# TIGER-AI-Lab/AnyV2V

Measured on AMD Instinct MI355X. Metric: frames/sec for 16fx512x512 DDIM-inversion+PnP-edit; spatial-attn MFMA % of peak, higher is better.
Workload: dtype f16; 1 GPU; BASELINE config 3 per GPU: 1 clip x 16f x 512x512, 50-step DDIM inversion (UNet B=1) + 50-step PnP edit (UNet B=3, cfg 9.0, conv+spatial+temporal injection on every step); a bench step = 1 inversion step + 1 edit step = 1/50 clip; I2VGen-XL 3D-UNet 1.42B params, random init; frames=16, hip_graphs=True, finite=True

## Files before the change

anyv2v_amd/_lib.py:

```python
from __future__ import annotations

import ctypes as C
import os

_HERE = os.path.dirname(os.path.abspath(__file__))
LIB_PATH = os.path.join(_HERE, "libanyv2v_hip.so")
ABI_VERSION = 105


class HipExtensionMissing(RuntimeError):
    pass


class HipKernelError(RuntimeError):
    pass


class GemmDesc(C.Structure):
    _fields_ = [
        ("A0", C.c_void_p), ("A1", C.c_void_p), ("W", C.c_void_p), ("C", C.c_void_p),
        ("bias", C.c_void_p), ("rowvec", C.c_void_p), ("R", C.c_void_p),
        ("M", C.c_int32), ("N", C.c_int32), ("C0", C.c_int32), ("C1", C.c_int32),
        ("lda0", C.c_int32), ("lda1", C.c_int32), ("ldc", C.c_int32), ("ldr", C.c_int32),
        ("ldrv", C.c_int32), ("rowvec_div", C.c_int32), ("mode", C.c_int32),
        ("Hi", C.c_int32), ("Wi", C.c_int32), ("Ho", C.c_int32), ("Wo", C.c_int32),
        ("stride", C.c_int32), ("up", C.c_int32), ("asym", C.c_int32), ("F", C.c_int32), ("HW", C.c_int32),
        ("act", C.c_int32), ("flags", C.c_int32),
        ("workspace", C.c_void_p), ("workspace_bytes", C.c_int64),
        ("ln_c1", C.c_void_p), ("ln_eps", C.c_float), ("reserved0", C.c_int32),
        ("gn_stats", C.c_void_p), ("gn_stats_floats", C.c_int64), ("gn_rows_per_group", C.c_int32), ("gn_groups", C.c_int32),
    ]

ANYV2V_GEMM_NAIVE = 1 << 0
ANYV2V_GEMM_LDS_DMA = 1 << 1
ANYV2V_GEMM_NO_BIG = 1 << 2
ANYV2V_GEMM_FORCE_BIG = 1 << 3
ANYV2V_GEMM_NO_SPLITK = 1 << 4
ANYV2V_GEMM_PROBE_TRACE = 1 << 5
ANYV2V_GEMM_PROBE_KO_SHIFT = 6
ANYV2V_GEMM_NO_WS = 1 << 9
ANYV2V_GEMM_FORCE_WS = 1 << 10
ANYV2V_GEMM_NF4 = 1 << 11
ANYV2V_GEMM_NF5 = 1 << 12
ANYV2V_GEMM_RASTER_SHIFT = 13
ANYV2V_GEMM_RASTER_NFAST = 1 << 16
ANYV2V_GEMM_PP = 1 << 17
ANYV2V_GEMM_NO_PP = 1 << 18
ANYV2V_GEMM_PP_192 = 1 << 19
ANYV2V_GEMM_PP_256 = 1 << 20
ANYV2V_GEMM_SW = 1 << 21
ANYV2V_GEMM_NO_SW = 1 << 22
ANYV2V_GEMM_PROBE_SW_KO_SHIFT = 23
ANYV2V_GEMM_STREAMK = 1 << 26
ANYV2V_GEMM_FORCE_STREAMK = 1 << 27
ANYV2V_GEMM_SWH = 1 << 28
ANYV2V_GEMM_PROBE_KORDER_SHIFT = 29


class FFDesc(C.Structure):
    _fields_ = [
        ("X", C.c_void_p), ("W1", C.c_void_p), ("b1", C.c_void_p), ("W2", C.c_void_p), ("b2", C.c_void_p), ("R", C.c_void_p),
        ("Y", C.c_void_p), ("M", C.c_int32), ("C", C.c_int32), ("H", C.c_int32), ("ldx", C.c_int32), ("ldr", C.c_int32),
        ("ldy", C.c_int32), ("flags", C.c_int32), ("reserved0", C.c_int32),
    ]


class AttnDesc(C.Structure):
    _fields_ = [
        ("Q", C.c_void_p), ("K", C.c_void_p), ("V", C.c_void_p), ("O", C.c_void_p),
        ("ldq", C.c_int32), ("ldk", C.c_int32), ("ldv", C.c_int32), ("ldo", C.c_int32),
        ("batch", C.c_int32), ("heads", C.c_int32), ("Sq", C.c_int32), ("Sk", C.c_int32),
        ("inner", C.c_int32),
        ("q_outer", C.c_int64), ("q_inner", C.c_int64), ("q_seq", C.c_int64),
        ("kv_outer", C.c_int64), ("kv_inner", C.c_int64), ("kv_seq", C.c_int64),
        ("kv_div", C.c_int32), ("qk_mod", C.c_int32), ("scale", C.c_float), ("flags", C.c_int32),
    ]


_VP, _I32, _I64, _F32 = C.c_void_p, C.c_int32, C.c_int64, C.c_float
SYMBOLS = {
    "anyv2v_gemm_f16": (C.c_int, [C.POINTER(GemmDesc), _VP]),
    "anyv2v_gemm_gn_stats_floats": (C.c_int64, [C.POINTER(GemmDesc)]),
    "anyv2v_gemm_gn_launches": (C.c_int64, [_I32]),
    "anyv2v_ff_geglu_f16": (C.c_int, [C.POINTER(FFDesc), _VP]),
    "anyv2v_groupnorm_f16": (C.c_int, [_VP, _VP, _I32, _I32, _VP, _VP, _VP, _VP, _I32, _I32, _I32, _F32, _I32, _VP]),
    "anyv2v_groupnorm_scratch_floats": (C.c_int64, [_I32, _I32, _I32]),
    "anyv2v_groupnorm_stats_floats": (C.c_int64, [_I32, _I32, _I32]),
    "anyv2v_groupnorm_apply_stats_f16": (C.c_int, [_VP, _VP, _VP, _VP, _VP, C.POINTER(C.c_int32), _F32, _I32, _VP]),
    "anyv2v_groupnorm_partial_floats": (C.c_int64, [_I32, _I32, _I32, _I32]),
    "anyv2v_groupnorm_partial_f16": (C.c_int, [_VP, _VP, _I32, _I32, _VP, _I32, _I32, _I32, _VP]),
    "anyv2v_groupnorm_apply_f16": (C.c_int, [_VP, _VP, _I32, _I32, _VP, _VP, _VP, _VP, _I32, _I32, _I32, _F32, _I32, _I32, _VP]),
    "anyv2v_groupnorm_pivot_f16": (C.c_int, [_VP, _VP, _I32, _I32, _VP, _I32, _I32, _I32, _I32, _VP]),
    "anyv2v_groupnorm_partial_pivot_f16": (C.c_int, [_VP, _VP, _I32, _I32, _VP, _VP, _I32, _I32, _I32, _VP]),
    "anyv2v_groupnorm_apply_pivot_f16": (C.c_int, [_VP, _VP, _I32, _I32, _VP, _VP, _VP, _VP, _VP, _I32, _I32, _I32, _F32, _I32, _I32, _VP]),
    "anyv2v_layernorm_f16": (C.c_int, [_VP, _VP, _VP, _VP, _I32, _I32, _F32, _VP]),
    "anyv2v_attention_f16": (C.c_int, [C.POINTER(AttnDesc), _VP]),
    "anyv2v_attention_small_f16": (C.c_int, [C.POINTER(AttnDesc), _I32, _VP]),
    "anyv2v_attention_bias_f16": (C.c_int, [C.POINTER(AttnDesc), _I32, _VP, _VP]),
    "anyv2v_softmax_rows_f32_f16": (C.c_int, [_VP, _I32, _VP, _I32, _I32, _I32, _F32, _VP]),
    "anyv2v_silu_f16": (C.c_int, [_VP, _VP, _I64, _VP]),
    "anyv2v_add_f16": (C.c_int, [_VP, _VP, _VP, _I64, _VP]),
    "anyv2v_timestep_embedding_f16": (C.c_int, [_VP, _VP, _I32, _I32, _VP]),
    "anyv2v_ncfhw_to_tokens_f16": (C.c_int, [_VP, _VP, _I32, _I32, _I32, _I32, _I32, _I32, _VP]),
    "anyv2v_tokens_to_ncfhw_f16": (C.c_int, [_VP, _VP, _I32, _I32, _I32, _I32, _I32, _I32, _VP]),
    "anyv2v_adaptive_avgpool_f16": (C.c_int, [_VP, _VP, _I32, _I32, _I32, _I32, _I32, _I32, _VP]),
    "anyv2v_copy_cols_f16": (C.c_int, [_VP, _I32, _I32, _VP, _I32, _I32, _I64, _I32, _VP]),
    "anyv2v_gather_rows_f16": (C.c_int, [_VP, _I32, _I32, _VP, _VP, _I32, _I32, _I64, _I32, _VP]),
    "anyv2v_freeu_f16": (C.c_int, [_VP, _I32, _VP, _I32, _I32, _F32, _VP, _I32, _VP, _I32, _I32, _F32, _I32, _I32, _I32, _VP]),
    "anyv2v_rotary_f16":(C.c_int, [_VP, _I32, _I64, _I32, _I32, _I32, _I32, _I32, _I32, C.c_float, _VP]),
    "anyv2v_cfg_ddim_step_f16": (C.c_int, [_VP, _I32, _I32, _I32, _F32, _VP, _VP, _VP, _I32, _I32, _I32, _VP]),
    "anyv2v_ddim_step_f16": (C.c_int, [_VP, _VP, _VP, _F32, _F32, _F32, _F32, _I64, _VP]),
    "anyv2v_guided_step_f16": (C.c_int, [_VP, _I64, _I32, _I32, _I32, _F32, _F32, _I32, _F32, _F32, _F32, _F32, _VP, _VP, _VP]),
    "anyv2v_guided_step_noise_f16": (C.c_int, [_VP, _I64, _I32, _I32, _I32, _F32, _F32, _I32, _F32, _F32, _F32, _F32, _VP, _VP, _VP, _F32, _VP]),
    "anyv2v_set_batch_hint": (C.c_int, [_I32, _I32]),
    "anyv2v_last_error": (C.c_char_p, []),
    "anyv2v_version": (C.c_int, []),
    "anyv2v_selftest": (C.c_int, [_VP, _I64, _VP]),
}

_lib = None


def load():
    global _lib
    if _lib is not None:
        return _lib
    if not os.path.isfile(LIB_PATH):
        raise HipExtensionMissing(
            f"{LIB_PATH} not found: the HIP kernels are the product path and there is no fallback. "
            f"Build with `make -C {os.path.join(_HERE, 'csrc')}` (or `python -c 'import __graft_entry__ as g; g.build()'`).")
    lib = C.CDLL(LIB_PATH)
    for name, (res, args) in SYMBOLS.items():
        fn = getattr(lib, name)
        fn.restype = res
        fn.argtypes = args
    if lib.anyv2v_version() < ABI_VERSION:
        raise HipExtensionMissing(f"{LIB_PATH} is ABI {lib.anyv2v_version()}, this binding needs >= {ABI_VERSION}: rebuild it "
                                  f"(`make -C {os.path.join(_HERE, 'csrc')}`)")
    _lib = lib
    return lib


def check(rc: int, what: str = ""):
    if rc != 0:
        msg = load().anyv2v_last_error()
        raise HipKernelError(f"{what} failed (rc={rc}): {msg.decode() if msg else ''}")
```

anyv2v_amd/csrc/gemm.hip:

```cpp
#include <stdlib.h>

#include "gemm_common.h"

__device__ __attribute__((aligned(256))) half_t g_zero_line[128];

static const half_t* zero_line() {
    static const half_t* z = nullptr;
    if (z == nullptr) {
        void* ptr = nullptr;
        if (hipGetSymbolAddress(&ptr, HIP_SYMBOL(g_zero_line)) == hipSuccess) z = (const half_t*)ptr;
    }
    return z;
}

static int64_t g_gn_launches = 0;

extern "C" int anyv2v_gemm_f16(const AnyV2VGemmDesc* d, void* stream) {
    AV_CHECK(d != nullptr, "gemm: null descriptor");
    AV_CHECK(d->A0 && d->W && d->C, "gemm: null A0/W/C");
    const int hinted = av_hint_rows(d->M);
    const GemmPlan plan = av_gemm_plan(*d, hinted);
    AV_CHECK(d->gn_stats == nullptr || plan.gn_decline == nullptr,
             "gemm: gn_stats set, but this launch runs on %s, which writes no GroupNorm statistics (ask anyv2v_gemm_gn_stats_floats first)",
             plan.gn_decline);
    if (plan.status != ANYV2V_OK) return plan.status;
    GemmK k = {};
    k.A0 = (const half_t*)d->A0;
    k.A1 = d->C1 > 0 ? (const half_t*)d->A1 : (const half_t*)d->A0;
    k.W = (const half_t*)d->W;
    k.C = (half_t*)d->C;
    k.bias = (const half_t*)d->bias;
    k.rowvec = (const half_t*)d->rowvec;
    k.R = (const half_t*)d->R;
    k.zeros = zero_line();
    AV_CHECK(k.zeros != nullptr, "gemm: zero line symbol unavailable");
    k.M = d->M; k.N = d->N; k.C0 = d->C0; k.C1 = d->C1;
    k.lda0 = d->lda0; k.lda1 = d->C1 > 0 ? d->lda1 : d->lda0; k.ldc = d->ldc; k.ldr = d->ldr; k.ldrv = d->ldrv;
    k.rowvec_div = d->rowvec_div > 0 ? d->rowvec_div : 1;
    k.mode = d->mode; k.Hi = d->Hi; k.Wi = d->Wi; k.Ho = d->Ho; k.Wo = d->Wo; k.stride = d->stride; k.up = d->up;
    k.F = d->F; k.HW = d->HW; k.act = d->act;
    k.pad_lo = d->asym ? 0 : 1;
    k.taps = plan.taps; k.Ktot = k.taps * (d->C0 + d->C1); k.nt0 = d->C0 / 64; k.nt1 = d->C1 / 64;
    k.tilesN = plan.tilesN; k.vec_epi = plan.vec_epi; k.splits = plan.splits;
    if (plan.splits > 1 || plan.family == GEMM_SW_STREAMK) k.partial = (float*)d->workspace;
    if (plan.family == GEMM_WS_LN) k.ln_c1 = d->ln_c1, k.ln_eps = d->ln_eps;
    k.rast_gm = plan.rast_gm; k.rast_gn = plan.rast_gn; k.rast_sm = plan.rast_sm; k.rast_sn = plan.rast_sn; k.rast_nfast = plan.rast_nfast;
    if (d->gn_stats != nullptr) {
        AV_CHECK(d->gn_stats_floats >= (int64_t)3 * (d->M / 16) * d->gn_groups, "gemm: gn_stats holds %lld floats, the launch writes %lld",
                 (long long)d->gn_stats_floats, (long long)3 * (d->M / 16) * d->gn_groups);
        AV_CHECK((((uintptr_t)d->gn_stats) & 3) == 0, "gemm: gn_stats must be 4-byte aligned");
        k.gn_stats = d->gn_stats;
        k.gn_groups = d->gn_groups;
        k.gn_cg = d->N / d->gn_groups;
        ++g_gn_launches;
    }
    static const bool log_on = getenv("ANYV2V_GEMM_LOG") != nullptr;
    if (log_on)
        fprintf(stderr, "gemm-plan mode %d M %d (hinted %d) N %d K %d act %d res %d big %d splits %d kernel %s nf %d grid %d\n", d->mode, d->M,
                hinted, d->N, k.Ktot, d->act, d->R != nullptr, plan.family == GEMM_BIG, plan.splits, av_gemm_family_name(plan.family),
                plan.nf, plan.grid);
    hipStream_t s = (hipStream_t)stream;
    switch (plan.family) {
    case GEMM_WS:
    case GEMM_WS_LN: return av_gemm_ws_launch(k, d, plan, s);
    case GEMM_SW: return av_gemm_sw_launch(k, d, plan, s);
    case GEMM_SW_STREAMK: return av_gemm_sw_sk_launch(k, d, plan, s);
    case GEMM_SWH: return av_gemm_swh_launch(k, d, plan, s);
    case GEMM_NAIVE: return av_gemm_naive_launch(k, d, plan, s);
    case GEMM_PP: return av_gemm_pp_launch(k, d, plan, s);
    case GEMM_BIG: return av_gemm_big_launch(k, d, plan, s);
    default: return av_gemm_mfma_launch(k, d, plan, s);
    }
}

extern "C" int64_t anyv2v_gemm_gn_stats_floats(const AnyV2VGemmDesc* d) {
    if (d == nullptr) return 0;
    const GemmPlan plan = av_gemm_plan(*d, av_hint_rows(d->M));
    return plan.status == ANYV2V_OK && plan.gn_records ? (int64_t)3 * (d->M / 16) * d->gn_groups : 0;
}

extern "C" int64_t anyv2v_gemm_gn_launches(int32_t reset) {
    const int64_t n = g_gn_launches;
    if (reset) g_gn_launches = 0;
    return n;
}
```

anyv2v_amd/csrc/gemm_big.hip:

```cpp
#include "gemm_common.h"

#ifdef ANYV2V_EXPERIMENTS
#include "../../tools/experiments/gemm_probe_config.h"
#else
constexpr int AV_TRACE_TILE = 0;
#endif

template <int MF, typename PieceFn>
__device__ __forceinline__ void mma_tile_big(f4 (&acc)[MF][10], const char* as, const char* bs, int wr, int wc, int lane,
                                             PieceFn&& piece) {
    const int l15 = lane & 15, lq = lane >> 4;
    const char* a0 = as + (wr * MF * 16 + l15) * 128;
    const char* b0 = bs + (wc * 160 + l15) * 128;
    const int c0 = ((0 * 4 + lq) ^ (l15 & 7)) * 16, c1 = ((1 * 4 + lq) ^ (l15 & 7)) * 16;
    h8 af[2][MF], bf[2][10];
    int seq = 0, a_seq[2] = {0, 0}, b_seq[2][10] = {};
    const unsigned abase[2] = {(unsigned)(size_t)(a0 + c0), (unsigned)(size_t)(a0 + c1)};
    const unsigned bbase[2] = {(unsigned)(size_t)(b0 + c0), (unsigned)(size_t)(b0 + c1)};
#define AV_RA(ks, mf) (af[ks][mf] = lds_frag(abase[ks], (mf) * 2048), a_seq[ks] = ++seq)
#define AV_RB(ks, nf) (bf[ks][nf] = lds_frag(bbase[ks], (nf) * 2048), b_seq[ks][nf] = ++seq)
#pragma unroll
    for (int mf = 0; mf < MF; ++mf) AV_RA(0, mf);
    AV_RB(0, 0);
    AV_RB(0, 1);
    __builtin_amdgcn_sched_barrier(0);
    int npiece = 0;
#pragma unroll
    for (int ks = 0; ks < 2; ++ks) {
#pragma unroll
        for (int nf = 0; nf < 10; ++nf) {
            {
                const int need = b_seq[ks][nf] > a_seq[ks] ? b_seq[ks][nf] : a_seq[ks];
                lgkm_wait(seq - need);
                __builtin_amdgcn_sched_barrier(0);
            }
#pragma unroll
            for (int mf = 0; mf < MF; ++mf)
                acc[mf][nf] = __builtin_amdgcn_mfma_f32_16x16x32_f16(bf[ks][nf], af[ks][mf], acc[mf][nf], 0, 0, 0);
            __builtin_amdgcn_sched_barrier(0);
            if (ks == 0 && nf >= 10 - MF) AV_RA(1, nf - (10 - MF));
            if (nf + 2 < 10) {
                AV_RB(ks, nf + 2);
            } else if (ks == 0) {
                AV_RB(1, nf + 2 - 10);
            }
            if (npiece < MF + 5) piece(npiece++);
            __builtin_amdgcn_sched_barrier(0);
        }
    }
#undef AV_RA
#undef AV_RB
}

template <int MF, bool GEGLU, int MODE, bool TRACE = false, bool SPLIT = false, bool RES = false, bool GN = false>
__global__ __launch_bounds__(512) void gemm_big_kernel(const GemmK p) {
    static_assert(!(RES && (GEGLU || SPLIT)), "no residual on GEGLU / split-K launches");
    static_assert(!(GN && (GEGLU || SPLIT)), "no GroupNorm records on GEGLU / split-K launches");
    constexpr int BM = 64 * MF, BN = 320;
    constexpr int A_BYTES = BM * 128, B_BYTES = BN * 128, STAGE_BYTES = A_BYTES + B_BYTES;
    constexpr int SLAB_LD = (GEGLU ? 80 : 160) + 8;
    constexpr int SLAB_BYTES = 16 * SLAB_LD * 2;
    static_assert(8 * SLAB_BYTES <= STAGE_BYTES, "epilogue slabs must fit in one pipeline stage");
    __shared__ __attribute__((aligned(16))) char smem[2 * STAGE_BYTES];

    const int tid = threadIdx.x, lane = tid & 63, w = tid >> 6, wr = w >> 1, wc = w & 1;
    const int G = gridDim.x;
    const bool rast = !SPLIT && p.rast_gm > 0;
    const int b0 = rast ? (int)blockIdx.x : (((G & 7) == 0) ? (blockIdx.x & 7) * (G >> 3) + (blockIdx.x >> 3) : blockIdx.x);
    const int tilesM = (p.M + BM - 1) / BM;
    const int ntiles_out = tilesM * p.tilesN;
    const int ntiles = SPLIT ? ntiles_out * p.splits : (rast ? G * ((p.rast_sm * p.rast_sn + 7) >> 3) : ntiles_out);
    auto decode = [&](int t, int& mt, int& nt) -> bool {
        if (!rast) {
            const int to = SPLIT ? t % ntiles_out : t;
            mt = to / p.tilesN;
            nt = to - mt * p.tilesN;
            return true;
        }
        const int q = (t & 7) + 8 * (t / G), j = (t % G) >> 3;
        int sm, sn;
        if (p.rast_nfast) {
            sm = q / p.rast_sn;
            sn = q - sm * p.rast_sn;
        } else {
            sn = q / p.rast_sm;
            sm = q - sn * p.rast_sm;
        }
        const int jm = j / p.rast_gn, jn = j - jm * p.rast_gn;
        mt = sm * p.rast_gm + jm;
        nt = sn * p.rast_gn + jn;
        return q < p.rast_sm * p.rast_sn && mt < tilesM;
    };
    auto next_valid = [&](int t) {
        int mt_, nt_;
        while (t < ntiles && !decode(t, mt_, nt_)) t += G;
        return t;
    };

    const int srow0 = tid >> 3, pc = tid & 7, kc = pc ^ (srow0 & 7);
    const int ntap = p.nt0 + p.nt1;
    const int nk_all = p.taps * ntap;
    auto k_begin = [&](int item) { return SPLIT ? (nk_all * (item / ntiles_out)) / p.splits : 0; };
    auto k_end = [&](int item) { return SPLIT ? (nk_all * (item / ntiles_out + 1)) / p.splits : nk_all; };

    RowInfo ri[4];
    const half_t* bptr;
    const size_t brow = (size_t)64 * p.Ktot;
    AGen<MODE, 4> gen;
    auto producer_start = [&](int item) {
        int mt, nt;
        decode(item, mt, nt);
        const int kb = k_begin(item);
#pragma unroll
        for (int i = 0; i < 4; ++i) ri[i] = make_row<MODE>(p, i < MF ? mt * BM + srow0 + 64 * i : p.M);
        bptr = p.W + (size_t)(nt * BN + srow0) * p.Ktot + kc * 8 + (size_t)kb * 64;
        if constexpr (SPLIT)
            gen.start(p, ri, kc, kb, ntap);
        else
            gen.start(p, ri, kc);
    };
    auto advance = [&]() {
        bptr += 64;
        gen.next(p, ri, kc, ntap);
    };
    auto issue = [&](int stage) {
        char* st = smem + stage * STAGE_BYTES;
#pragma unroll
        for (int i = 0; i < MF; ++i) glds16(gen.ap[i], st + (i * 512 + w * 64) * 16);
#pragma unroll
        for (int i = 0; i < 5; ++i) glds16(bptr + i * brow, st + A_BYTES + (i * 512 + w * 64) * 16);
        advance();
    };

    f4 acc[MF][10];
    int tile = next_valid(b0);
    if (tile >= ntiles) return;
    producer_start(tile);
    issue(0);
    int stage = 0;
    bool landed = false;
    bool rederive = false;
    while (true) {
        int mt, nt;
        decode(tile, mt, nt);
        const int nk = k_end(tile) - k_begin(tile);
        const int m_wave = mt * BM + wr * MF * 16;
        const int n_wave = nt * BN + wc * 160;
        const int next_tile = next_valid(tile + G);
        const bool has_next = next_tile < ntiles;
#pragma unroll
        for (int i = 0; i < MF; ++i)
#pragma unroll
            for (int j = 0; j < 10; ++j) acc[i][j] = (f4){0.f, 0.f, 0.f, 0.f};
        if (rederive) {
            producer_start(tile);
            advance();
        }

        for (int kt = 0; kt < nk; ++kt) {
            if constexpr (TRACE) if (tid == 0 && tile == b0 + AV_TRACE_TILE * G && kt < 8) p.trace[(size_t)blockIdx.x * 32 + 2 + 3 * kt] = (long long)__builtin_amdgcn_s_memtime();
            if (kt > 0 || !landed) asm volatile("s_waitcnt vmcnt(0)" ::: "memory");
            if constexpr (TRACE) if (tid == 0 && tile == b0 + AV_TRACE_TILE * G && kt == 3) p.trace[(size_t)blockIdx.x * 32 + 29] = (long long)__builtin_amdgcn_s_memtime();
            __builtin_amdgcn_s_barrier();
            if constexpr (TRACE) if (tid == 0 && tile == b0 + AV_TRACE_TILE * G && kt < 8) p.trace[(size_t)blockIdx.x * 32 + 3 + 3 * kt] = (long long)__builtin_amdgcn_s_memtime();
            const bool last = kt + 1 == nk;
            if (last) producer_start(has_next ? next_tile : tile);
            const bool fetch = !last || has_next;
            const char* as = smem + stage * STAGE_BYTES;
            char* st = smem + (stage ^ 1) * STAGE_BYTES;
            mma_tile_big<MF>(acc, as, as + A_BYTES, wr, wc, lane, [&](int i) {
                if (i < MF)
                    glds16(gen.ap[i], st + (i * 512 + w * 64) * 16);
                else
                    glds16(bptr + (i - MF) * brow, st + A_BYTES + ((i - MF) * 512 + w * 64) * 16);
            });
            if constexpr (TRACE) if (tid == 0 && tile == b0 + AV_TRACE_TILE * G && kt < 8) p.trace[(size_t)blockIdx.x * 32 + 4 + 3 * kt] = (long long)__builtin_amdgcn_s_memtime();
            if (fetch) advance();
            stage ^= 1;
        }
        if constexpr (TRACE) if (tid == 0 && tile == b0 + AV_TRACE_TILE * G) p.trace[(size_t)blockIdx.x * 32 + 26] = (long long)__builtin_amdgcn_s_memtime();
        constexpr int OUT_W = GEGLU ? 80 : 160;
        constexpr int CPRW = OUT_W / 8;
        constexpr int NIT = (16 * CPRW + 63) / 64;
        const int n_out_wave = GEGLU ? n_wave / 2 : n_wave;
        h8 rr[RES ? MF : 1][NIT];
        if constexpr (RES) {
            int lane_r = lane;
            asm volatile("" : "+v"(lane_r));
#pragma unroll
            for (int mf = 0; mf < MF; ++mf)
#pragma unroll
                for (int it = 0; it < NIT; ++it) {
                    const int c = it * 64 + lane_r;
                    const int row = c / CPRW, cc = c - row * CPRW;
                    int m = m_wave + mf * 16 + row;
                    m = m < p.M ? m : p.M - 1;
                    rr[mf][it] = *(const h8*)(p.R + (size_t)m * p.ldr + n_out_wave + cc * 8);
                }
        }
        asm volatile("s_waitcnt vmcnt(0)" ::: "memory");
        if constexpr (TRACE) if (tid == 0 && tile == b0 + AV_TRACE_TILE * G) p.trace[(size_t)blockIdx.x * 32 + 30] = (long long)__builtin_amdgcn_s_memtime();
        __builtin_amdgcn_s_barrier();
        if constexpr (TRACE) if (tid == 0 && tile == b0 + AV_TRACE_TILE * G) p.trace[(size_t)blockIdx.x * 32 + 31] = (long long)__builtin_amdgcn_s_memtime();
        landed = true;
        rederive = true;

        int lane_e = lane;
        asm volatile("" : "+v"(lane_e));
        const int l15 = lane_e & 15, lq = lane_e >> 4;
        if constexpr (SPLIT) {
            float* dst = p.partial + (size_t)(tile / ntiles_out) * p.M * p.N;
#pragma unroll
            for (int mf = 0; mf < MF; ++mf) {
                const int m = m_wave + mf * 16 + l15;
#pragma unroll
                for (int nf = 0; nf < 10; ++nf)
                    if (m < p.M) *(f4*)(dst + (size_t)m * p.N + n_wave + nf * 16 + 4 * lq) = acc[mf][nf];
            }
            if (!has_next) break;
            tile = next_tile;
            continue;
        }
        if constexpr (SPLIT) __builtin_unreachable();
        half_t* const slab = (half_t*)(smem + (stage ^ 1) * STAGE_BYTES + w * SLAB_BYTES);
        h4 bvec[10];
#pragma unroll
        for (int nf = 0; nf < 10; ++nf)
            bvec[nf] = *(const h4*)(p.bias != nullptr ? p.bias + n_wave + nf * 16 + 4 * lq : p.zeros);
        if constexpr (RES) {
#pragma unroll
            for (int mf = 0; mf < MF; ++mf)
#pragma unroll
                for (int it = 0; it < NIT; ++it) asm volatile("" : "+v"(rr[mf][it]));
        }
#pragma unroll
        for (int mf = 0; mf < MF; ++mf) {
            if constexpr (GEGLU) {
#pragma unroll
                for (int np = 0; np < 5; ++np) {
                    h4 o;
#pragma unroll
                    for (int r = 0; r < 4; ++r) {
                        const float hv = acc[mf][2 * np][r] + (float)bvec[2 * np][r];
                        const float gv = acc[mf][2 * np + 1][r] + (float)bvec[2 * np + 1][r];
                        o[r] = (half_t)(hv * av_gelu(gv));
                    }
                    *(h4*)(slab + l15 * SLAB_LD + np * 16 + 4 * lq) = o;
                }
            } else {
                const bool has_rv = p.rowvec != nullptr;
                const int mrow = m_wave + mf * 16 + l15;
                const half_t* rv = has_rv ? p.rowvec + (size_t)((mrow < p.M ? mrow : 0) / p.rowvec_div) * p.ldrv + n_wave + 4 * lq
                                          : p.zeros;
#pragma unroll
                for (int nf = 0; nf < 10; ++nf) {
                    h4 tv = (h4){0, 0, 0, 0};
                    if (has_rv) tv = *(const h4*)(rv + nf * 16);
                    h4 o;
#pragma unroll
                    for (int r = 0; r < 4; ++r) o[r] = (half_t)(acc[mf][nf][r] + (float)bvec[nf][r] + (float)tv[r]);
                    *(h4*)(slab + l15 * SLAB_LD + nf * 16 + 4 * lq) = o;
                }
            }
#pragma unroll
            for (int it = 0; it < NIT; ++it) {
                const int c = it * 64 + lane_e;
                const int row = c / CPRW, cc = c - row * CPRW;
                const bool ok = (16 * CPRW % 64 == 0 || c < 16 * CPRW) && m_wave + mf * 16 + row < p.M;
                h8 v = *(const h8*)(slab + (ok ? row * SLAB_LD + cc * 8 : 0));
                if constexpr (RES) v = v + rr[mf][it];
                if constexpr (RES && GN) {
                    if (ok) *(h8*)(slab + row * SLAB_LD + cc * 8) = v;
                }
                if (ok) *(h8*)(p.C + (size_t)(m_wave + mf * 16 + row) * p.ldc + n_out_wave + cc * 8) = v;
            }
            if constexpr (GN) {
                const int m0 = m_wave + mf * 16;
                if (m0 < p.M)
                    gn_slab_records(slab, SLAB_LD, p.gn_cg, lane_e, p.gn_stats + ((size_t)(m0 >> 4) * p.gn_groups + n_wave / p.gn_cg) * 3);
            }
        }

        if constexpr (TRACE) {
            if (tid == 0 && tile == b0 + AV_TRACE_TILE * G) {
                p.trace[(size_t)blockIdx.x * 32 + 27] = (long long)__builtin_amdgcn_s_memtime();
                p.trace[(size_t)blockIdx.x * 32 + 28] = nk;
            }
        }
        if (!has_next) break;
        tile = next_tile;
    }
}

#define AV_GO(kernel, threads) hipLaunchKernelGGL((kernel), grid, dim3(threads), 0, s, k)
template <int MODE>
static int big_launch_mode(GemmK k, const AnyV2VGemmDesc* d, const GemmPlan& plan, hipStream_t s) {
    const bool geglu = d->act == ACT_GEGLU, res = d->R != nullptr, gn = k.gn_stats != nullptr;
    const dim3 grid((unsigned)plan.grid);
    if (plan.splits > 1) {
        AV_GO((gemm_big_kernel<3, false, MODE, false, true>), 512);
        av_gemm_splitk_reduce_launch(k, s);
        return av_launch_status("gemm_big<split-K>");
    }
#ifdef ANYV2V_EXPERIMENTS
#include "../../tools/experiments/gemm_dispatch_big_probe.inc"
#endif
    if (gn) {
        if (res) AV_GO((gemm_big_kernel<3, false, MODE, false, false, true, true>), 512);
        else AV_GO((gemm_big_kernel<3, false, MODE, false, false, false, true>), 512);
        return av_launch_status("gemm_big<gn>");
    }
    if constexpr (MODE == MODE_LINEAR) {
        if (geglu) {
            AV_GO((gemm_big_kernel<3, true, MODE_LINEAR>), 512);
            return av_launch_status("gemm_big");
        }
    }
    if (res) AV_GO((gemm_big_kernel<3, false, MODE, false, false, true>), 512);
    else AV_GO((gemm_big_kernel<3, false, MODE>), 512);
    return av_launch_status("gemm_big");
}
#undef AV_GO

int av_gemm_big_launch(const GemmK& k, const AnyV2VGemmDesc* d, const GemmPlan& plan, hipStream_t s) {
    if (d->mode == MODE_CONV2D) return big_launch_mode<MODE_CONV2D>(k, d, plan, s);
    if (d->mode == MODE_TEMPORAL) return big_launch_mode<MODE_TEMPORAL>(k, d, plan, s);
    return big_launch_mode<MODE_LINEAR>(k, d, plan, s);
}
```

anyv2v_amd/csrc/gemm_common.h:

```cpp
#pragma once
#include "common.h"
#include "gemm_plan.h"

struct GemmK {
    const half_t* A0;
    const half_t* A1;
    const half_t* W;
    half_t* C;
    const half_t* bias;
    const half_t* rowvec;
    const half_t* R;
    const half_t* zeros;
    int M, N, C0, C1, lda0, lda1, ldc, ldr, ldrv, rowvec_div;
    int mode, Hi, Wi, Ho, Wo, stride, up, F, HW, act;
    int pad_lo;
    int taps, Ktot, nt0, nt1, tilesN;
    int vec_epi;
    int splits;
    float* partial;
    long long* trace;
    const float* ln_c1;
    float ln_eps;
    int rast_gm, rast_gn, rast_sm, rast_sn, rast_nfast;
    float* gn_stats;
    int gn_groups, gn_cg;
};

struct RowInfo {
    int base;
    int y, x;
};

template <int MODE>
__device__ __forceinline__ RowInfo make_row(const GemmK& p, int m) {
    RowInfo r;
    const bool ok = m < p.M;
    if constexpr (MODE == MODE_CONV2D) {
        const int hw = p.Ho * p.Wo;
        const int img = m / hw, rem = m - img * hw;
        const int yo = rem / p.Wo, xo = rem - yo * p.Wo;
        r.base = img * p.Hi * p.Wi;
        r.y = ok ? yo * p.stride - p.pad_lo : -(1 << 28);
        r.x = xo * p.stride - p.pad_lo;
    } else if constexpr (MODE == MODE_TEMPORAL) {
        r.base = m;
        r.y = ok ? (m / p.HW) % p.F : -(1 << 28);
        r.x = 0;
    } else {
        r.base = ok ? m : -1;
        r.y = r.x = 0;
    }
    return r;
}

template <int MODE>
__device__ __forceinline__ int src_row(const GemmK& p, const RowInfo& r, int tap) {
    if constexpr (MODE == MODE_CONV2D) {
        const int dy = tap / 3, dx = tap - dy * 3;
        int yi = r.y + dy, xi = r.x + dx;
        const int ly = p.Hi << p.up, lx = p.Wi << p.up;
        const bool ok = (yi >= 0) & (yi < ly) & (xi >= 0) & (xi < lx);
        yi >>= p.up;
        xi >>= p.up;
        return ok ? r.base + yi * p.Wi + xi : -1;
    } else if constexpr (MODE == MODE_TEMPORAL) {
        const int f = r.y + tap - 1;
        const bool ok = (f >= 0) & (f < p.F);
        return ok ? r.base + (tap - 1) * p.HW : -1;
    } else {
        return r.base;
    }
}

struct ASrc {
    const half_t* base;
    int ld;
};
__device__ __forceinline__ ASrc a_source(const GemmK& p, int kt_c, int kc) {
    ASrc s;
    const bool first = kt_c < p.nt0;
    s.base = (first ? p.A0 + kt_c * 64 : p.A1 + (kt_c - p.nt0) * 64) + kc * 8;
    s.ld = first ? p.lda0 : p.lda1;
    return s;
}
__device__ __forceinline__ const half_t* a_addr(const GemmK& p, const ASrc& s, int sr) {
    const half_t* g = s.base + (long long)sr * s.ld;
    return sr < 0 ? p.zeros : g;
}

template <int MODE, int ROWS, int ORD = 0>
struct AGen {
    const half_t* ap[ROWS];
    int astep[ROWS];
    int ktc, tap;
    __device__ __forceinline__ void recompute(const GemmK& p, const RowInfo (&ri)[ROWS], int kc) {
        const ASrc s = a_source(p, ktc, kc);
#pragma unroll
        for (int i = 0; i < ROWS; ++i) {
            const int sr = src_row<MODE>(p, ri[i], tap);
            ap[i] = a_addr(p, s, sr);
            astep[i] = sr < 0 ? 0 : 64;
        }
    }
    __device__ __forceinline__ void start(const GemmK& p, const RowInfo (&ri)[ROWS], int kc, int kt0 = 0, int ntap = 1) {
        tap = kt0 / ntap;
        ktc = kt0 - tap * ntap;
        recompute(p, ri, kc);
    }
    __device__ __forceinline__ void next(const GemmK& p, const RowInfo (&ri)[ROWS], int kc, int ntap) {
        if constexpr (ORD == 1) {
            if (++tap == p.taps) {
                tap = 0;
                ++ktc;
            }
            recompute(p, ri, kc);
            return;
        }
        if (++ktc == ntap) {
            ktc = 0;
            ++tap;
        }
        if (ktc == 0 || ktc == p.nt0) {
            recompute(p, ri, kc);
        } else {
#pragma unroll
            for (int i = 0; i < ROWS; ++i) ap[i] += astep[i];
        }
    }
    __device__ __forceinline__ void bump() {
#pragma unroll
        for (int i = 0; i < ROWS; ++i) ap[i] += astep[i];
    }
    __device__ __forceinline__ void count(const GemmK& p, const RowInfo (&ri)[ROWS], int kc, int ntap) {
        if (++ktc == ntap) {
            ktc = 0;
            ++tap;
        }
        if (ktc == 0 || ktc == p.nt0) recompute(p, ri, kc);
    }
};

__device__ __forceinline__ void glds16(const half_t* g, char* lds_wave_base) {
    __builtin_amdgcn_global_load_lds((const __attribute__((address_space(1))) void*)g,
                                     (__attribute__((address_space(3))) void*)lds_wave_base, 16, 0, 0);
}

#if defined(HIP_VERSION_MAJOR) && (HIP_VERSION_MAJOR != 7 || HIP_VERSION_MINOR != 2)
#warning "GEMM kernels: inline-asm LDS fragment reads were validated with ROCm 7.2 only; rerun tests/test_isa_guards.py and the -m gpu suite"
#endif
__device__ __forceinline__ h8 lds_frag(unsigned base, int off) {
    h8 v;
    asm volatile("ds_read_b128 %0, %1 offset:%2" : "=v"(v) : "v"(base), "n"(off) : "memory");
    return v;
}
__device__ __forceinline__ h8 lds_frag(unsigned addr) {
    h8 v;
    asm volatile("ds_read_b128 %0, %1" : "=v"(v) : "v"(addr) : "memory");
    return v;
}
__device__ __forceinline__ void lgkm_wait(int n) {
    switch (n) {
#define AV_LGW(k) case k: asm volatile("s_waitcnt lgkmcnt(" #k ")" ::: "memory"); break;
        AV_LGW(0) AV_LGW(1) AV_LGW(2) AV_LGW(3) AV_LGW(4) AV_LGW(5) AV_LGW(6) AV_LGW(7) AV_LGW(8) AV_LGW(9) AV_LGW(10)
        AV_LGW(11) AV_LGW(12) AV_LGW(13) AV_LGW(14) AV_LGW(15)
#undef AV_LGW
        default: asm volatile("s_waitcnt lgkmcnt(15)" ::: "memory"); break;
    }
}

__device__ __forceinline__ float acc_read(const float& a) {
    float v;
    asm volatile("v_accvgpr_read_b32 %0, %1" : "=v"(v) : "a"(a));
    return v;
}

__device__ __forceinline__ void gn_slab_records(const half_t* slab, int ld, int cg, int lane, float* dst) {
    const int r = lane & 15, q = lane >> 4;
    const int ngq = 40 / cg;
    for (int gi = 0; gi < ngq; ++gi) {
        const int gl = q * ngq + gi;
        const half_t* g0 = slab + gl * cg;
        const float K = (float)g0[0];
        const half_t* x = g0 + r * ld;
        float s = 0.f, qq = 0.f;
        for (int c = 0; c < cg; ++c) {
            const float f = (float)x[c] - K;
            s += f;
            qq = fmaf(f, f, qq);
        }
#pragma unroll
        for (int o = 1; o < 16; o <<= 1) {
            s += __shfl_xor(s, o, 64);
            qq += __shfl_xor(qq, o, 64);
        }
        if (r == 0) {
            float* o = dst + gl * 3;
            o[0] = K;
            o[1] = s;
            o[2] = qq;
        }
    }
}

int av_gemm_mfma_launch(const GemmK& k, const AnyV2VGemmDesc* d, const GemmPlan& plan, hipStream_t s);
int av_gemm_big_launch(const GemmK& k, const AnyV2VGemmDesc* d, const GemmPlan& plan, hipStream_t s);
int av_gemm_pp_launch(const GemmK& k, const AnyV2VGemmDesc* d, const GemmPlan& plan, hipStream_t s);
int av_gemm_naive_launch(const GemmK& k, const AnyV2VGemmDesc* d, const GemmPlan& plan, hipStream_t s);
void av_gemm_splitk_reduce_launch(const GemmK& k, hipStream_t s);
struct WsPlan {
    int S;
    int px;
    int nstrips;
    int spr;
    int trace_waves;
};
int av_gemm_ws_launch(const GemmK& k, const AnyV2VGemmDesc* d, const GemmPlan& plan, hipStream_t s);
int av_gemm_sw_launch(const GemmK& k, const AnyV2VGemmDesc* d, const GemmPlan& plan, hipStream_t s);
int av_gemm_sw_sk_launch(const GemmK& k, const AnyV2VGemmDesc* d, const GemmPlan& plan, hipStream_t s);
int av_gemm_swh_launch(const GemmK& k, const AnyV2VGemmDesc* d, const GemmPlan& plan, hipStream_t s);
```

anyv2v_amd/csrc/gemm_mfma.hip:

```cpp
#include <type_traits>

#include "gemm_common.h"

template <int NF, bool GEGLU, int BM, int NTHREADS, bool GN = false>
__device__ __forceinline__ void epilogue(const GemmK& p, f4 (&acc)[4][NF], char* smem, int m_blk, int n_blk, int wr,
                                         int wc, int lane, int tid, int split = 0, long long* tr = nullptr) {
    constexpr int BN = NF * 32;
    constexpr int BNO = GEGLU ? BN / 2 : BN;
    constexpr int CS_LD = BNO + 8;
    half_t* const Cs = (half_t*)smem;
    const int l15 = lane & 15, lq = lane >> 4;
    if (p.splits > 1) {
        float* dst = p.partial + (size_t)split * p.M * p.N;
#pragma unroll
        for (int mf = 0; mf < 4; ++mf) {
            const int m = m_blk + wr * 64 + mf * 16 + l15;
#pragma unroll
            for (int nf = 0; nf < NF; ++nf) {
                const int n = n_blk + wc * NF * 16 + nf * 16 + 4 * lq;
                if (m < p.M && n + 4 <= p.N) *(f4*)(dst + (size_t)m * p.N + n) = acc[mf][nf];
            }
        }
        return;
    }
    if (p.act == ACT_F32OUT) {
        float* dst = (float*)p.C;
#pragma unroll
        for (int mf = 0; mf < 4; ++mf) {
            const int m = m_blk + wr * 64 + mf * 16 + l15;
#pragma unroll
            for (int nf = 0; nf < NF; ++nf) {
                const int n = n_blk + wc * NF * 16 + nf * 16 + 4 * lq;
                if (m < p.M && n + 4 <= p.N) {
                    f4 v = acc[mf][nf];
                    if (p.bias != nullptr) {
                        const h4 b = *(const h4*)(p.bias + n);
#pragma unroll
                        for (int r = 0; r < 4; ++r) v[r] += (float)b[r];
                    }
                    *(f4*)(dst + (size_t)m * p.ldc + n) = v;
                }
            }
        }
        return;
    }
    const int Nout = GEGLU ? p.N / 2 : p.N;
    const int n_out_blk = GEGLU ? n_blk / 2 : n_blk;
    constexpr int CPR = BNO / 8;
    constexpr int NIT = BM * CPR / NTHREADS;
    static_assert(BM * CPR % NTHREADS == 0, "store phase assumes an exact chunk split");
    const bool full_chunks = (Nout & 7) == 0;
    h8 rr[NIT];
    if (p.R != nullptr && full_chunks) {
#pragma unroll
        for (int it = 0; it < NIT; ++it) {
            const int id = tid + it * NTHREADS;
            const int r = id / CPR, cc = id - r * CPR;
            const int m = m_blk + r, n0 = n_out_blk + cc * 8;
            rr[it] = *(const h8*)((m < p.M && n0 < Nout) ? p.R + (size_t)m * p.ldr + n0 : p.zeros);
        }
    }
    h4 bvec[NF];
#pragma unroll
    for (int nf = 0; nf < NF; ++nf) {
        const int n = n_blk + wc * NF * 16 + nf * 16 + 4 * lq;
        const half_t* src = (p.bias != nullptr && n + 4 <= p.N) ? p.bias + n : p.zeros;
        bvec[nf] = *(const h4*)src;
    }
    h4 tvec[GEGLU ? 1 : 4][GEGLU ? 1 : NF];
    const bool has_rowvec = !GEGLU && p.rowvec != nullptr;
    if constexpr (!GEGLU) {
        if (has_rowvec) {
#pragma unroll
            for (int mf = 0; mf < 4; ++mf) {
                const int m = m_blk + wr * 64 + mf * 16 + l15;
                const bool ok = m < p.M;
                const half_t* rv = p.rowvec + (size_t)((ok ? m : 0) / p.rowvec_div) * p.ldrv;
#pragma unroll
                for (int nf = 0; nf < NF; ++nf) {
                    const int n = n_blk + wc * NF * 16 + nf * 16 + 4 * lq;
                    tvec[mf][nf] = *(const h4*)((ok && n + 4 <= p.N) ? rv + n : p.zeros);
                }
            }
        }
    }
    if constexpr (GEGLU) {
#pragma unroll
        for (int mf = 0; mf < 4; ++mf) {
            const int ml = wr * 64 + mf * 16 + l15;
#pragma unroll
            for (int np = 0; np < NF / 2; ++np) {
                h4 o;
#pragma unroll
                for (int r = 0; r < 4; ++r) {
                    const float hv = acc[mf][2 * np][r] + (float)bvec[2 * np][r];
                    const float gv = acc[mf][2 * np + 1][r] + (float)bvec[2 * np + 1][r];
                    o[r] = (half_t)(hv * av_gelu(gv));
                }
                *(h4*)(Cs + ml * CS_LD + wc * NF * 8 + np * 16 + 4 * lq) = o;
            }
        }
    } else {
        auto stage = [&](auto act_tag) {
            constexpr int ACT = decltype(act_tag)::value;
#pragma unroll
            for (int mf = 0; mf < 4; ++mf) {
                const int ml = wr * 64 + mf * 16 + l15;
#pragma unroll
                for (int nf = 0; nf < NF; ++nf) {
                    const int nl = wc * NF * 16 + nf * 16 + 4 * lq;
                    h4 o;
#pragma unroll
                    for (int r = 0; r < 4; ++r) {
                        float v = acc[mf][nf][r] + (float)bvec[nf][r];
                        if (has_rowvec) v += (float)tvec[mf][nf][r];
                        if constexpr (ACT == ACT_SILU) v = av_silu(v);
                        if constexpr (ACT == ACT_GELU) v = av_gelu(v);
                        o[r] = (half_t)v;
                    }
                    *(h4*)(Cs + ml * CS_LD + nl) = o;
                }
            }
        };
        if (p.act == ACT_SILU)
            stage(std::integral_constant<int, ACT_SILU>{});
        else if (p.act == ACT_GELU)
            stage(std::integral_constant<int, ACT_GELU>{});
        else
            stage(std::integral_constant<int, ACT_NONE>{});
    }
    if (tr != nullptr && tid == 0) tr[24] = (long long)__builtin_amdgcn_s_memtime();
    __syncthreads();
    if (tr != nullptr && tid == 0) tr[25] = (long long)__builtin_amdgcn_s_memtime();
    if (full_chunks) {
#pragma unroll
        for (int it = 0; it < NIT; ++it) {
            const int id = tid + it * NTHREADS;
            const int r = id / CPR, cc = id - r * CPR;
            const int m = m_blk + r, n0 = n_out_blk + cc * 8;
            h8 v = *(const h8*)(Cs + r * CS_LD + cc * 8);
            if (p.R != nullptr) {
                v = v + rr[it];
                if constexpr (GN) *(h8*)(Cs + r * CS_LD + cc * 8) = v;
            }
            if (m < p.M && n0 < Nout) *(h8*)(p.C + (size_t)m * p.ldc + n0) = v;
        }
        if constexpr (GN) {
            static_assert(!GEGLU && BN == 160 && BM % 16 == 0, "GroupNorm records: 160-column tiles of 16-row fragments");
            if (p.R != nullptr) __syncthreads();
            const int wv = tid >> 6;
            for (int f = wv; f < BM / 16; f += NTHREADS / 64) {
                const int m0 = m_blk + f * 16;
                if (m0 < p.M)
                    gn_slab_records(Cs + f * 16 * CS_LD, CS_LD, p.gn_cg, lane,
                                    p.gn_stats + ((size_t)(m0 >> 4) * p.gn_groups + n_blk / p.gn_cg) * 3);
            }
        }
        return;
    }
    for (int id = tid; id < BM * CPR; id += NTHREADS) {
        const int r = id / CPR, cc = id - r * CPR;
        const int m = m_blk + r;
        const int n0 = n_out_blk + cc * 8;
        if (m >= p.M || n0 >= Nout) continue;
        const h8 v = *(const h8*)(Cs + r * CS_LD + cc * 8);
        for (int e = 0; e < 8 && n0 + e < Nout; ++e) {
            float x = (float)v[e];
            if (p.R != nullptr) x += (float)p.R[(size_t)m * p.ldr + n0 + e];
            p.C[(size_t)m * p.ldc + n0 + e] = (half_t)x;
        }
    }
}

template <int NF, int KO = 0>
__device__ __forceinline__ void mma_tile(f4 (&acc)[4][NF], const char* as, const char* bs, int wr, int wc, int lane) {
    const int l15 = lane & 15, lq = lane >> 4;
    h8 af[2][4], bf[2][NF];
#pragma unroll
    for (int ks = 0; ks < 2; ++ks) {
        const int c = (ks * 4 + lq) ^ (l15 & 7);
        if constexpr (KO == 4) {
            h8 x;
#pragma unroll
            for (int e = 0; e < 8; ++e) x[e] = (half_t)(float)(lane + e);
            asm volatile("" : "+v"(x));
#pragma unroll
            for (int nf = 0; nf < NF; ++nf) bf[ks][nf] = x;
#pragma unroll
            for (int mf = 0; mf < 4; ++mf) af[ks][mf] = x;
        } else {
#pragma unroll
            for (int nf = 0; nf < NF; ++nf) bf[ks][nf] = *(const h8*)(bs + ((wc * NF * 16 + nf * 16 + l15) * 8 + c) * 16);
#pragma unroll
            for (int mf = 0; mf < 4; ++mf) af[ks][mf] = *(const h8*)(as + ((wr * 64 + mf * 16 + l15) * 8 + c) * 16);
        }
    }
    if constexpr (KO == 5) {
#pragma unroll
        for (int ks = 0; ks < 2; ++ks) {
#pragma unroll
            for (int nf = 0; nf < NF; ++nf) asm volatile("" ::"v"(bf[ks][nf]));
#pragma unroll
            for (int mf = 0; mf < 4; ++mf) asm volatile("" ::"v"(af[ks][mf]));
        }
        return;
    }
#pragma unroll
    for (int ks = 0; ks < 2; ++ks)
#pragma unroll
        for (int mf = 0; mf < 4; ++mf)
#pragma unroll
            for (int nf = 0; nf < NF; ++nf)
                acc[mf][nf] = __builtin_amdgcn_mfma_f32_16x16x32_f16(bf[ks][nf], af[ks][mf], acc[mf][nf], 0, 0, 0);
    if constexpr (KO == 4) {
        __builtin_amdgcn_sched_barrier(0);
        return;
    }
    __builtin_amdgcn_sched_group_barrier(0x100, 4 + NF, 0);
#pragma unroll
    for (int i = 0; i < 4 + NF; ++i) {
        __builtin_amdgcn_sched_group_barrier(0x008, 2, 0);
        __builtin_amdgcn_sched_group_barrier(0x100, 1, 0);
    }
    __builtin_amdgcn_sched_group_barrier(0x008, 8 * NF - 2 * (4 + NF), 0);
    __builtin_amdgcn_sched_barrier(0);
}

template <int NF>
__device__ __forceinline__ void mma_tile_asm(f4 (&acc)[4][NF], const char* as, const char* bs, int wr, int wc, int lane) {
    const int l15 = lane & 15, lq = lane >> 4;
    const int c0 = ((0 * 4 + lq) ^ (l15 & 7)) * 16, c1 = ((1 * 4 + lq) ^ (l15 & 7)) * 16;
    const char* a0 = as + (wr * 64 + l15) * 128;
    const char* b0 = bs + (wc * NF * 16 + l15) * 128;
    const unsigned abase[2] = {(unsigned)(size_t)(a0 + c0), (unsigned)(size_t)(a0 + c1)};
    const unsigned bbase[2] = {(unsigned)(size_t)(b0 + c0), (unsigned)(size_t)(b0 + c1)};
    h8 af[2][4], bf[2][NF];
    int seq = 0, done = 0, a_seq[2][4] = {}, b_seq[2][NF] = {};
#define AV_RA(ks, mf) (af[ks][mf] = lds_frag(abase[ks], (mf) * 2048), a_seq[ks][mf] = ++seq)
#define AV_RB(ks, nf) (bf[ks][nf] = lds_frag(bbase[ks], (nf) * 2048), b_seq[ks][nf] = ++seq)
    AV_RA(0, 0);
#pragma unroll
    for (int nf = 0; nf < NF; ++nf) AV_RB(0, nf);
#pragma unroll
    for (int mf = 1; mf < 4; ++mf) AV_RA(0, mf);
    __builtin_amdgcn_sched_barrier(0);
    int slot = 0;
#pragma unroll
    for (int ks = 0; ks < 2; ++ks)
#pragma unroll
        for (int mf = 0; mf < 4; ++mf)
#pragma unroll
            for (int nf = 0; nf < NF; ++nf) {
                const int need = a_seq[ks][mf] > b_seq[ks][nf] ? a_seq[ks][mf] : b_seq[ks][nf];
                if (need > done) {
                    lgkm_wait(seq - need);
                    done = need;
                    __builtin_amdgcn_sched_barrier(0);
                }
                acc[mf][nf] = __builtin_amdgcn_mfma_f32_16x16x32_f16(bf[ks][nf], af[ks][mf], acc[mf][nf], 0, 0, 0);
                if (ks == 0 && ((mf * NF + nf) & 1) && slot < 4 + NF) {
                    __builtin_amdgcn_sched_barrier(0);
                    if (slot == 0)
                        AV_RA(1, 0);
                    else if (slot <= NF)
                        AV_RB(1, slot - 1);
                    else
                        AV_RA(1, slot - NF);
                    ++slot;
                    __builtin_amdgcn_sched_barrier(0);
                }
            }
#undef AV_RA
#undef AV_RB
    __builtin_amdgcn_sched_barrier(0);
}

template <int NF, bool GLDS, bool GEGLU, int MODE, bool TRACE = false, int KO = 0, bool GN = false>
__global__ __launch_bounds__(256, 2) void gemm_mfma_kernel(const GemmK p) {
    constexpr int BM = 128, BN = NF * 32;
    constexpr int A_BYTES = BM * 64 * 2;
    constexpr int B_BYTES = BN * 64 * 2;
    constexpr int NB = BN / 32;
    __shared__ __attribute__((aligned(16))) char smem[2 * (A_BYTES + B_BYTES)];
    char* const As0 = smem;
    char* const Bs0 = smem + 2 * A_BYTES;

    const int tid = threadIdx.x, lane = tid & 63, w = tid >> 6, wr = w >> 1, wc = w & 1;
    int bid = blockIdx.x;
    const int nwg = gridDim.x;
    long long* tr = nullptr;
    if constexpr (TRACE) {
        tr = p.trace + (size_t)blockIdx.x * 32;
        if (tid == 0) {
            tr[0] = ((long long)__builtin_amdgcn_s_getreg((3 << 11) | 20) << 32) | (unsigned)__builtin_amdgcn_s_getreg((31 << 11) | 4);
            tr[1] = (long long)__builtin_amdgcn_s_memrealtime();
            tr[2] = (long long)__builtin_amdgcn_s_memtime();
        }
    }
    if ((nwg & 7) == 0) bid = (bid & 7) * (nwg >> 3) + (bid >> 3);
    const int ntiles = nwg / p.splits;
    const int split = bid / ntiles;
    bid -= split * ntiles;
    const int mt = bid / p.tilesN, nt = bid - mt * p.tilesN;
    const int m_blk = mt * BM, n_blk = nt * BN;

    const int srow0 = tid >> 3;
    const int pc = tid & 7;
    const int kc = pc ^ (srow0 & 7);
    RowInfo ri[4];
#pragma unroll
    for (int i = 0; i < 4; ++i) ri[i] = make_row<MODE>(p, m_blk + srow0 + 32 * i);
    const half_t* bptr[NB];
#pragma unroll
    for (int i = 0; i < NB; ++i) {
        int n = n_blk + srow0 + 32 * i;
        n = n < p.N ? n : p.N - 1;
        bptr[i] = p.W + (size_t)n * p.Ktot + kc * 8;
    }

    h8 ra[4], rb[NB];
    const int ntap = p.nt0 + p.nt1;
    const int nk_all = p.taps * ntap;
    const int kt_begin = (int)(((long long)nk_all * split) / p.splits);
    const int kt_end = (int)(((long long)nk_all * (split + 1)) / p.splits);
#pragma unroll
    for (int i = 0; i < NB; ++i) bptr[i] += (size_t)kt_begin * 64;
    AGen<MODE, 4> gen;
    gen.start(p, ri, kc, kt_begin, ntap);
    auto issue = [&](int buf, bool with_a = true) {
#pragma unroll
        for (int i = 0; i < 4; ++i) {
            if constexpr (GLDS) {
                if (with_a) glds16(gen.ap[i], As0 + buf * A_BYTES + (i * 256 + w * 64) * 16);
            } else {
                ra[i] = *(const h8*)gen.ap[i];
            }
        }
#pragma unroll
        for (int i = 0; i < NB; ++i) {
            if constexpr (GLDS)
                glds16(bptr[i], Bs0 + buf * B_BYTES + (i * 256 + w * 64) * 16);
            else
                rb[i] = *(const h8*)bptr[i];
            bptr[i] += 64;
        }
        gen.next(p, ri, kc, ntap);
    };
    auto commit = [&](int buf) {
#pragma unroll
        for (int i = 0; i < 4; ++i) *(h8*)(As0 + buf * A_BYTES + ((srow0 + 32 * i) * 8 + pc) * 16) = ra[i];
#pragma unroll
        for (int i = 0; i < NB; ++i) *(h8*)(Bs0 + buf * B_BYTES + ((srow0 + 32 * i) * 8 + pc) * 16) = rb[i];
    };

    f4 acc[4][NF];
#pragma unroll
    for (int i = 0; i < 4; ++i)
#pragma unroll
        for (int j = 0; j < NF; ++j) acc[i][j] = (f4){0.f, 0.f, 0.f, 0.f};

    const int nk = kt_end - kt_begin;
    issue(0);
    if constexpr (!GLDS) commit(0);
    if constexpr (GLDS) asm volatile("s_waitcnt vmcnt(0)" ::: "memory");
    __syncthreads();
    if constexpr (TRACE) if (tid == 0) tr[3] = (long long)__builtin_amdgcn_s_memtime();
    for (int kt = 0; kt < nk; ++kt) {
        const int cur = kt & 1;
        const bool has_next = kt + 1 < nk;
        if (has_next && KO != 3) issue(cur ^ 1, KO != 2);
        if constexpr (GLDS && KO == 0)
            mma_tile_asm<NF>(acc, As0 + cur * A_BYTES, Bs0 + cur * B_BYTES, wr, wc, lane);
        else
            mma_tile<NF, KO>(acc, As0 + cur * A_BYTES, Bs0 + cur * B_BYTES, wr, wc, lane);
        if constexpr (TRACE) if (tid == 0 && kt < 8) tr[4 + kt] = (long long)__builtin_amdgcn_s_memtime();
        if constexpr (!GLDS) {
            if (has_next) commit(cur ^ 1);
        } else {
            asm volatile("s_waitcnt vmcnt(0)" ::: "memory");
        }
        __syncthreads();
        if constexpr (TRACE) if (tid == 0 && kt < 8) tr[12 + kt] = (long long)__builtin_amdgcn_s_memtime();
    }
    if constexpr (TRACE) if (tid == 0) tr[20] = (long long)__builtin_amdgcn_s_memtime();
    epilogue<NF, GEGLU, BM, 256, GN>(p, acc, smem, m_blk, n_blk, wr, wc, lane, tid, split, tr);
    if constexpr (TRACE) {
        if (tid == 0) tr[26] = (long long)__builtin_amdgcn_s_memtime();
        asm volatile("s_waitcnt vmcnt(0)" ::: "memory");
        if (tid == 0) {
            tr[21] = (long long)__builtin_amdgcn_s_memtime();
            tr[22] = (long long)__builtin_amdgcn_s_memrealtime();
            tr[23] = nk;
        }
    }
}

#define AV_GO(kernel, threads) hipLaunchKernelGGL((kernel), grid, dim3(threads), 0, s, k)
template <int MODE>
static int mfma_launch_mode(GemmK k, const AnyV2VGemmDesc* d, const GemmPlan& plan, hipStream_t s) {
    const bool geglu = d->act == ACT_GEGLU, gn = k.gn_stats != nullptr;
    const bool glds = (d->flags & ANYV2V_GEMM_LDS_DMA) != 0;
    const dim3 grid((unsigned)plan.grid);
#ifdef ANYV2V_EXPERIMENTS
#include "../../tools/experiments/gemm_dispatch_mfma_probe.inc"
#endif
    if (gn) AV_GO((gemm_mfma_kernel<5, true, false, MODE, false, 0, true>), 256);
    else if (geglu && glds) AV_GO((gemm_mfma_kernel<4, true, true, MODE>), 256);
    else if (geglu) AV_GO((gemm_mfma_kernel<4, false, true, MODE>), 256);
    else if (plan.nf == 5 && glds) AV_GO((gemm_mfma_kernel<5, true, false, MODE>), 256);
    else if (plan.nf == 5) AV_GO((gemm_mfma_kernel<5, false, false, MODE>), 256);
    else if (glds) AV_GO((gemm_mfma_kernel<4, true, false, MODE>), 256);
    else AV_GO((gemm_mfma_kernel<4, false, false, MODE>), 256);
    if (plan.splits > 1) av_gemm_splitk_reduce_launch(k, s);
    return av_launch_status("gemm_mfma");
}
#undef AV_GO

int av_gemm_mfma_launch(const GemmK& k, const AnyV2VGemmDesc* d, const GemmPlan& plan, hipStream_t s) {
    if (d->mode == MODE_CONV2D) return mfma_launch_mode<MODE_CONV2D>(k, d, plan, s);
    if (d->mode == MODE_TEMPORAL) return mfma_launch_mode<MODE_TEMPORAL>(k, d, plan, s);
    return mfma_launch_mode<MODE_LINEAR>(k, d, plan, s);
}
```

anyv2v_amd/csrc/gemm_plan.cpp:

```cpp
#include "gemm_plan.h"

const char* av_gemm_family_name(GemmFamily f) {
    static const char* const names[] = {"naive", "ws", "ws_ln", "mfma128", "big", "pp", "sw", "sw_streamk", "swh"};
    static_assert(sizeof(names) / sizeof(names[0]) == GEMM_FAMILY_COUNT, "one name per family");
    return names[f];
}

namespace {
bool aligned16(const void* p) { return (((uintptr_t)p) & 15) == 0; }
int ceil_div(int a, int b) { return (a + b - 1) / b; }

#define PLAN_FAIL(code, ...) do { anyv2v_set_error(__VA_ARGS__); p.status = code; return p; } while (0)
#define PLAN_CHECK(cond, ...) if (!(cond)) PLAN_FAIL(ANYV2V_EINVAL, __VA_ARGS__)

int ws_slab_cols(const AnyV2VGemmDesc& d) {
    if (d.C0 == 320) return 160;
    if (d.C0 == 512) return d.act == ACT_GEGLU ? 128 : (d.N == 512 ? 64 : 0);
    return 0;
}
bool ws_eligible(const AnyV2VGemmDesc& d) {
    const int ns = ws_slab_cols(d);
    if (d.ln_c1 != nullptr && (d.R != nullptr || (d.C0 == 512 && d.act != ACT_GEGLU))) return false;
    return d.mode == MODE_LINEAR && ns > 0 && d.C1 == 0 && d.N % ns == 0 && d.N / ns <= 32 &&
           (d.act == ACT_NONE || (d.act == ACT_GEGLU && d.R == nullptr)) && d.rowvec == nullptr && d.M > 0;
}

bool sw_eligible(const AnyV2VGemmDesc& d, int nk) {
    const bool geglu = d.act == ACT_GEGLU;
    return d.N % 320 == 0 && (geglu ? d.mode == MODE_LINEAR && d.R == nullptr && d.rowvec == nullptr : d.act == ACT_NONE) &&
           !(d.R != nullptr && d.rowvec != nullptr) && nk >= 2 && d.ldc % 8 == 0 && (d.R == nullptr || d.ldr % 8 == 0) &&
           (d.rowvec == nullptr || d.ldrv % 8 == 0);
}
size_t sw_sk_workspace(int blocks) { return (size_t)2 * blocks * AV_GEMM_BM * AV_GEMM_BN * sizeof(float); }
int sw_sk_blocks(int tiles, int nk, bool force) {
    const long long U = (long long)tiles * nk;
    if (U < 256 * 4 || U > (1ll << 22)) return force && U >= 8 ? (int)(U / 4 < 256 ? U / 4 : 256) : 0;
    if (force) return 256;
    const int rounds = (tiles + 255) / 256;
    const double eff = (double)tiles / (rounds * 256.0);
    return eff < 0.9 ? 256 : 0;
}

bool swh_eligible(const AnyV2VGemmDesc& d) {
    return d.mode == MODE_CONV2D && d.stride == 1 && d.up == 0 && d.asym == 0 && d.Hi == d.Ho && d.Wi == d.Wo &&
           (d.Wi == 16 || d.Wi == 32 || d.Wi == 64) && d.N % 320 == 0 && d.act == ACT_NONE && d.C0 % 64 == 0 && d.C1 % 64 == 0 &&
           !(d.R != nullptr && d.rowvec != nullptr) && d.ldc % 8 == 0 && (d.R == nullptr || d.ldr % 8 == 0) &&
           (d.rowvec == nullptr || d.ldrv % 8 == 0);
}

bool gn_shape_ok(const AnyV2VGemmDesc& d) {
    if (d.gn_groups <= 0 || d.gn_rows_per_group <= 0 || d.N % 160 != 0 || d.N % d.gn_groups != 0) return false;
    const int cg = d.N / d.gn_groups;
    return 40 % cg == 0 && d.M % 16 == 0 && d.gn_rows_per_group % 16 == 0 && d.M % d.gn_rows_per_group == 0 &&
           (d.act == ACT_NONE || d.act == ACT_SILU || d.act == ACT_GELU);
}

void persistent_grid(GemmPlan& p, const AnyV2VGemmDesc& d) {
    p.tilesN = d.N / AV_GEMM_BN;
    p.tiles = ceil_div(d.M, AV_GEMM_BM) * p.tilesN;
    p.grid = p.tiles < 256 ? p.tiles : 256;
}
void raster(GemmPlan& p, const AnyV2VGemmDesc& d) {
    const int code = (d.flags >> ANYV2V_GEMM_RASTER_SHIFT) & 7;
    static const int gm_of[8] = {0, 0, 4, 8, 16, 32, 2, 0};
    int gm = gm_of[code];
    if (code == 0 && p.tilesN >= 8 && p.tiles >= 512) gm = 8;
    if (gm > 0 && p.grid == 256 && p.tilesN % (32 / gm) == 0) {
        p.rast_gm = gm;
        p.rast_gn = 32 / gm;
        p.rast_sm = ceil_div(ceil_div(d.M, AV_GEMM_BM), gm);
        p.rast_sn = p.tilesN / p.rast_gn;
        p.rast_nfast = (d.flags & ANYV2V_GEMM_RASTER_NFAST) != 0;
    }
}

}

GemmPlan av_gemm_plan(const AnyV2VGemmDesc& d, int hinted_rows) {
    GemmPlan p = {};
    p.nf = 4;
    p.splits = p.tilesN = 1;
    auto take = [&p](GemmFamily family, const char* what) { p.family = family; p.gn_decline = what; return p; };
    PLAN_CHECK(d.A0 && d.W, "gemm: null A0/W/C");
    PLAN_CHECK(d.M > 0 && d.N > 0 && d.C0 > 0 && d.C1 >= 0, "gemm: bad M/N/C0/C1 (%d %d %d %d)", d.M, d.N, d.C0, d.C1);
    PLAN_CHECK(d.mode >= 0 && d.mode <= 2, "gemm: bad mode %d", d.mode);
    PLAN_CHECK(d.act >= 0 && d.act <= 4, "gemm: bad act %d", d.act);
    PLAN_CHECK(d.act != ACT_F32OUT || (d.rowvec == nullptr && d.R == nullptr && d.N % 4 == 0 && d.ldc % 4 == 0),
               "gemm: fp32 output supports bias only and needs N, ldc multiples of 4");
    PLAN_CHECK(d.asym == 0 || d.asym == 1, "gemm: asym must be 0 or 1");
    PLAN_CHECK(d.C1 == 0 || d.A1 != nullptr, "gemm: C1 > 0 but A1 is null");
    PLAN_CHECK(d.rowvec == nullptr || d.rowvec_div > 0, "gemm: rowvec needs rowvec_div > 0");
    if (d.mode == MODE_CONV2D) {
        PLAN_CHECK(d.Hi > 0 && d.Wi > 0 && d.Ho > 0 && d.Wo > 0 && (d.stride == 1 || d.stride == 2), "gemm: bad conv geometry");
        PLAN_CHECK(d.M % (d.Ho * d.Wo) == 0, "gemm: M not a multiple of Ho*Wo");
        PLAN_CHECK(d.up == 0 || d.up == 1, "gemm: up must be 0 or 1");
    }
    if (d.mode == MODE_TEMPORAL) { PLAN_CHECK(d.F > 0 && d.HW > 0 && d.M % (d.F * d.HW) == 0, "gemm: bad temporal geometry"); }
    const bool geglu = d.act == ACT_GEGLU;
    if (geglu) {
        PLAN_CHECK(d.N % 32 == 0, "gemm: GEGLU needs N %% 32 == 0");
        PLAN_CHECK(d.rowvec == nullptr, "gemm: GEGLU with rowvec unsupported");
    }
    p.taps = d.mode == MODE_LINEAR ? 1 : (d.mode == MODE_CONV2D ? 9 : 3);
    p.nk = p.taps * (d.C0 / 64 + d.C1 / 64);
    p.vec_epi = (((uintptr_t)d.bias & 7) == 0) && (((uintptr_t)d.rowvec & 7) == 0) && (d.ldrv % 4 == 0) && (d.N % 4 == 0);
    const int flags = d.flags, nk = p.nk;
    const bool glds = (flags & ANYV2V_GEMM_LDS_DMA) != 0;
    const bool fast = !(flags & ANYV2V_GEMM_NAIVE) && d.C0 % 64 == 0 && d.C1 % 64 == 0 && d.lda0 % 8 == 0 &&
                      (d.C1 == 0 || d.lda1 % 8 == 0) && d.ldc % 8 == 0 && aligned16(d.A0) && (d.C1 == 0 || aligned16(d.A1)) &&
                      aligned16(d.W) && aligned16(d.C) && (d.R == nullptr || (d.ldr % 8 == 0 && aligned16(d.R))) &&
                      (!geglu || d.N % 128 == 0) && p.vec_epi;

    const bool ws_ok = fast && glds && ws_eligible(d);
    const bool ws_take = ws_ok && !(flags & (ANYV2V_GEMM_NO_WS | ANYV2V_GEMM_NO_BIG)) && (hinted_rows >= 32768 || (flags & ANYV2V_GEMM_FORCE_WS));
    if (d.ln_c1 != nullptr || ws_take) {
        p.grid = 256;
        if (ws_ok) p.tilesN = d.N / ws_slab_cols(d);
        if (d.ln_c1 == nullptr) return take(GEMM_WS, "the weight-stationary kernel");
        take(GEMM_WS_LN, "the LayerNorm-fold kernel");
        if (!(ws_ok && aligned16(d.ln_c1)))
            PLAN_FAIL(ANYV2V_EUNSUPPORTED, "gemm: ln_c1 (LayerNorm fold) needs mode 0, C0 = 320 (N %% 160 = 0) or C0 = 512 with GEGLU "
                      "(N %% 128 = 0), no residual / rowvec, 16-byte aligned operands -- got C0 %d N %d act %d", d.C0, d.N, d.act);
        return p;
    }
    if (!fast) {
        p.grid = (int)(unsigned)(((long long)d.M * (geglu ? d.N / 2 : d.N) + 255) / 256);
        return take(GEMM_NAIVE, "the naive kernel");
    }
    const bool sw_on = glds && !(flags & ANYV2V_GEMM_NO_SW);
    if (sw_on && (flags & (ANYV2V_GEMM_STREAMK | ANYV2V_GEMM_FORCE_STREAMK)) && sw_eligible(d, nk) && hinted_rows == d.M &&
        d.workspace != nullptr) {
        persistent_grid(p, d);
        const int blocks = sw_sk_blocks(p.tiles, nk, (flags & ANYV2V_GEMM_FORCE_STREAMK) != 0);
        if (blocks > 0 && sw_sk_workspace(blocks) <= (size_t)d.workspace_bytes) {
            p.grid = p.sk_blocks = blocks;
            return take(GEMM_SW_STREAMK, "the stream-K kernel");
        }
    }
    if (sw_on && (flags & ANYV2V_GEMM_SWH) && swh_eligible(d)) {
        persistent_grid(p, d);
        return take(GEMM_SWH, "the LDS-patch convolution kernel");
    }
    if (sw_on && (flags & ANYV2V_GEMM_SW) && sw_eligible(d, nk)) {
        persistent_grid(p, d);
        raster(p, d);
        return take(GEMM_SW, "the one-wave-per-SIMD kernel");
    }
    auto choose_nf = [&](int rows) -> int {
        int nf_ = geglu ? 4 : (d.N % 160 == 0 ? 5 : 4);
        if (!geglu && nf_ == 5 && d.N % 128 == 0) {
            const int mt = (rows + 127) / 128;
            const int t5 = mt * (d.N / 160), t4 = mt * (d.N / 128);
            const bool would_split = t4 < 384 && ((t4 <= 128 && nk >= 32) || nk >= 72);
            const bool prefer4 = !would_split && ((t4 <= 256) || (t5 > 256 && (t5 + 511) / 512 == (t4 + 511) / 512));
            if (((flags & ANYV2V_GEMM_NF4) || prefer4) && !(flags & ANYV2V_GEMM_NF5)) nf_ = 4;
        }
        return nf_;
    };
    const bool big_ok = glds && !(flags & ANYV2V_GEMM_NO_BIG) && d.N % 320 == 0 && (!geglu || d.mode == MODE_LINEAR) &&
                        (geglu || d.act == ACT_NONE);
    const size_t split_ws_bytes = (size_t)d.workspace_bytes < ((size_t)64 << 20) ? (size_t)d.workspace_bytes : ((size_t)64 << 20);
    struct Choice { bool big; int splits; };
    auto choose = [&](int rows) -> Choice {
        const bool ws_buf = d.workspace != nullptr && d.N % 8 == 0;
        if (big_ok) {
            const int tb = ceil_div(rows, AV_GEMM_BM) * (d.N / 320);
            const int rounds = (tb + 255) / 256;
            const bool fills = tb >= 224 && tb * 4 >= rounds * 256 * 3;
            if (!fills && !geglu && !(flags & (ANYV2V_GEMM_NO_SPLITK | ANYV2V_GEMM_FORCE_BIG)) && ws_buf && tb <= 128 && nk >= 72) {
                int sp = 256 / tb;
                if (sp > 8) sp = 8;
                if (sp > nk / 12) sp = nk / 12;
                if (sp >= 2 && tb * sp >= 224 && (size_t)sp * rows * d.N * sizeof(float) <= split_ws_bytes) return {true, sp};
            }
            if (fills || (flags & ANYV2V_GEMM_FORCE_BIG)) return {true, 1};
        }
        const int tm = ((rows + 127) / 128) * ceil_div(d.N, choose_nf(rows) * 32);
        const bool split_pays = (tm <= 128 && nk >= 32) || nk >= 72;
        if (glds && !geglu && d.act != ACT_F32OUT && !(flags & ANYV2V_GEMM_NO_SPLITK) && ws_buf && tm < 384 && split_pays) {
            int sp = (512 + tm - 1) / tm;
            if (sp > 8) sp = 8;
            if (sp > nk / 8) sp = nk / 8;
            if (sp >= 2 && (size_t)sp * rows * d.N * sizeof(float) <= split_ws_bytes) return {false, sp};
        }
        return {false, 1};
    };
    Choice use = choose(d.M);
    if (hinted_rows != d.M) {
        const Choice ref = choose(hinted_rows);
        if (ref.splits > 1)
            use = ref;
        else if (use.splits > 1)
            use = Choice{false, 1};
    }
    p.splits = use.splits;
    if (big_ok && !geglu && use.splits == 1 && !(flags & ANYV2V_GEMM_NO_PP) && (flags & ANYV2V_GEMM_PP)) {
        auto tiles_of = [&](int mf) { return ceil_div(d.M, 64 * mf) * (d.N / 320); };
        auto eff = [&](int mf) { return (double)tiles_of(mf) / (((tiles_of(mf) + 255) / 256) * 256.0); };
        p.pp_mf = (flags & ANYV2V_GEMM_PP_192) ? 3 : ((flags & ANYV2V_GEMM_PP_256) ? 4 : (eff(4) + 0.02 >= eff(3) ? 4 : 3));
        p.tilesN = d.N / 320;
        p.tiles = tiles_of(p.pp_mf);
        p.grid = p.tiles < 256 ? p.tiles : 256;
        return take(GEMM_PP, "the ping-pong kernel");
    }
    if (use.splits > 1)
        p.gn_decline = "a split-K plan";
    else if (geglu || d.act == ACT_F32OUT || !glds || !gn_shape_ok(d))
        p.gn_decline = "a GEGLU / fp32-output / register-staged launch or a shape the record layout does not cover (N % 160 = 0, "
                       "N / gn_groups dividing 40, M and gn_rows_per_group multiples of 16)";
    else
        p.gn_records = true;
    if (use.big) {
        p.family = GEMM_BIG;
        persistent_grid(p, d);
        if (use.splits > 1)
            p.grid = p.tiles * use.splits < 256 ? p.tiles * use.splits : 256;
        else
            raster(p, d);
        return p;
    }
    p.family = GEMM_MFMA128;
    p.nf = d.gn_stats != nullptr && p.gn_records ? 5 : choose_nf(d.M);
    p.tilesN = ceil_div(d.N, p.nf * 32);
    p.tiles = ((d.M + 127) / 128) * p.tilesN;
    p.grid = p.tiles * p.splits;
    return p;
}
```

anyv2v_amd/csrc/gemm_plan.h:

```cpp
#pragma once
#include <stddef.h>

#include "../../include/anyv2v_hip.h"

enum { MODE_LINEAR = 0, MODE_CONV2D = 1, MODE_TEMPORAL = 2 };
enum { ACT_NONE = 0, ACT_SILU = 1, ACT_GELU = 2, ACT_GEGLU = 3, ACT_F32OUT = 4 };

enum GemmFamily { GEMM_NAIVE, GEMM_WS, GEMM_WS_LN, GEMM_MFMA128, GEMM_BIG, GEMM_PP, GEMM_SW, GEMM_SW_STREAMK, GEMM_SWH, GEMM_FAMILY_COUNT };
const char* av_gemm_family_name(GemmFamily f);
void anyv2v_set_error(const char* fmt, ...);

constexpr int AV_GEMM_BM = 192, AV_GEMM_BN = 320;

struct GemmPlan {
    int status;
    GemmFamily family;
    int taps, nk;
    bool vec_epi;
    int nf;
    int splits;
    int tilesN, tiles, grid;
    int rast_gm, rast_gn, rast_sm, rast_sn, rast_nfast;
    int pp_mf;
    int sk_blocks;
    bool gn_records;
    const char* gn_decline;
};

GemmPlan av_gemm_plan(const AnyV2VGemmDesc& d, int hinted_rows);
```

anyv2v_amd/ops.py:

```python
from __future__ import annotations

import ctypes as C
import os
from typing import Optional

import torch

from . import _lib
from ._lib import AttnDesc, GemmDesc

MODE_LINEAR, MODE_CONV2D, MODE_TEMPORAL = 0, 1, 2
ACT_NONE, ACT_SILU, ACT_GELU, ACT_GEGLU, ACT_F32OUT = 0, 1, 2, 3, 4

FORCE_NAIVE = False
ATTN_FLAGS = int(os.environ.get("ANYV2V_ATTN_FLAGS", "0"))
GEMM_FLAGS = int(os.environ.get("ANYV2V_GEMM_FLAGS", "0"))
USE_GLDS = os.environ.get("ANYV2V_GLDS", "1") == "1"


def _parse_switch(value: Optional[str]) -> bool:
    return (value or "0").strip() == "1"


GN_EPILOGUE = _parse_switch(os.environ.get("ANYV2V_GN_EPILOGUE"))


def _stream() -> int:
    return torch.cuda.current_stream().cuda_stream


def _p(t: Optional[torch.Tensor]) -> Optional[int]:
    return None if t is None else t.data_ptr()


def _rowmajor(t: torch.Tensor, name: str):
    assert t.dim() == 2 and t.stride(1) == 1, f"{name}: need a 2-D row-major (stride(1)==1) fp16 view, got {tuple(t.shape)} {t.stride()}"
    assert t.dtype == torch.float16, f"{name}: fp16 expected, got {t.dtype}"
    assert t.is_cuda, f"{name}: device tensor expected"


_WS = {}
WS_SLOT = 0


class workspace_slot:

    def __init__(self, slot: int):
        self.slot, self.prev = int(slot), 0

    def __enter__(self):
        global WS_SLOT
        self.prev, WS_SLOT = WS_SLOT, self.slot
        return self

    def __exit__(self, *exc):
        global WS_SLOT
        WS_SLOT = self.prev
        return False


def _workspace(device) -> torch.Tensor:
    key = f"{device}:{WS_SLOT}"
    if key not in _WS:
        _WS[key] = torch.empty(32 * 1024 * 1024, dtype=torch.float32, device=device)
    return _WS[key]


def gemm(a0: torch.Tensor, w: torch.Tensor, *, a1: Optional[torch.Tensor] = None, bias=None, rowvec=None,
         rowvec_div: int = 0, residual=None, act: int = ACT_NONE, out: Optional[torch.Tensor] = None,
         mode: int = MODE_LINEAR, conv=None, temporal=None, M: Optional[int] = None, naive: bool = False, ln=None, gn=None,
         _query: bool = False):
    lib = _lib.load()
    _rowmajor(a0, "A0")
    _rowmajor(w, "W")
    C0 = a0.shape[1]
    C1 = 0
    if a1 is not None:
        _rowmajor(a1, "A1")
        C1 = a1.shape[1]
    taps = 1 if mode == MODE_LINEAR else (9 if mode == MODE_CONV2D else 3)
    N = w.shape[0]
    assert w.shape[1] == taps * (C0 + C1), f"W is {tuple(w.shape)}, expected [{N}, {taps}*({C0}+{C1})]"
    assert w.stride(0) == w.shape[1], "W must be contiguous"
    if M is None:
        M = a0.shape[0]
    n_out = N // 2 if act == ACT_GEGLU else N
    if _query and out is None:
        pass
    elif act == ACT_F32OUT:
        if out is None:
            out = torch.empty((M, n_out), dtype=torch.float32, device=a0.device)
        assert out.dim() == 2 and out.stride(1) == 1 and out.dtype == torch.float32 and out.is_cuda
        assert rowvec is None and residual is None
    else:
        if out is None:
            out = torch.empty((M, n_out), dtype=torch.float16, device=a0.device)
        _rowmajor(out, "C")
    assert out is None or (out.shape[0] >= M and out.shape[1] >= n_out)
    d = GemmDesc()
    d.A0, d.A1, d.W, d.C = _p(a0), _p(a1), _p(w), _p(out)
    d.bias, d.rowvec, d.R = _p(bias), _p(rowvec), _p(residual)
    d.M, d.N, d.C0, d.C1 = M, N, C0, C1
    d.lda0 = a0.stride(0)
    d.lda1 = a1.stride(0) if a1 is not None else 0
    d.ldc = out.stride(0) if out is not None else n_out
    d.ldr = residual.stride(0) if residual is not None else 0
    d.ldrv = rowvec.stride(0) if rowvec is not None else 0
    d.rowvec_div = rowvec_div
    d.mode = mode
    if mode == MODE_CONV2D:
        d.Hi, d.Wi, d.Ho, d.Wo, d.stride, d.up = conv[:6]
        d.asym = conv[6] if len(conv) > 6 else 0
    elif mode == MODE_TEMPORAL:
        d.F, d.HW = temporal
    d.act = act
    d.flags = ((_lib.ANYV2V_GEMM_NAIVE if (naive or FORCE_NAIVE) else 0) | (_lib.ANYV2V_GEMM_LDS_DMA if USE_GLDS else 0)
               | GEMM_FLAGS)
    if ln is not None:
        c1, eps = ln
        assert c1.dtype == torch.float32 and c1.is_cuda and c1.numel() >= N and c1.is_contiguous()
        d.ln_c1, d.ln_eps = _p(c1), float(eps)
    ws = _workspace(a0.device)
    d.workspace, d.workspace_bytes = ws.data_ptr(), ws.numel() * 4
    if gn is not None:
        stats, rows_per_group, groups = gn
        d.gn_rows_per_group, d.gn_groups = int(rows_per_group), int(groups)
        if stats is not None:
            assert stats.dtype == torch.float32 and stats.is_cuda and stats.is_contiguous()
            d.gn_stats, d.gn_stats_floats = stats.data_ptr(), stats.numel()
    if _query:
        return int(lib.anyv2v_gemm_gn_stats_floats(C.byref(d)))
    _lib.check(lib.anyv2v_gemm_f16(C.byref(d), _stream()), "anyv2v_gemm_f16")
    return out


def gemm_gn_stats_floats(a0: torch.Tensor, w: torch.Tensor, *, rows_per_group: int, groups: int = 32, **kw) -> int:
    return gemm(a0, w, gn=(None, rows_per_group, groups), _query=True, **kw)


def gn_launches(reset: bool = True) -> int:
    return int(_lib.load().anyv2v_gemm_gn_launches(int(reset)))


def gn_stats_floats(M: int, rows_per_group: int, groups: int = 32) -> int:
    return int(_lib.load().anyv2v_groupnorm_stats_floats(int(M), int(rows_per_group), int(groups)))


def groupnorm_from_stats(x: torch.Tensor, gamma, beta, stats: torch.Tensor, rows_per_group: int, *, groups: int = 32,
                         eps: float = 1e-5, silu: bool = False, out=None):
    lib = _lib.load()
    _rowmajor(x, "X")
    assert x.is_contiguous()
    M, Cc = x.shape
    if out is None:
        out = torch.empty((M, Cc), dtype=torch.float16, device=x.device)
    assert out.is_contiguous()
    assert stats.dtype == torch.float32 and stats.is_contiguous() and stats.numel() >= gn_stats_floats(M, rows_per_group, groups) > 0
    sizes = (C.c_int32 * 5)(M, Cc, rows_per_group, groups, min(stats.numel(), 2 ** 31 - 1))
    _lib.check(lib.anyv2v_groupnorm_apply_stats_f16(_p(x), _p(out), _p(gamma), _p(beta), _p(stats), sizes, eps, int(silu),
                                                    _stream()), "anyv2v_groupnorm_apply_stats_f16")
    return out


FF_FUSED = os.environ.get("ANYV2V_FF_FUSED", "1") == "1"


def ff_fused_supported(M: int, C: int, H: int) -> bool:
    return FF_FUSED and not FORCE_NAIVE and USE_GLDS and C == 320 and H == 1280 and M * _HINT[0] // _HINT[1] >= 32768


def ff_pack_w2(w2: torch.Tensor) -> torch.Tensor:
    C, H = w2.shape
    assert H % 32 == 0
    q, e = torch.arange(4).view(4, 1), torch.arange(8).view(1, 8)
    perm = torch.where(e < 4, 4 * q + e, 16 + 4 * q + (e - 4)).reshape(32).to(w2.device)
    return w2.view(C, H // 32, 32)[:, :, perm].permute(1, 0, 2).contiguous()


def ff_geglu(x: torch.Tensor, w1p: torch.Tensor, b1p: torch.Tensor, w2s: torch.Tensor, b2: torch.Tensor, residual=None, out=None):
    lib = _lib.load()
    M, Cc = x.shape
    H = w2s.shape[0] * 32
    assert x.dtype == torch.float16 and x.stride(1) == 1 and w1p.is_contiguous() and w2s.is_contiguous()
    assert tuple(w1p.shape) == (2 * H, Cc) and tuple(w2s.shape) == (H // 32, Cc, 32) and b1p.numel() == 2 * H and b2.numel() == Cc
    if out is None:
        out = torch.empty((M, Cc), dtype=torch.float16, device=x.device)
    for name, t in (("residual", residual), ("out", out)):
        assert t is None or (tuple(t.shape) == (M, Cc) and t.dtype == torch.float16 and t.stride(1) == 1 and t.device == x.device), \
            f"ff_geglu: {name} must be an fp16 [{M}, {Cc}] matrix with unit column stride on {x.device}"
    d = _lib.FFDesc()
    d.X, d.W1, d.b1, d.W2, d.b2, d.Y = _p(x), _p(w1p), _p(b1p), _p(w2s), _p(b2), _p(out)
    d.R = _p(residual) if residual is not None else None
    d.M, d.C, d.H = M, Cc, H
    d.ldx, d.ldy, d.ldr = x.stride(0), out.stride(0), (residual.stride(0) if residual is not None else 0)
    d.flags = d.reserved0 = 0
    _lib.check(lib.anyv2v_ff_geglu_f16(C.byref(d), _stream()), "anyv2v_ff_geglu_f16")
    return out


def ln_gemm_supported(M: int, K: int, N: int, act: int = ACT_NONE, hinted: bool = True) -> bool:
    if FORCE_NAIVE or not USE_GLDS or (GEMM_FLAGS & (_lib.ANYV2V_GEMM_NO_WS | _lib.ANYV2V_GEMM_NO_BIG)) or (M * _HINT[0] // _HINT[1] if hinted else M) < 32768:
        return False
    if K == 320:
        return N % 160 == 0 and N // 160 <= 32
    return K == 512 and act == ACT_GEGLU and N % 128 == 0 and N // 128 <= 32


def ln_fold(w: torch.Tensor, bias: Optional[torch.Tensor], gamma: torch.Tensor, beta: torch.Tensor):
    wf = w.float() * gamma.float()[None, :]
    w16 = wf.to(torch.float16).contiguous()
    c1 = w16.float().sum(1).contiguous()
    b = w.float() @ beta.float()
    if bias is not None:
        b = b + bias.float()
    return w16, b.to(torch.float16).contiguous(), c1


def gn_scratch_floats(M: int, rows_per_group: int, groups: int = 32) -> int:
    return (M // rows_per_group) * groups * 2 * 257


def groupnorm(x0: torch.Tensor, gamma, beta, stats: torch.Tensor, rows_per_group: int, *, x1=None, groups: int = 32,
              eps: float = 1e-5, silu: bool = False, out=None, shard=None):
    if shard is not None:
        return _groupnorm_sharded(x0, gamma, beta, stats, rows_per_group, x1, groups, eps, silu, out, shard)
    lib = _lib.load()
    _rowmajor(x0, "X0")
    assert x0.is_contiguous()
    M, C0 = x0.shape
    C1 = 0
    if x1 is not None:
        _rowmajor(x1, "X1")
        assert x1.is_contiguous() and x1.shape[0] == M
        C1 = x1.shape[1]
    if out is None:
        out = torch.empty((M, C0 + C1), dtype=torch.float16, device=x0.device)
    assert out.is_contiguous()
    need = gn_scratch_floats(M, rows_per_group, groups)
    assert stats.dtype == torch.float32 and stats.numel() >= need, "GroupNorm scratch too small"
    _lib.check(lib.anyv2v_groupnorm_f16(_p(x0), _p(x1), C0, C1, _p(out), _p(gamma), _p(beta), _p(stats), M,
                                        rows_per_group, groups, eps, int(silu), _stream()), "anyv2v_groupnorm_f16")
    return out


def _groupnorm_sharded(x0, gamma, beta, stats, rows_per_group, x1, groups, eps, silu, out, shard):
    lib = _lib.load()
    shards, all_reduce_sum = shard
    _rowmajor(x0, "X0")
    assert x0.is_contiguous()
    M, C0 = x0.shape
    C1 = 0
    if x1 is not None:
        _rowmajor(x1, "X1")
        assert x1.is_contiguous() and x1.shape[0] == M
        C1 = x1.shape[1]
    if out is None:
        out = torch.empty((M, C0 + C1), dtype=torch.float16, device=x0.device)
    assert out.is_contiguous()
    n = int(lib.anyv2v_groupnorm_partial_floats(M, rows_per_group, groups, C0 + C1))
    npiv = (M // rows_per_group) * groups
    assert n > 0 and stats.dtype == torch.float32 and stats.numel() >= n + npiv, "GroupNorm scratch too small"
    piv = stats[n:n + npiv]
    _lib.check(lib.anyv2v_groupnorm_pivot_f16(_p(x0), _p(x1), C0, C1, _p(piv), M, rows_per_group, groups, int(shards), _stream()),
               "anyv2v_groupnorm_pivot_f16")
    all_reduce_sum(piv)
    _lib.check(lib.anyv2v_groupnorm_partial_pivot_f16(_p(x0), _p(x1), C0, C1, _p(piv), _p(stats), M, rows_per_group, groups,
                                                      _stream()), "anyv2v_groupnorm_partial_pivot_f16")
    all_reduce_sum(stats[:n])
    _lib.check(lib.anyv2v_groupnorm_apply_pivot_f16(_p(x0), _p(x1), C0, C1, _p(out), _p(gamma), _p(beta), _p(piv), _p(stats), M,
                                                    rows_per_group, groups, eps, int(silu), int(shards), _stream()),
               "anyv2v_groupnorm_apply_pivot_f16")
    return out


def layernorm(x: torch.Tensor, gamma, beta, eps: float = 1e-5, out=None):
    lib = _lib.load()
    _rowmajor(x, "X")
    assert x.is_contiguous()
    M, Cc = x.shape
    if out is None:
        out = torch.empty_like(x)
    _lib.check(lib.anyv2v_layernorm_f16(_p(x), _p(out), _p(gamma), _p(beta), M, Cc, eps, _stream()), "anyv2v_layernorm_f16")
    return out


def softmax_rows(s: torch.Tensor, scale: float, out: Optional[torch.Tensor] = None):
    lib = _lib.load()
    assert s.dim() == 2 and s.stride(1) == 1 and s.dtype == torch.float32 and s.is_cuda
    rows, cols = s.shape
    if out is None:
        out = torch.empty((rows, cols), dtype=torch.float16, device=s.device)
    _rowmajor(out, "P")
    _lib.check(lib.anyv2v_softmax_rows_f32_f16(_p(s), s.stride(0), _p(out), out.stride(0), rows, cols, float(scale), _stream()),
               "anyv2v_softmax_rows_f32_f16")
    return out


def attention(q, k, v, out, *, batch, heads, Sq, Sk, inner=1, q_strides, kv_strides, kv_div=1, qk_mod=0,
              scale=0.125, head_dim=64, naive=False, causal=False, bias=None):
    lib = _lib.load()
    for t, n in ((q, "Q"), (k, "K"), (v, "V"), (out, "O")):
        _rowmajor(t, n)
    d = AttnDesc()
    d.Q, d.K, d.V, d.O = _p(q), _p(k), _p(v), _p(out)
    d.ldq, d.ldk, d.ldv, d.ldo = q.stride(0), k.stride(0), v.stride(0), out.stride(0)
    d.batch, d.heads, d.Sq, d.Sk, d.inner = batch, heads, Sq, Sk, inner
    d.q_outer, d.q_inner, d.q_seq = q_strides
    d.kv_outer, d.kv_inner, d.kv_seq = kv_strides
    d.kv_div, d.qk_mod, d.scale = kv_div, qk_mod, scale
    d.flags = (1 if (naive or FORCE_NAIVE) else 0) | ATTN_FLAGS | (16 if causal else 0)
    if bias is not None:
        assert bias.dtype == torch.float32 and bias.is_contiguous() and tuple(bias.shape) == (heads, Sq, Sk) and bias.device == q.device
        _lib.check(lib.anyv2v_attention_bias_f16(C.byref(d), head_dim, _p(bias), _stream()), "anyv2v_attention_bias_f16")
    elif head_dim == 64 and not causal:
        _lib.check(lib.anyv2v_attention_f16(C.byref(d), _stream()), "anyv2v_attention_f16")
    else:
        _lib.check(lib.anyv2v_attention_small_f16(C.byref(d), head_dim, _stream()), "anyv2v_attention_small_f16")
    return out


def silu(x: torch.Tensor, out=None):
    lib = _lib.load()
    assert x.is_contiguous() and x.dtype == torch.float16
    if out is None:
        out = torch.empty_like(x)
    _lib.check(lib.anyv2v_silu_f16(_p(x), _p(out), x.numel(), _stream()), "anyv2v_silu_f16")
    return out


def add(a: torch.Tensor, b: torch.Tensor, out=None):
    lib = _lib.load()
    assert a.is_contiguous() and b.is_contiguous() and a.numel() == b.numel()
    if out is None:
        out = torch.empty_like(a)
    _lib.check(lib.anyv2v_add_f16(_p(a), _p(b), _p(out), a.numel(), _stream()), "anyv2v_add_f16")
    return out


def timestep_embedding(t_f32: torch.Tensor, dim: int, out=None):
    lib = _lib.load()
    assert t_f32.dtype == torch.float32 and t_f32.is_contiguous()
    B = t_f32.numel()
    if out is None:
        out = torch.empty((B, dim), dtype=torch.float16, device=t_f32.device)
    _lib.check(lib.anyv2v_timestep_embedding_f16(_p(t_f32), _p(out), B, dim, _stream()), "anyv2v_timestep_embedding_f16")
    return out


def ncfhw_to_tokens(x: torch.Tensor, out: torch.Tensor, col0: int = 0):
    lib = _lib.load()
    B, Cc, F, H, W = x.shape
    assert x.is_contiguous() and x.dtype == torch.float16
    _rowmajor(out, "Y")
    _lib.check(lib.anyv2v_ncfhw_to_tokens_f16(_p(x), _p(out), B, Cc, F, H * W, out.stride(0), col0, _stream()),
               "anyv2v_ncfhw_to_tokens_f16")
    return out


def tokens_to_ncfhw(x: torch.Tensor, B: int, Cc: int, F: int, H: int, W: int, col0: int = 0, out=None):
    lib = _lib.load()
    _rowmajor(x, "X")
    if out is None:
        out = torch.empty((B, Cc, F, H, W), dtype=torch.float16, device=x.device)
    _lib.check(lib.anyv2v_tokens_to_ncfhw_f16(_p(x), _p(out), B, Cc, F, H * W, x.stride(0), col0, _stream()),
               "anyv2v_tokens_to_ncfhw_f16")
    return out


def adaptive_avgpool(x: torch.Tensor, N: int, Hi: int, Wi: int, Ho: int, Wo: int, out=None):
    lib = _lib.load()
    _rowmajor(x, "X")
    assert x.is_contiguous()
    Cc = x.shape[1]
    if out is None:
        out = torch.empty((N * Ho * Wo, Cc), dtype=torch.float16, device=x.device)
    assert out.is_contiguous() and out.dtype == torch.float16 and tuple(out.shape) == (N * Ho * Wo, Cc)
    _lib.check(lib.anyv2v_adaptive_avgpool_f16(_p(x), _p(out), N, Hi, Wi, Ho, Wo, Cc, _stream()), "anyv2v_adaptive_avgpool_f16")
    return out


def copy_cols(x: torch.Tensor, xcol0: int, y: torch.Tensor, ycol0: int, ncols: int):
    lib = _lib.load()
    _rowmajor(x, "X")
    _rowmajor(y, "Y")
    assert x.shape[0] == y.shape[0]
    _lib.check(lib.anyv2v_copy_cols_f16(_p(x), x.stride(0), xcol0, _p(y), y.stride(0), ycol0, x.shape[0], ncols, _stream()),
               "anyv2v_copy_cols_f16")
    return y


def gather_rows(x: torch.Tensor, xcol0: int, idx: torch.Tensor, y: torch.Tensor, ycol0: int, ncols: int):
    lib = _lib.load()
    _rowmajor(x, "X")
    _rowmajor(y, "Y")
    assert idx.dtype == torch.int32 and idx.is_contiguous() and idx.numel() == y.shape[0] and idx.device == x.device
    _lib.check(lib.anyv2v_gather_rows_f16(_p(x), x.stride(0), xcol0, _p(idx), _p(y), y.stride(0), ycol0, y.shape[0], ncols,
                                          _stream()), "anyv2v_gather_rows_f16")
    return y


def freeu(hidden: torch.Tensor, skip: torch.Tensor, n_img: int, H: int, W: int, b: float, s: float, out=None):
    lib = _lib.load()
    _rowmajor(hidden, "hidden")
    _rowmajor(skip, "skip")
    rows = n_img * H * W
    assert hidden.shape[0] == rows and skip.shape[0] == rows, f"freeu: {tuple(hidden.shape)} / {tuple(skip.shape)} rows, expected {rows}"
    if out is None:
        out = (torch.empty((rows, hidden.shape[1]), dtype=torch.float16, device=hidden.device),
               torch.empty((rows, skip.shape[1]), dtype=torch.float16, device=skip.device))
    ho, so = out
    _rowmajor(ho, "hidden'")
    _rowmajor(so, "skip'")
    assert tuple(ho.shape) == tuple(hidden.shape) and tuple(so.shape) == tuple(skip.shape)
    _lib.check(lib.anyv2v_freeu_f16(_p(hidden), hidden.stride(0), _p(ho), ho.stride(0), hidden.shape[1], float(b),
                                    _p(skip), skip.stride(0), _p(so), so.stride(0), skip.shape[1], float(s), n_img, H, W, _stream()),
               "anyv2v_freeu_f16")
    return ho, so


def rotary(x: torch.Tensor, col0: int, rot_dim: int, rows_per_pos: int, n_pos: int, theta: float = 10000.0, windows: int = 1,
           window_stride: int = 0):
    lib = _lib.load()
    _rowmajor(x, "X")
    _lib.check(lib.anyv2v_rotary_f16(_p(x), x.stride(0), x.shape[0], col0, rot_dim, windows, window_stride, rows_per_pos, n_pos,
                                     float(theta), _stream()), "anyv2v_rotary_f16")
    return x


def cfg_ddim_step(vtok: torch.Tensor, b_unc: int, b_cond: int, guidance: float, coef: torch.Tensor,
                  lat: torch.Tensor, out: torch.Tensor):
    lib = _lib.load()
    _rowmajor(vtok, "V")
    assert lat.is_contiguous() and out.is_contiguous() and lat.dtype == torch.float16 and lat.shape[0] == 1
    assert coef.dtype == torch.float32 and coef.numel() >= 4
    _, Cc, F, H, W = lat.shape
    _lib.check(lib.anyv2v_cfg_ddim_step_f16(_p(vtok), vtok.stride(0), b_unc, b_cond, float(guidance), _p(coef), _p(lat),
                                            _p(out), Cc, F, H * W, _stream()), "anyv2v_cfg_ddim_step_f16")
    return out


def ddim_step(v: torch.Tensor, x: torch.Tensor, sa_t: float, sb_t: float, sa_p: float, sb_p: float, out=None):
    lib = _lib.load()
    v = v.to(torch.float16).contiguous()
    x = x.to(torch.float16).contiguous()
    if out is None:
        out = torch.empty_like(x)
    _lib.check(lib.anyv2v_ddim_step_f16(_p(v), _p(x), _p(out), sa_t, sb_t, sa_p, sb_p, x.numel(), _stream()),
               "anyv2v_ddim_step_f16")
    return out


PRED_V, PRED_EPSILON, PRED_SAMPLE = 0, 1, 2


def guided_step(e: torch.Tensor, x: torch.Tensor, coef, *, b_txt: int, b_unc: int = -1, b_img: int = -1, g_txt: float = 1.0,
                g_img: float = 1.0, prediction: int = PRED_V, out=None, noise=None, sigma: float = 0.0):
    lib = _lib.load()
    assert e.is_contiguous() and x.is_contiguous() and e.dtype == x.dtype == torch.float16
    n = x.numel()
    assert e.numel() % n == 0 and max(b_txt, b_unc, b_img) < e.numel() // n
    if out is None:
        out = torch.empty_like(x)
    sa_t, sb_t, sa_p, sb_p = (float(c) for c in coef)
    if noise is not None or sigma != 0.0:
        assert noise is None or (noise.is_contiguous() and noise.dtype == torch.float16 and noise.numel() == n)
        _lib.check(lib.anyv2v_guided_step_noise_f16(_p(e), n, b_unc, b_img, b_txt, float(g_img), float(g_txt), int(prediction), sa_t, sb_t,
                                                    sa_p, sb_p, _p(x), _p(out), _p(noise), float(sigma), _stream()),
                   "anyv2v_guided_step_noise_f16")
        return out
    _lib.check(lib.anyv2v_guided_step_f16(_p(e), n, b_unc, b_img, b_txt, float(g_img), float(g_txt), int(prediction), sa_t, sb_t, sa_p,
                                          sb_p, _p(x), _p(out), _stream()), "anyv2v_guided_step_f16")
    return out


_HINT = [1, 1]


def set_batch_hint(num: int, den: int):
    _lib.check(_lib.load().anyv2v_set_batch_hint(int(num), int(den)), "anyv2v_set_batch_hint")
    _HINT[:] = [int(num), int(den)]


class batch_hint:

    def __init__(self, num: int, den: int):
        self.num, self.den = int(num), int(den)

    def __enter__(self):
        _lib.check(_lib.load().anyv2v_set_batch_hint(self.num, self.den), "anyv2v_set_batch_hint")
        _HINT[:] = [self.num, self.den]
        return self

    def __exit__(self, *exc):
        _lib.check(_lib.load().anyv2v_set_batch_hint(1, 1), "anyv2v_set_batch_hint")
        _HINT[:] = [1, 1]
        return False


def selftest(scratch: torch.Tensor):
    lib = _lib.load()
    assert scratch.dtype == torch.uint8 and scratch.is_contiguous()
    _lib.check(lib.anyv2v_selftest(_p(scratch), scratch.numel(), _stream()), "anyv2v_selftest")
```

anyv2v_amd/unet.py:

```python
from __future__ import annotations

import copy
import math
import os

from dataclasses import dataclass
from typing import List, Optional, Tuple

import torch
import torch.nn as nn

from . import ops
from .ops import ACT_GEGLU, ACT_GELU, ACT_NONE, ACT_SILU, MODE_CONV2D, MODE_TEMPORAL


@dataclass
class I2VGenXLUNetConfig:
    in_channels: int = 4
    out_channels: int = 4
    block_out_channels: Tuple[int, ...] = (320, 640, 1280, 1280)
    layers_per_block: int = 2
    norm_num_groups: int = 32
    cross_attention_dim: int = 1024
    attention_head_dim: int = 64
    transformer_in_heads: int = 8
    sample_size: int = 32
    down_block_types: Tuple[str, ...] = ("CrossAttnDownBlock3D",) * 3 + ("DownBlock3D",)
    up_block_types: Tuple[str, ...] = ("UpBlock3D",) + ("CrossAttnUpBlock3D",) * 3

    @property
    def time_embed_dim(self) -> int:
        return self.block_out_channels[0] * 4

    @staticmethod
    def from_json(path: str) -> "I2VGenXLUNetConfig":
        import json
        with open(path) as f:
            d = json.load(f)
        kw = {}
        for k in ("in_channels", "out_channels", "layers_per_block", "norm_num_groups", "cross_attention_dim", "sample_size"):
            if d.get(k) is not None:
                kw[k] = int(d[k])
        for k in ("block_out_channels", "down_block_types", "up_block_types"):
            if d.get(k) is not None:
                kw[k] = tuple(d[k])
        if d.get("attention_head_dim") is not None:
            ahd = d["attention_head_dim"]
            kw["attention_head_dim"] = int(ahd[0] if isinstance(ahd, (list, tuple)) else ahd)
        if d.get("transformer_in_heads") is not None:
            kw["transformer_in_heads"] = int(d["transformer_in_heads"])
        return I2VGenXLUNetConfig(**kw)

    @staticmethod
    def mini() -> "I2VGenXLUNetConfig":
        return I2VGenXLUNetConfig(block_out_channels=(64, 128, 256, 256), cross_attention_dim=128,
                                  transformer_in_heads=2, sample_size=8)


def _param(*shape):
    return nn.Parameter(torch.empty(*shape, dtype=torch.float16), requires_grad=False)


def pnp_on(t, schedule) -> bool:
    if schedule is None or t is None:
        return False
    t = int(t)
    if t == 1000:
        return True
    if isinstance(schedule, (set, frozenset)):
        return t in schedule
    return t in {int(s) for s in schedule}


class Linear(nn.Module):
    def __init__(self, cin, cout, bias=True):
        super().__init__()
        self.in_features, self.out_features = cin, cout
        self.weight = _param(cout, cin)
        self.bias = _param(cout) if bias else None

    def forward(self, x, *unused):
        shp = x.shape
        y = ops.gemm(x.reshape(-1, shp[-1]).contiguous(), self.weight, bias=self.bias)
        return y.reshape(*shp[:-1], self.out_features)


class Conv2d(nn.Module):
    def __init__(self, cin, cout, k, stride=1, padding=0, pad_cin_to: Optional[int] = None):
        super().__init__()
        self.cin, self.cout, self.k, self.stride = cin, cout, k, stride
        self.weight = _param(cout, cin, k, k)
        self.bias = _param(cout)
        self.pad_cin_to = pad_cin_to
        self._w = None

    def pack(self):
        w = self.weight.data
        if self.pad_cin_to and self.pad_cin_to > self.cin:
            wp = torch.zeros(self.cout, self.pad_cin_to, self.k, self.k, dtype=w.dtype, device=w.device)
            wp[:, : self.cin] = w
            w = wp
        self._w = w.permute(0, 2, 3, 1).reshape(self.cout, -1).contiguous()

    def forward(self, x, *unused):
        if self._w is None:
            self.pack()
        n, c, H, W = x.shape
        tok = x.to(torch.float16).permute(0, 2, 3, 1).reshape(n * H * W, c).contiguous()
        if self.pad_cin_to and self.pad_cin_to > c:
            tok = torch.nn.functional.pad(tok, (0, self.pad_cin_to - c))
        y = self.tokens(tok, H, W)
        Ho, Wo = (H, W) if self.k == 1 else ((H + 2 - 3) // self.stride + 1, (W + 2 - 3) // self.stride + 1)
        return y.view(n, Ho, Wo, self.cout).permute(0, 3, 1, 2)

    def tokens(self, x, H, W, *, x1=None, up=False, act=ACT_NONE, rowvec=None, rowvec_div=0, residual=None, out=None,
               asym=False, gn=None, _launch=None):
        if _launch is not None:
            launch, kw = _launch, {}
        else:
            launch, kw = ops.gemm, ({"out": out} if gn is None else {"out": out, "gn": gn})
        if self.k == 1:
            return launch(x, self._w, a1=x1, bias=self.bias, act=act, residual=residual, **kw)
        if up:
            Ho, Wo = 2 * H, 2 * W
        elif asym:
            Ho, Wo = (H + 1 - 3) // self.stride + 1, (W + 1 - 3) // self.stride + 1
        else:
            Ho, Wo = (H + 2 - 3) // self.stride + 1, (W + 2 - 3) // self.stride + 1
        n_img = x.shape[0] // (H * W)
        return launch(x, self._w, a1=x1, bias=self.bias, act=act, rowvec=rowvec, rowvec_div=rowvec_div,
                      residual=residual, mode=MODE_CONV2D, conv=(H, W, Ho, Wo, self.stride, int(up), int(asym)),
                      M=n_img * Ho * Wo, **kw)

    def tokens_gn_floats(self, x, H, W, rows_per_group, groups, **kw):
        return self.tokens(x, H, W, _launch=lambda *a, **k: ops.gemm_gn_stats_floats(*a, rows_per_group=rows_per_group, groups=groups, **k),
                           **kw)


def _gn_records(ctx, M, rows_per_group, groups):
    if not ops.GN_EPILOGUE or getattr(ctx, "fp", None) is not None:
        return None
    need = ops.gn_stats_floats(M, rows_per_group, groups)
    if need == 0:
        return None
    rec = getattr(ctx, "gn_rec", None)
    if rec is None or rec.numel() < need:
        assert not torch.cuda.is_current_stream_capturing(), "GroupNorm record buffer must exist before a graph capture"
        rec = ctx.gn_rec = torch.empty(need, dtype=torch.float32, device="cuda")
    return rec


class Conv3dTemporal(nn.Module):

    def __init__(self, cin, cout):
        super().__init__()
        self.weight = _param(cout, cin, 3, 1, 1)
        self.bias = _param(cout)
        self._w = None

    def pack(self):
        w = self.weight.data[:, :, :, 0, 0]
        self._w = w.permute(0, 2, 1).reshape(w.shape[0], -1).contiguous()


class GroupNorm(nn.Module):
    def __init__(self, groups, channels, eps=1e-5):
        super().__init__()
        self.num_groups, self.eps = groups, eps
        self.weight = _param(channels)
        self.bias = _param(channels)

    def forward(self, x):
        n, c = x.shape[:2]
        hw = x[0, 0].numel()
        tok = x.to(torch.float16).reshape(n, c, hw).permute(0, 2, 1).reshape(n * hw, c).contiguous()
        stats = torch.empty(ops.gn_scratch_floats(n, 1, self.num_groups), dtype=torch.float32, device=x.device)
        y = ops.groupnorm(tok, self.weight, self.bias, stats, hw, groups=self.num_groups, eps=self.eps)
        return y.view(n, hw, c).permute(0, 2, 1).reshape(x.shape)


class LayerNorm(nn.Module):
    def __init__(self, channels, eps=1e-5):
        super().__init__()
        self.eps = eps
        self.weight = _param(channels)
        self.bias = _param(channels)


class SiLU(nn.Module):
    def forward(self, x):
        return ops.silu(x.contiguous())


class Identity(nn.Module):
    def forward(self, x, *a, **k):
        return x


def expand_shared(x, full_ctx):
    Bs = full_ctx.B - 1
    n = x.shape[0] // Bs
    out = torch.empty(((Bs + 1) * n, x.shape[1]), dtype=x.dtype, device=x.device)
    out[:Bs * n].copy_(x)
    out[Bs * n:].copy_(x[(Bs - 1) * n:])
    return out


class Geom:

    def __init__(self, kind: str, B: int, F: int, HW: int):
        self.kind, self.B, self.F, self.HW = kind, B, F, HW
        if kind == "spatial":
            self.batch, self.S, self.inner = B * F, HW, 1
            self.strides = (HW, 0, 1)
        else:
            self.batch, self.S, self.inner = B * HW, F, HW
            self.strides = (F * HW, 1, HW)


class HipAttnProcessor:

    def __init__(self, injection_schedule=None):
        self.injection_schedule = injection_schedule
        self.t = None
        self.src_io = None

    def run(self, attn: "Attention", ctx, h, geom: Geom, residual, kv=None, ln_in=None):
        Cq = attn.inner_dim
        if ln_in is not None:
            h, (w_in, b_in, c1_in), ln_eps = ln_in

            def proj(rows, lo=0, out=None):
                return ops.gemm(rows, w_in[lo:], bias=b_in[lo:], ln=(c1_in[lo:], ln_eps), out=out)
        else:
            def proj(rows, lo=0, out=None):
                return ops.gemm(rows, (attn._w_qkv if kv is None else attn.to_q.weight)[lo:], out=out)
        T = h.shape[0]
        o = torch.empty((T, Cq), dtype=torch.float16, device=h.device)
        if kv is None:
            inject = pnp_on(self.t, self.injection_schedule)
            io = self.src_io if inject else None
            if io is not None and io[0] == "replay":
                src_qk = io[1]
                assert src_qk.shape[0] * 2 == T and src_qk.shape[1] == 2 * Cq
                qkv = torch.empty((T, 3 * Cq), dtype=torch.float16, device=h.device)
                proj(h, 2 * Cq, qkv[:, 2 * Cq:])
                ops.attention(src_qk[:, :Cq], src_qk[:, Cq:], qkv[:, 2 * Cq:], o, batch=geom.batch, heads=attn.heads, Sq=geom.S,
                              Sk=geom.S, inner=geom.inner, q_strides=geom.strides, kv_strides=geom.strides,
                              qk_mod=geom.batch // 2, scale=attn.scale)
                return ops.gemm(o, attn.to_out[0].weight, bias=attn.to_out[0].bias, residual=residual)
            if inject and T % 3 == 0 and _V_ONLY:
                Ts = T // 3
                qkv = torch.empty((T, 3 * Cq), dtype=torch.float16, device=h.device)
                proj(h[:Ts], 0, qkv[:Ts])
                proj(h[Ts:], 2 * Cq, qkv[Ts:, 2 * Cq:])
            else:
                qkv = proj(h)
            if io is not None and io[0] == "record":
                io[1].copy_(qkv[:T // 3, :2 * Cq])
            qk_mod = geom.batch // 3 if inject else 0
            ops.attention(qkv[:, :Cq], qkv[:, Cq:2 * Cq], qkv[:, 2 * Cq:], o, batch=geom.batch, heads=attn.heads,
                          Sq=geom.S, Sk=geom.S, inner=geom.inner, q_strides=geom.strides, kv_strides=geom.strides,
                          qk_mod=qk_mod, scale=attn.scale)
        else:
            q = proj(h)
            k_, v_, Sk = kv
            ops.attention(q, k_, v_, o, batch=geom.batch, heads=attn.heads, Sq=geom.S, Sk=Sk, inner=1,
                          q_strides=geom.strides, kv_strides=(Sk, 0, 1), kv_div=geom.F, scale=attn.scale)
        return ops.gemm(o, attn.to_out[0].weight, bias=attn.to_out[0].bias, residual=residual)


class Attention(nn.Module):
    def __init__(self, query_dim, cross_attention_dim=None, heads=8, dim_head=64):
        super().__init__()
        self.inner_dim = heads * dim_head
        self.heads, self.dim_head = heads, dim_head
        self.scale = dim_head ** -0.5
        self.is_cross = cross_attention_dim is not None
        ctx_dim = cross_attention_dim if cross_attention_dim is not None else query_dim
        self.to_q = Linear(query_dim, self.inner_dim, bias=False)
        self.to_k = Linear(ctx_dim, self.inner_dim, bias=False)
        self.to_v = Linear(ctx_dim, self.inner_dim, bias=False)
        self.to_out = nn.ModuleList([Linear(self.inner_dim, query_dim, bias=True), Identity()])
        self.spatial_norm = None
        self.group_norm = None
        self.norm_cross = None
        self.residual_connection = False
        self.rescale_output_factor = 1.0
        self.processor = HipAttnProcessor()
        self._w_qkv = None
        self._w_kv = None

    def pack(self):
        if self.is_cross:
            self._w_kv = torch.cat([self.to_k.weight.data, self.to_v.weight.data], 0).contiguous()
        else:
            self._w_qkv = torch.cat([self.to_q.weight.data, self.to_k.weight.data, self.to_v.weight.data], 0).contiguous()

    def prepare_attention_mask(self, attention_mask, target_length, batch_size, out_dim=3):
        return attention_mask

    def run(self, ctx, h, geom: Geom, residual, kv=None, ln_in=None):
        proc = self.processor
        if isinstance(proc, HipAttnProcessor):
            return proc.run(self, ctx, h, geom, residual, kv, ln_in)
        assert ln_in is None, "a foreign processor takes the normalised hidden states"
        return self._run_foreign(proc, ctx, h, geom, residual, kv)

    def _run_foreign(self, proc, ctx, h, geom: Geom, residual, kv):
        C = h.shape[1]
        if geom.kind == "spatial":
            hs = h.view(geom.batch, geom.S, C)
        else:
            hs = h.view(geom.B, geom.F, geom.HW, C).permute(0, 2, 1, 3).reshape(geom.batch, geom.S, C)
        ehs = None
        if kv is not None:
            ehs = ctx.context.view(ctx.B, ctx.Sk, -1).repeat_interleave(geom.F, dim=0)
        out = proc(self, hs, encoder_hidden_states=ehs)
        if geom.kind != "spatial":
            out = out.view(geom.B, geom.HW, geom.F, C).permute(0, 2, 1, 3)
        out = out.reshape(-1, C).contiguous()
        return ops.add(out, residual)


class GEGLU(nn.Module):
    def __init__(self, dim_in, dim_out):
        super().__init__()
        self.proj = Linear(dim_in, dim_out * 2)
        self.dim_out = dim_out
        self._w = self._b = None

    def pack(self):
        w, b = self.proj.weight.data, self.proj.bias.data
        n = self.dim_out
        assert n % 16 == 0
        wh, wg = w[:n].view(n // 16, 16, -1), w[n:].view(n // 16, 16, -1)
        self._w = torch.stack([wh, wg], 1).reshape(2 * n, -1).contiguous()
        bh, bg = b[:n].view(n // 16, 16), b[n:].view(n // 16, 16)
        self._b = torch.stack([bh, bg], 1).reshape(2 * n).contiguous()


class GELUProj(nn.Module):
    def __init__(self, dim_in, dim_out):
        super().__init__()
        self.proj = Linear(dim_in, dim_out)


class FeedForward(nn.Module):
    def __init__(self, dim, inner_dim=None, activation_fn="geglu"):
        super().__init__()
        inner_dim = inner_dim or dim * 4
        self.geglu = activation_fn == "geglu"
        act = GEGLU(dim, inner_dim) if self.geglu else GELUProj(dim, inner_dim)
        self.net = nn.ModuleList([act, Identity(), Linear(inner_dim, dim)])

    def pack(self):
        lin = self.net[2]
        self._w2s = ops.ff_pack_w2(lin.weight.data) if (self.geglu and tuple(lin.weight.shape) == (320, 1280)) else None

    def run(self, h, residual, ln_in=None):
        w2s = getattr(self, "_w2s", None)
        if ln_in is None and w2s is not None and ops.ff_fused_supported(h.shape[0], h.shape[1], w2s.shape[0] * 32):
            return ops.ff_geglu(h, self.net[0]._w, self.net[0]._b, w2s, self.net[2].bias, residual=residual)
        if ln_in is not None:
            x, (w_in, b_in, c1_in), ln_eps = ln_in
            g = ops.gemm(x, w_in, bias=b_in, act=ACT_GEGLU, ln=(c1_in, ln_eps))
        elif self.geglu:
            g = ops.gemm(h, self.net[0]._w, bias=self.net[0]._b, act=ACT_GEGLU)
        else:
            g = ops.gemm(h, self.net[0].proj.weight, bias=self.net[0].proj.bias, act=ACT_GELU)
        return ops.gemm(g, self.net[2].weight, bias=self.net[2].bias, residual=residual)


class BasicTransformerBlock(nn.Module):
    def __init__(self, dim, heads, dim_head, cross_attention_dim=None, double_self_attention=False):
        super().__init__()
        self.norm1 = LayerNorm(dim)
        self.attn1 = Attention(dim, None, heads, dim_head)
        self.norm2 = LayerNorm(dim)
        self.attn2 = Attention(dim, None if double_self_attention else cross_attention_dim, heads, dim_head)
        self.norm3 = LayerNorm(dim)
        self.ff = FeedForward(dim)

    def pack(self):
        self._ln = {}
        dim = self.norm1.weight.shape[0]
        if dim not in (320, 512) or _NO_LN_FOLD:
            return
        cat = lambda a: torch.cat([a.to_q.weight.data, a.to_k.weight.data, a.to_v.weight.data], 0)
        if dim == 320:
            self._ln["attn1"] = ops.ln_fold(cat(self.attn1), None, self.norm1.weight.data, self.norm1.bias.data)
            w2 = self.attn2.to_q.weight.data if self.attn2.is_cross else cat(self.attn2)
            self._ln["attn2"] = ops.ln_fold(w2, None, self.norm2.weight.data, self.norm2.bias.data)
        if self.ff.geglu and _LN_FOLD_FF:
            g = self.ff.net[0]
            w, b, c1 = ops.ln_fold(g.proj.weight.data, g.proj.bias.data, self.norm3.weight.data, self.norm3.bias.data)
            n = g.dim_out
            il = lambda t: torch.stack([t[:n].reshape(n // 16, 16, *t.shape[1:]), t[n:].reshape(n // 16, 16, *t.shape[1:])], 1) \
                .reshape(2 * n, *t.shape[1:]).contiguous()
            self._ln["ff"] = (il(w), il(b), il(c1))

    def _fold(self, name, proc_ok, M, N, act=ACT_NONE, per_branch=False):
        f = getattr(self, "_ln", {}).get(name)
        return f if (f is not None and proc_ok and ops.ln_gemm_supported(M, self.norm1.weight.shape[0], N, act, hinted=not per_branch)) else None

    def run(self, ctx, x, geom: Geom, expand=None, shrink=None):
        dim = x.shape[1]
        rows_b = lambda t, g: t.shape[0] // g.B
        f = self._fold("attn1", isinstance(self.attn1.processor, HipAttnProcessor), rows_b(x, geom), 3 * dim, per_branch=True)
        if f is not None:
            x = self.attn1.run(ctx, None, geom, residual=x, ln_in=(x, f, self.norm1.eps))
        else:
            h = ops.layernorm(x, self.norm1.weight, self.norm1.bias, self.norm1.eps)
            x = self.attn1.run(ctx, h, geom, residual=x)
        if expand is not None:
            after = getattr(ctx, "batch_hint_after", None)
            ctx, geom = expand
            x = expand_shared(x, ctx)
            if after is not None:
                ops.set_batch_hint(*after)
        if shrink is not None:
            x = x[x.shape[0] // 3:]
            geom = shrink
            ops.set_batch_hint(3, 2)
        kv = ctx.kv_for(self.attn2) if self.attn2.is_cross else None
        f = self._fold("attn2", isinstance(self.attn2.processor, HipAttnProcessor), rows_b(x, geom), dim if self.attn2.is_cross else 3 * dim,
                       per_branch=True)
        if f is not None:
            x = self.attn2.run(ctx, None, geom, residual=x, kv=kv, ln_in=(x, f, self.norm2.eps))
        else:
            h = ops.layernorm(x, self.norm2.weight, self.norm2.bias, self.norm2.eps)
            x = self.attn2.run(ctx, h, geom, residual=x, kv=kv)
        f = self._fold("ff", True, x.shape[0], 8 * dim, ACT_GEGLU)
        if f is not None:
            return self.ff.run(None, residual=x, ln_in=(x, f, self.norm3.eps))
        h = ops.layernorm(x, self.norm3.weight, self.norm3.bias, self.norm3.eps)
        return self.ff.run(h, residual=x)


class Transformer2DModel(nn.Module):
    def __init__(self, heads, dim_head, in_channels, cross_attention_dim, groups):
        super().__init__()
        inner = heads * dim_head
        self.norm = GroupNorm(groups, in_channels, eps=1e-6)
        self.proj_in = Linear(in_channels, inner)
        self.transformer_blocks = nn.ModuleList([BasicTransformerBlock(inner, heads, dim_head, cross_attention_dim)])
        self.proj_out = Linear(inner, in_channels)

    def run(self, ctx, x, H, W, full_ctx=None):
        HW = H * W
        h = ops.groupnorm(x, self.norm.weight, self.norm.bias, ctx.stats, HW, groups=self.norm.num_groups,
                          eps=self.norm.eps)
        h = ops.gemm(h, self.proj_in.weight, bias=self.proj_in.bias)
        geom = Geom("spatial", ctx.B, ctx.F, HW)
        for i, blk in enumerate(self.transformer_blocks):
            if full_ctx is not None and i == 0:
                h = blk.run(ctx, h, geom, expand=(full_ctx, Geom("spatial", full_ctx.B, full_ctx.F, HW)))
                ctx, geom = full_ctx, Geom("spatial", full_ctx.B, full_ctx.F, HW)
                x = expand_shared(x, full_ctx)
            else:
                h = blk.run(ctx, h, geom)
        return ops.gemm(h, self.proj_out.weight, bias=self.proj_out.bias, residual=x)


class TransformerTemporalModel(nn.Module):
    def __init__(self, heads, dim_head, in_channels, groups):
        super().__init__()
        inner = heads * dim_head
        self.norm = GroupNorm(groups, in_channels, eps=1e-6)
        self.proj_in = Linear(in_channels, inner)
        self.transformer_blocks = nn.ModuleList(
            [BasicTransformerBlock(inner, heads, dim_head, None, double_self_attention=True)])
        self.proj_out = Linear(inner, in_channels)

    def run(self, ctx, x, H, W):
        fp = getattr(ctx, "fp", None)
        return self._run(ctx, x, H * W, None) if fp is None else fp.temporal(ctx, x, H * W, self._run)

    def _run(self, ctx, x, HW, shard):
        h = ops.groupnorm(x, self.norm.weight, self.norm.bias, ctx.stats, ctx.F * HW, groups=self.norm.num_groups,
                          eps=self.norm.eps, shard=shard)
        h = ops.gemm(h, self.proj_in.weight, bias=self.proj_in.bias)
        geom = Geom("temporal", ctx.B, ctx.F, HW)
        drop = shard is None and getattr(ctx, "drop_tail_at", None) is self and not self.transformer_blocks[0].attn2.is_cross
        for i, blk in enumerate(self.transformer_blocks):
            if drop and i == 0:
                h = blk.run(ctx, h, geom, shrink=Geom("temporal", ctx.B - 1, ctx.F, HW))
                geom = Geom("temporal", ctx.B - 1, ctx.F, HW)
                x = x[x.shape[0] // 3:]
            else:
                h = blk.run(ctx, h, geom)
        return ops.gemm(h, self.proj_out.weight, bias=self.proj_out.bias, residual=x)


class Upsample2D(nn.Module):
    def __init__(self, channels):
        super().__init__()
        self.conv = Conv2d(channels, channels, 3, padding=1)


class Downsample2D(nn.Module):
    def __init__(self, channels):
        super().__init__()
        self.conv = Conv2d(channels, channels, 3, stride=2, padding=1)


class ResnetBlock2D(nn.Module):

    def __init__(self, in_channels, out_channels, temb_channels, groups, eps=1e-5):
        super().__init__()
        self.in_channels, self.out_channels = in_channels, out_channels
        self.norm1 = GroupNorm(groups, in_channels, eps)
        self.conv1 = Conv2d(in_channels, out_channels, 3, padding=1)
        self.time_emb_proj = Linear(temb_channels, out_channels)
        self.norm2 = GroupNorm(groups, out_channels, eps)
        self.dropout = Identity()
        self.conv2 = Conv2d(out_channels, out_channels, 3, padding=1)
        self.nonlinearity = SiLU()
        self.upsample = self.downsample = None
        self.conv_shortcut = Conv2d(in_channels, out_channels, 1) if in_channels != out_channels else None
        self.skip_time_act = False
        self.time_embedding_norm = "default"
        self.output_scale_factor = 1.0
        self.t = None
        self.injection_schedule = None
        self.src_io = None
        self._temb_col = 0
        self.norm_over_frames = False

    def forward(self, input_tensor, temb, scale: float = 1.0):
        n, c, H, W = input_tensor.shape
        h = self.nonlinearity(self.norm1(input_tensor))
        h = self.conv1(h) + self.time_emb_proj(self.nonlinearity(temb.to(torch.float16)))[:, :, None, None]
        h = self.conv2(self.nonlinearity(self.norm2(h)))
        if self.conv_shortcut is not None:
            input_tensor = self.conv_shortcut(input_tensor)
        return (input_tensor.to(torch.float16) + h) / self.output_scale_factor

    def _run_foreign(self, ctx, x0, x1, H, W):
        N = x0.shape[0] // (H * W)
        x = x0 if x1 is None else torch.cat([x0, x1], 1)
        x = x.view(N, H, W, -1).permute(0, 3, 1, 2)
        per = N // ctx.emb.shape[0]
        temb = ctx.emb.repeat_interleave(per, dim=0)
        out = self.__dict__["forward"](x, temb)
        return out.to(torch.float16).permute(0, 2, 3, 1).reshape(N * H * W, -1).contiguous()

    def run(self, ctx, x0, x1, H, W):
        if "forward" in self.__dict__:
            return self._run_foreign(ctx, x0, x1, H, W)
        HW = H * W
        T = x0.shape[0]
        inject = pnp_on(self.t, self.injection_schedule)
        io = self.src_io if inject else None
        if io is not None and io[0] == "replay":
            res = self.conv_shortcut.tokens(x0, H, W, x1=x1) if self.conv_shortcut is not None else x0
            hs, Th = io[1], T // 2
            assert hs.shape[0] == Th
            out = torch.empty((T, self.out_channels), dtype=torch.float16, device=x0.device)
            for b in range(2):
                ops.add(res[b * Th:(b + 1) * Th], hs, out=out[b * Th:(b + 1) * Th])
            return out
        Ts = T // 3 if inject else T
        a0 = x0[:Ts]
        a1 = x1[:Ts] if x1 is not None else None
        g = self.norm1.num_groups
        rpg = ctx.F * HW if self.norm_over_frames else HW
        h = ops.groupnorm(a0, self.norm1.weight, self.norm1.bias, ctx.stats, rpg, x1=a1, groups=g, eps=self.norm1.eps,
                          silu=True)
        tv = ctx.temb_all[:, self._temb_col:self._temb_col + self.out_channels]
        rec = _gn_records(ctx, Ts, rpg, g)
        if rec is not None and self.conv1.tokens_gn_floats(h, H, W, rpg, g, rowvec=tv, rowvec_div=ctx.F * HW) > 0:
            h = self.conv1.tokens(h, H, W, rowvec=tv, rowvec_div=ctx.F * HW, gn=(rec, rpg, g))
            h = ops.groupnorm_from_stats(h, self.norm2.weight, self.norm2.bias, rec, rpg, groups=g, eps=self.norm2.eps, silu=True)
        else:
            h = self.conv1.tokens(h, H, W, rowvec=tv, rowvec_div=ctx.F * HW)
            h = ops.groupnorm(h, self.norm2.weight, self.norm2.bias, ctx.stats, rpg, groups=g, eps=self.norm2.eps, silu=True)
        if self.conv_shortcut is not None:
            res = self.conv_shortcut.tokens(x0, H, W, x1=x1)
        else:
            res = x0
        if not inject:
            return self.conv2.tokens(h, H, W, residual=res)
        hs = self.conv2.tokens(h, H, W)
        if io is not None and io[0] == "record":
            io[1].copy_(hs)
        out = torch.empty((T, self.out_channels), dtype=torch.float16, device=x0.device)
        for b in range(3):
            ops.add(res[b * Ts:(b + 1) * Ts], hs, out=out[b * Ts:(b + 1) * Ts])
        return out


class TemporalConvLayer(nn.Module):
    def __init__(self, dim, groups):
        super().__init__()
        self.conv1 = nn.Sequential(GroupNorm(groups, dim), SiLU(), Conv3dTemporal(dim, dim))
        self.conv2 = nn.Sequential(GroupNorm(groups, dim), SiLU(), Identity(), Conv3dTemporal(dim, dim))
        self.conv3 = nn.Sequential(GroupNorm(groups, dim), SiLU(), Identity(), Conv3dTemporal(dim, dim))
        self.conv4 = nn.Sequential(GroupNorm(groups, dim), SiLU(), Identity(), Conv3dTemporal(dim, dim))

    def run(self, ctx, x, H, W):
        fp = getattr(ctx, "fp", None)
        return self._run(ctx, x, H * W, None) if fp is None else fp.temporal(ctx, x, H * W, self._run)

    def _run(self, ctx, x, HW, shard):
        h = x
        seqs = (self.conv1, self.conv2, self.conv3, self.conv4)
        rpg = ctx.F * HW
        rec = None
        for i, seq in enumerate(seqs):
            gn, conv = seq[0], seq[-1]
            if rec is not None:
                h = ops.groupnorm_from_stats(h, gn.weight, gn.bias, rec, rpg, groups=gn.num_groups, eps=gn.eps, silu=True)
            else:
                h = ops.groupnorm(h, gn.weight, gn.bias, ctx.stats, rpg, groups=gn.num_groups, eps=gn.eps, silu=True,
                                  shard=shard)
            rec = None
            if i < 3 and shard is None:
                g_next = seqs[i + 1][0].num_groups
                rec = _gn_records(ctx, h.shape[0], rpg, g_next)
                if rec is not None and ops.gemm_gn_stats_floats(h, conv._w, bias=conv.bias, mode=MODE_TEMPORAL, temporal=(ctx.F, HW),
                                                                rows_per_group=rpg, groups=g_next) == 0:
                    rec = None
            if rec is not None:
                h = ops.gemm(h, conv._w, bias=conv.bias, mode=MODE_TEMPORAL, temporal=(ctx.F, HW), gn=(rec, rpg, g_next))
            else:
                h = ops.gemm(h, conv._w, bias=conv.bias, mode=MODE_TEMPORAL, temporal=(ctx.F, HW),
                             residual=x if i == 3 else None)
        return h


class DownBlock3D(nn.Module):
    def __init__(self, cfg, cin, cout, cross_attn, add_downsample):
        super().__init__()
        g, temb = cfg.norm_num_groups, cfg.time_embed_dim
        self.has_cross_attention = cross_attn
        self.resnets, self.temp_convs = nn.ModuleList(), nn.ModuleList()
        if cross_attn:
            self.attentions, self.temp_attentions = nn.ModuleList(), nn.ModuleList()
        for i in range(cfg.layers_per_block):
            self.resnets.append(ResnetBlock2D(cin if i == 0 else cout, cout, temb, g))
            self.temp_convs.append(TemporalConvLayer(cout, g))
            if cross_attn:
                heads = cout // cfg.attention_head_dim
                self.attentions.append(Transformer2DModel(heads, cfg.attention_head_dim, cout, cfg.cross_attention_dim, g))
                self.temp_attentions.append(TransformerTemporalModel(heads, cfg.attention_head_dim, cout, g))
        self.downsamplers = nn.ModuleList([Downsample2D(cout)]) if add_downsample else None

    def run(self, ctx, x, H, W, stem_ctx=None):
        outs = []
        for i in range(len(self.resnets)):
            c = stem_ctx if (stem_ctx is not None and i == 0) else ctx
            x = self.resnets[i].run(c, x, None, H, W)
            x = self.temp_convs[i].run(c, x, H, W)
            if self.has_cross_attention:
                x = self.attentions[i].run(c, x, H, W, full_ctx=ctx if c is not ctx else None)
                x = self.temp_attentions[i].run(ctx, x, H, W)
            outs.append(x)
        if self.downsamplers is not None:
            x = self.downsamplers[0].conv.tokens(x, H, W)
            H, W = (H - 1) // 2 + 1, (W - 1) // 2 + 1
            outs.append(x)
        return x, outs, H, W


class MidBlock3D(nn.Module):
    def __init__(self, cfg, c):
        super().__init__()
        g, temb = cfg.norm_num_groups, cfg.time_embed_dim
        heads = c // cfg.attention_head_dim
        self.resnets = nn.ModuleList([ResnetBlock2D(c, c, temb, g), ResnetBlock2D(c, c, temb, g)])
        self.temp_convs = nn.ModuleList([TemporalConvLayer(c, g), TemporalConvLayer(c, g)])
        self.attentions = nn.ModuleList([Transformer2DModel(heads, cfg.attention_head_dim, c, cfg.cross_attention_dim, g)])
        self.temp_attentions = nn.ModuleList([TransformerTemporalModel(heads, cfg.attention_head_dim, c, g)])

    def run(self, ctx, x, H, W):
        x = self.resnets[0].run(ctx, x, None, H, W)
        x = self.temp_convs[0].run(ctx, x, H, W)
        x = self.attentions[0].run(ctx, x, H, W)
        x = self.temp_attentions[0].run(ctx, x, H, W)
        x = self.resnets[1].run(ctx, x, None, H, W)
        x = self.temp_convs[1].run(ctx, x, H, W)
        return x


class UpBlock3D(nn.Module):
    def __init__(self, cfg, cin, cout, prev_out, cross_attn, add_upsample):
        super().__init__()
        g, temb = cfg.norm_num_groups, cfg.time_embed_dim
        n = cfg.layers_per_block + 1
        self.has_cross_attention = cross_attn
        self.resnets, self.temp_convs = nn.ModuleList(), nn.ModuleList()
        if cross_attn:
            self.attentions, self.temp_attentions = nn.ModuleList(), nn.ModuleList()
        for i in range(n):
            res_skip = cin if i == n - 1 else cout
            res_in = prev_out if i == 0 else cout
            self.resnets.append(ResnetBlock2D(res_in + res_skip, cout, temb, g))
            self.temp_convs.append(TemporalConvLayer(cout, g))
            if cross_attn:
                heads = cout // cfg.attention_head_dim
                self.attentions.append(Transformer2DModel(heads, cfg.attention_head_dim, cout, cfg.cross_attention_dim, g))
                self.temp_attentions.append(TransformerTemporalModel(heads, cfg.attention_head_dim, cout, g))
        self.upsamplers = nn.ModuleList([Upsample2D(cout)]) if add_upsample else None
        self.freeu = None

    def run(self, ctx, x, skips: List[torch.Tensor], H, W, out_hw=None):
        for i in range(len(self.resnets)):
            skip = skips.pop()
            if self.freeu is not None:
                x, skip = ops.freeu(x, skip, x.shape[0] // (H * W), H, W, *self.freeu)
            x = self.resnets[i].run(ctx, x, skip, H, W)
            x = self.temp_convs[i].run(ctx, x, H, W)
            if self.has_cross_attention:
                x = self.attentions[i].run(ctx, x, H, W)
                x = self.temp_attentions[i].run(ctx, x, H, W)
        if self.upsamplers is not None:
            x, H, W = upsample_tokens(self.upsamplers[0].conv, x, H, W, out_hw)
        return x, H, W


def upsample_tokens(conv, x, H, W, out_hw=None):
    if out_hw is None or tuple(out_hw) == (2 * H, 2 * W):
        return conv.tokens(x, H, W, up=True), 2 * H, 2 * W
    Ho, Wo = out_hw
    if Ho not in (2 * H - 1, 2 * H) or Wo not in (2 * W - 1, 2 * W):
        raise ValueError(f"upsample {H} x {W} -> {Ho} x {Wo}: not the size of a skip connection of this UNet")
    n_img = x.shape[0] // (H * W)
    up = torch.empty((n_img * Ho * Wo, x.shape[1]), dtype=x.dtype, device=x.device)
    ops.gather_rows(x, 0, _nearest_rows(n_img, H, W, Ho, Wo, x.device), up, 0, x.shape[1])
    return conv.tokens(up, Ho, Wo), Ho, Wo


_NEAREST_ROWS = {}


def _nearest_rows(n_img, H, W, Ho, Wo, device):
    key = (n_img, H, W, Ho, Wo, str(device))
    idx = _NEAREST_ROWS.get(key)
    if idx is None:
        yi = (torch.arange(Ho) * H) // Ho
        xi = (torch.arange(Wo) * W) // Wo
        one = (yi[:, None] * W + xi[None, :]).reshape(-1)
        idx = (torch.arange(n_img)[:, None] * (H * W) + one[None, :]).reshape(-1).to(device=device, dtype=torch.int32).contiguous()
        if idx.is_cuda:
            torch.cuda.current_stream(idx.device).synchronize()
        _NEAREST_ROWS[key] = idx
    return idx


class I2VGenXLTransformerTemporalEncoder(nn.Module):
    def __init__(self, dim, heads, dim_head, ff_inner):
        super().__init__()
        self.norm1 = LayerNorm(dim)
        self.attn1 = Attention(dim, None, heads, dim_head)
        self.ff = FeedForward(dim, ff_inner, activation_fn="gelu")


class _Ctx:

    def __init__(self):
        self.key = None
        self.kv_slices = {}

    def kv_for(self, attn):
        c0, C = self.kv_slices[id(attn)]
        return self.kv_all[:, c0:c0 + C], self.kv_all[:, c0 + C:c0 + 2 * C], self.Sk


class _ConfigView:
    def __init__(self, cfg):
        self.in_channels = cfg.in_channels
        self.sample_size = cfg.sample_size
        self.cross_attention_dim = cfg.cross_attention_dim


_V_ONLY = os.environ.get("ANYV2V_VONLY", "1") == "1"
_NO_LN_FOLD = os.environ.get("ANYV2V_LN_FOLD", "1") != "1"
_LN_FOLD_FF = os.environ.get("ANYV2V_LN_FOLD_FF", "0") == "1"
PAD_CIN = 64


class I2VGenXLUNet(nn.Module):
    def __init__(self, cfg: Optional[I2VGenXLUNetConfig] = None):
        super().__init__()
        cfg = cfg or I2VGenXLUNetConfig()
        self.cfg = cfg
        self.config = _ConfigView(cfg)
        boc, g, ic, ted = cfg.block_out_channels, cfg.norm_num_groups, cfg.in_channels, cfg.time_embed_dim
        hd = cfg.attention_head_dim
        self.conv_in = Conv2d(2 * ic, boc[0], 3, padding=1, pad_cin_to=PAD_CIN)
        self.transformer_in = TransformerTemporalModel(cfg.transformer_in_heads, hd, boc[0], g)
        self.image_latents_proj_in = nn.Sequential(Conv2d(4, ic * 4, 3, padding=1), SiLU(),
                                                   Conv2d(ic * 4, ic * 4, 3, padding=1), SiLU(),
                                                   Conv2d(ic * 4, ic, 3, padding=1))
        self.image_latents_temporal_encoder = I2VGenXLTransformerTemporalEncoder(ic, 2, ic, ic * 4)
        self.image_latents_context_embedding = nn.Sequential(
            Conv2d(4, ic * 8, 3, padding=1), SiLU(), Identity(),
            Conv2d(ic * 8, ic * 16, 3, stride=2, padding=1), SiLU(),
            Conv2d(ic * 16, cfg.cross_attention_dim, 3, stride=2, padding=1))
        self.time_embedding = nn.ModuleDict(dict(linear_1=Linear(boc[0], ted), linear_2=Linear(ted, ted)))
        self.context_embedding = nn.Sequential(Linear(cfg.cross_attention_dim, ted), SiLU(),
                                               Linear(ted, cfg.cross_attention_dim * ic))
        self.fps_embedding = nn.Sequential(Linear(boc[0], ted), SiLU(), Linear(ted, ted))
        self.down_blocks = nn.ModuleList()
        out = boc[0]
        for i, typ in enumerate(cfg.down_block_types):
            cin, out = out, boc[i]
            self.down_blocks.append(DownBlock3D(cfg, cin, out, typ.startswith("CrossAttn"), i != len(boc) - 1))
        self.mid_block = MidBlock3D(cfg, boc[-1])
        self.up_blocks = nn.ModuleList()
        rev = list(reversed(boc))
        out = rev[0]
        for i, typ in enumerate(cfg.up_block_types):
            prev_out, out = out, rev[i]
            cin = rev[min(i + 1, len(boc) - 1)]
            self.up_blocks.append(UpBlock3D(cfg, cin, out, prev_out, typ.startswith("CrossAttn"), i != len(boc) - 1))
        self.conv_norm_out = GroupNorm(g, boc[0], eps=1e-5)
        self.conv_act = SiLU()
        self.conv_out = Conv2d(boc[0], cfg.out_channels, 3, padding=1)
        self._packed = False
        self._pack_gen = 0
        self._ctx = _Ctx()
        self.frame_parallel = None

    def set_frame_parallel(self, fp):
        if fp is not None and self.freeu is not None:
            raise NotImplementedError("FreeU is enabled: frame-parallel clips do not support it (disable_freeu() first)")
        self.frame_parallel = fp
        self._ctx = _Ctx()

    def enable_freeu(self, s1, s2, b1, b2):
        vals = tuple(float(v) for v in (s1, s2, b1, b2))
        if not all(math.isfinite(v) for v in vals):
            raise ValueError(f"enable_freeu: s1, s2, b1, b2 = {vals} must be finite")
        if self.frame_parallel is not None:
            raise NotImplementedError("enable_freeu: not supported on a frame-parallel clip (set_frame_parallel(None) first)")
        self.up_blocks[0].freeu = (vals[2], vals[0])
        self.up_blocks[1].freeu = (vals[3], vals[1])

    def disable_freeu(self):
        for blk in self.up_blocks:
            blk.freeu = None

    @property
    def freeu(self):
        f0, f1 = self.up_blocks[0].freeu, self.up_blocks[1].freeu
        return None if f0 is None or f1 is None else (f0[1], f1[1], f0[0], f1[0])

    @property
    def dtype(self):
        return self.conv_in.weight.dtype

    @property
    def device(self):
        return self.conv_in.weight.device

    def load_state_dict(self, sd, strict=True, **kw):
        r = super().load_state_dict({k: v.to(torch.float16) for k, v in sd.items()}, strict=strict, **kw)
        self._packed = False
        return r

    def _apply(self, fn, *a, **k):
        r = super()._apply(fn, *a, **k)
        self._packed = False
        return r

    def pack(self):
        for m in self.modules():
            if m is not self and hasattr(m, "pack"):
                m.pack()
        resnets = [m for m in self.modules() if isinstance(m, ResnetBlock2D)]
        col = 0
        ws, bs = [], []
        for r in resnets:
            r._temb_col = col
            col += r.out_channels
            ws.append(r.time_emb_proj.weight.data)
            bs.append(r.time_emb_proj.bias.data)
        self._w_temb_all = torch.cat(ws, 0).contiguous()
        self._b_temb_all = torch.cat(bs, 0).contiguous()
        cross = [m for m in self.modules() if isinstance(m, Attention) and m.is_cross]
        self._cross = cross
        self._w_kv_all = torch.cat([m._w_kv for m in cross], 0).contiguous()
        self._ctx = _Ctx()
        self._packed = True
        self._pack_gen += 1

    def _prepare_clip(self, B, F, H, W, ehs, fps, image_latents, image_embeddings):
        cfg = self.cfg
        dev = ehs.device
        key = (B, F, H, W, ehs.data_ptr(), ehs._version, image_latents.data_ptr(), image_latents._version,
               image_embeddings.data_ptr(), image_embeddings._version, fps.data_ptr(), fps._version)
        ctx = self._ctx
        if ctx.key == key:
            return ctx
        ctx = _Ctx()
        ctx.B, ctx.F, ctx.H, ctx.W = B, F, H, W
        ctx.fp = fp = self.frame_parallel
        if fp is not None:
            fp.check(F, H, W, len(cfg.block_out_channels))
        HW = H * W
        T = B * F * HW
        ctx.stats = torch.empty(ops.gn_scratch_floats(B * F, 1, cfg.norm_num_groups), dtype=torch.float32, device=dev)
        if ops.GN_EPILOGUE and fp is None:
            g = cfg.norm_num_groups
            need = max(ops.gn_stats_floats(T, HW, g), ops.gn_stats_floats(T, F * HW, g))
            ctx.gn_rec = torch.empty(need, dtype=torch.float32, device=dev) if need > 0 else None
        ctx.t_buf = torch.zeros(B, dtype=torch.float32, device=dev)
        boc0, cd = cfg.block_out_channels[0], cfg.cross_attention_dim
        fe = ops.timestep_embedding(fps.reshape(-1).to(torch.float32).expand(B).contiguous(), boc0)
        fe = ops.gemm(fe, self.fps_embedding[0].weight, bias=self.fps_embedding[0].bias, act=ACT_SILU)
        ctx.fps_emb = ops.gemm(fe, self.fps_embedding[2].weight, bias=self.fps_embedding[2].bias)
        il0 = torch.empty((B * HW, 4), dtype=torch.float16, device=dev)
        ops.ncfhw_to_tokens(image_latents[:, :, :1].to(torch.float16).contiguous(), il0)
        ce = self.image_latents_context_embedding
        c = ce[0].tokens(il0, H, W, act=ACT_SILU)
        c = ops.adaptive_avgpool(c, B, H, W, 32, 32)
        c = ce[3].tokens(c, 32, 32, act=ACT_SILU)
        c = ce[5].tokens(c, 16, 16)
        ie = image_embeddings.reshape(B, cd).to(torch.float16).contiguous()
        e = ops.gemm(ie, self.context_embedding[0].weight, bias=self.context_embedding[0].bias, act=ACT_SILU)
        e = ops.gemm(e, self.context_embedding[2].weight, bias=self.context_embedding[2].bias)
        n_txt = ehs.shape[1]
        n_il = c.shape[0] // B
        Sk = n_txt + n_il + cfg.in_channels
        ctx.Sk = Sk
        context = torch.empty((B * Sk, cd), dtype=torch.float16, device=dev)
        ehs16 = ehs.to(torch.float16).contiguous()
        for b in range(B):
            r0 = b * Sk
            ops.copy_cols(ehs16[b], 0, context[r0:r0 + n_txt], 0, cd)
            ops.copy_cols(c[b * n_il:(b + 1) * n_il], 0, context[r0 + n_txt:r0 + n_txt + n_il], 0, cd)
            ops.copy_cols(e[b].view(cfg.in_channels, cd), 0, context[r0 + n_txt + n_il:r0 + Sk], 0, cd)
        ctx.context = context
        ctx.kv_all = ops.gemm(context, self._w_kv_all)
        col = 0
        for m in self._cross:
            ctx.kv_slices[id(m)] = (col, m.inner_dim)
            col += 2 * m.inner_dim
        il = torch.empty((T, 4), dtype=torch.float16, device=dev)
        ops.ncfhw_to_tokens(image_latents.to(torch.float16).contiguous(), il)
        pi = self.image_latents_proj_in
        h = pi[0].tokens(il, H, W, act=ACT_SILU)
        h = pi[2].tokens(h, H, W, act=ACT_SILU)
        h = pi[4].tokens(h, H, W)
        enc = self.image_latents_temporal_encoder
        a = enc.attn1
        n = ops.layernorm(h, enc.norm1.weight, enc.norm1.bias, enc.norm1.eps)
        qkv = ops.gemm(n, a._w_qkv)
        Cq = a.inner_dim
        o = torch.empty((T, Cq), dtype=torch.float16, device=dev)
        geom = Geom("temporal", B, F, HW)
        ops.attention(qkv[:, :Cq], qkv[:, Cq:2 * Cq], qkv[:, 2 * Cq:], o, batch=geom.batch, heads=a.heads, Sq=F, Sk=F,
                      inner=geom.inner, q_strides=geom.strides, kv_strides=geom.strides, scale=a.scale,
                      head_dim=a.dim_head)
        h = ops.gemm(o, a.to_out[0].weight, bias=a.to_out[0].bias, residual=h)
        h = enc.ff.run(h, residual=h)
        if fp is not None:
            f0, f1 = fp.frames(F)
            h = h.view(B, F, HW, -1)[:, f0:f1].reshape(B * (f1 - f0) * HW, -1).contiguous()
            ctx.F, T = f1 - f0, B * (f1 - f0) * HW
        ctx.xin = torch.zeros((T, PAD_CIN), dtype=torch.float16, device=dev)
        ops.copy_cols(h, 0, ctx.xin, cfg.in_channels, cfg.in_channels)
        ctx.key = key
        ctx._keepalive = (ehs, image_latents, image_embeddings, fps)
        ctx.shared_stem = False
        ctx.stem_ctx = copy.copy(ctx)
        ctx.stem_ctx.B = max(B - 1, 1)
        self._ctx = ctx
        return ctx

    def forward_tokens(self, sample, timestep, fps, image_latents, image_embeddings, encoder_hidden_states):
        if not self._packed:
            self.pack()
        B, C, F, H, W = sample.shape
        ctx = self._prepare_clip(B, F, H, W, encoder_hidden_states, fps, image_latents, image_embeddings)
        if torch.is_tensor(timestep):
            ctx.t_buf.copy_(timestep.reshape(-1).to(torch.float32).expand(B), non_blocking=True)
        else:
            ctx.t_buf.fill_(float(timestep))
        return self._forward_core(ctx, sample)

    def _forward_core(self, ctx, sample, drop_source_tail=False):
        cfg = self.cfg
        B, C, F, H, W = sample.shape
        fp = ctx.fp
        if fp is not None:
            f0, f1 = fp.frames(F)
            sample, F = sample[:, :, f0:f1].contiguous(), f1 - f0
        te = ops.timestep_embedding(ctx.t_buf, cfg.block_out_channels[0])
        te = ops.gemm(te, self.time_embedding["linear_1"].weight, bias=self.time_embedding["linear_1"].bias, act=ACT_SILU)
        emb = ops.gemm(te, self.time_embedding["linear_2"].weight, bias=self.time_embedding["linear_2"].bias,
                       residual=ctx.fps_emb)
        ctx.temb_all = ops.gemm(ops.silu(emb), self._w_temb_all, bias=self._b_temb_all)
        ctx.stem_ctx.temb_all = ctx.temb_all
        ctx.emb = emb
        ctx.stem_ctx.emb = emb[:ctx.stem_ctx.B]
        stem = ctx.stem_ctx if (getattr(ctx, "shared_stem", False) and B >= 2 and self.down_blocks[0].has_cross_attention) else None
        hint = getattr(ctx, "batch_hint", None)
        ctx.stem_ctx.batch_hint_after = None
        if hint is not None:
            ctx.stem_ctx.batch_hint_after = hint if stem is not None else None
            ops.set_batch_hint(*((hint[0] - 1, hint[1] - 1) if stem is not None else hint))
        if stem is not None:
            T2 = (B - 1) * F * H * W
            ops.ncfhw_to_tokens(sample[:B - 1], ctx.xin[:T2], col0=0)
            x = self.conv_in.tokens(ctx.xin[:T2], H, W)
            x = self.transformer_in.run(stem, x, H, W)
            skips = [expand_shared(x, ctx)]
        else:
            ops.ncfhw_to_tokens(sample, ctx.xin, col0=0)
            x = self.conv_in.tokens(ctx.xin, H, W)
            x = self.transformer_in.run(ctx, x, H, W)
            skips = [x]
        h_, w_ = H, W
        sizes = [(H, W)]
        for bi, blk in enumerate(self.down_blocks):
            x, outs, h_, w_ = blk.run(ctx, x, h_, w_, stem_ctx=stem if bi == 0 else None)
            skips.extend(outs)
            if blk.downsamplers is not None:
                sizes.append((h_, w_))
        x = self.mid_block.run(ctx, x, h_, w_)
        last = self.up_blocks[-1].temp_attentions[-1] if getattr(self.up_blocks[-1], "has_cross_attention", False) else None
        drop = bool(drop_source_tail and B == 3 and fp is None and hint is None and last is not None)
        ctx.drop_tail_at = last if drop else None
        try:
            for blk in self.up_blocks:
                sizes.pop()
                x, h_, w_ = blk.run(ctx, x, skips, h_, w_, out_hw=sizes[-1] if sizes else None)
            ctx.drop_tail_at = None
            x = ops.groupnorm(x, self.conv_norm_out.weight, self.conv_norm_out.bias, ctx.stats, H * W,
                              groups=self.conv_norm_out.num_groups, eps=self.conv_norm_out.eps, silu=True)
            vtok = torch.empty((x.shape[0], 8), dtype=torch.float16, device=x.device)
            self.conv_out.tokens(x, H, W, out=vtok)
            if fp is not None:
                vtok = fp.gather_frames(vtok, B, F, H * W)
        finally:
            ctx.drop_tail_at = None
            if drop:
                ops.set_batch_hint(1, 1)
        return vtok

    def forward(self, sample, timestep, fps=None, image_latents=None, image_embeddings=None,
                encoder_hidden_states=None, cross_attention_kwargs=None, return_dict=False):
        B, C, F, H, W = sample.shape
        vtok = self.forward_tokens(sample.to(torch.float16).contiguous(), timestep, fps, image_latents, image_embeddings,
                                   encoder_hidden_states)
        out = ops.tokens_to_ncfhw(vtok, B, self.cfg.out_channels, F, H, W)
        return (out,)
```

include/anyv2v_hip.h:

```cpp
#ifndef ANYV2V_HIP_H
#define ANYV2V_HIP_H

#include <stdint.h>

#ifdef __cplusplus
extern "C" {
#endif

#define ANYV2V_OK 0
#define ANYV2V_EINVAL (-1)
#define ANYV2V_EUNSUPPORTED (-2)

#define ANYV2V_GEMM_NAIVE (1 << 0)
#define ANYV2V_GEMM_LDS_DMA (1 << 1)
#define ANYV2V_GEMM_NO_BIG (1 << 2)
#define ANYV2V_GEMM_FORCE_BIG (1 << 3)
#define ANYV2V_GEMM_NO_SPLITK (1 << 4)
#define ANYV2V_GEMM_PROBE_TRACE (1 << 5)
#define ANYV2V_GEMM_PROBE_KO_SHIFT 6
#define ANYV2V_GEMM_NO_WS (1 << 9)
#define ANYV2V_GEMM_FORCE_WS (1 << 10)
#define ANYV2V_GEMM_NF4 (1 << 11)
#define ANYV2V_GEMM_NF5 (1 << 12)
#define ANYV2V_GEMM_RASTER_SHIFT 13
#define ANYV2V_GEMM_RASTER_NFAST (1 << 16)
#define ANYV2V_GEMM_PP (1 << 17)
#define ANYV2V_GEMM_NO_PP (1 << 18)
#define ANYV2V_GEMM_PP_192 (1 << 19)
#define ANYV2V_GEMM_PP_256 (1 << 20)
#define ANYV2V_GEMM_SW (1 << 21)
#define ANYV2V_GEMM_NO_SW (1 << 22)
#define ANYV2V_GEMM_PROBE_SW_KO_SHIFT 23
#define ANYV2V_GEMM_STREAMK (1 << 26)
#define ANYV2V_GEMM_FORCE_STREAMK (1 << 27)
#define ANYV2V_GEMM_SWH (1 << 28)
#define ANYV2V_GEMM_PROBE_KORDER_SHIFT 29
typedef struct AnyV2VGemmDesc {
    const void* A0;
    const void* A1;
    const void* W;
    void* C;
    const void* bias;
    const void* rowvec;
    const void* R;
    int32_t M, N;
    int32_t C0, C1;
    int32_t lda0, lda1, ldc, ldr, ldrv, rowvec_div;
    int32_t mode;
    int32_t Hi, Wi, Ho, Wo, stride, up;
    int32_t asym;
    int32_t F, HW;
    int32_t act;
    int32_t flags;
    void* workspace;
    int64_t workspace_bytes;
    const float* ln_c1;
    float ln_eps;
    int32_t reserved0;
    float* gn_stats;
    int64_t gn_stats_floats;
    int32_t gn_rows_per_group;
    int32_t gn_groups;
} AnyV2VGemmDesc;

int anyv2v_gemm_f16(const AnyV2VGemmDesc* d, void* stream);
int64_t anyv2v_gemm_gn_stats_floats(const AnyV2VGemmDesc* d);
int64_t anyv2v_gemm_gn_launches(int32_t reset);

typedef struct AnyV2VFFDesc {
    const void* X;
    const void* W1;
    const void* b1;
    const void* W2;
    const void* b2;
    const void* R;
    void* Y;
    int32_t M, C, H;
    int32_t ldx, ldr, ldy;
    int32_t flags;
    int32_t reserved0;
} AnyV2VFFDesc;

int anyv2v_ff_geglu_f16(const AnyV2VFFDesc* d, void* stream);

int64_t anyv2v_groupnorm_scratch_floats(int32_t M, int32_t rows_per_group, int32_t G);
int anyv2v_groupnorm_f16(const void* X0, const void* X1, int32_t C0, int32_t C1, void* Y, const void* gamma,
                         const void* beta, float* stats, int32_t M, int32_t rows_per_group, int32_t G, float eps,
                         int32_t silu, void* stream);
int64_t anyv2v_groupnorm_stats_floats(int32_t M, int32_t rows_per_group, int32_t G);
int anyv2v_groupnorm_apply_stats_f16(const void* X, void* Y, const void* gamma, const void* beta, float* stats,
                                     const int32_t* sizes, float eps, int32_t silu, void* stream);

int64_t anyv2v_groupnorm_partial_floats(int32_t M, int32_t rows_per_group, int32_t G, int32_t C);
int anyv2v_groupnorm_pivot_f16(const void* X0, const void* X1, int32_t C0, int32_t C1, float* pivot, int32_t M,
                               int32_t rows_per_group, int32_t G, int32_t shards, void* stream);
int anyv2v_groupnorm_partial_pivot_f16(const void* X0, const void* X1, int32_t C0, int32_t C1, const float* pivot,
                                       float* stats, int32_t M, int32_t rows_per_group, int32_t G, void* stream);
int anyv2v_groupnorm_apply_pivot_f16(const void* X0, const void* X1, int32_t C0, int32_t C1, void* Y, const void* gamma,
                                     const void* beta, const float* pivot, const float* stats, int32_t M,
                                     int32_t rows_per_group, int32_t G, float eps, int32_t silu, int32_t shards, void* stream);
int anyv2v_groupnorm_partial_f16(const void* X0, const void* X1, int32_t C0, int32_t C1, float* stats, int32_t M,
                                 int32_t rows_per_group, int32_t G, void* stream);
int anyv2v_groupnorm_apply_f16(const void* X0, const void* X1, int32_t C0, int32_t C1, void* Y, const void* gamma,
                               const void* beta, const float* stats, int32_t M, int32_t rows_per_group, int32_t G,
                               float eps, int32_t silu, int32_t shards, void* stream);

int anyv2v_layernorm_f16(const void* X, void* Y, const void* gamma, const void* beta, int32_t M, int32_t C,
                         float eps, void* stream);

typedef struct AnyV2VAttnDesc {
    const void* Q;
    const void* K;
    const void* V;
    void* O;
    int32_t ldq, ldk, ldv, ldo;
    int32_t batch, heads, Sq, Sk;
    int32_t inner;
    int64_t q_outer, q_inner, q_seq;
    int64_t kv_outer, kv_inner, kv_seq;
    int32_t kv_div;
    int32_t qk_mod;
    float scale;
    int32_t flags;
} AnyV2VAttnDesc;

int anyv2v_attention_f16(const AnyV2VAttnDesc* d, void* stream);

int anyv2v_attention_small_f16(const AnyV2VAttnDesc* d, int32_t head_dim, void* stream);
int anyv2v_attention_bias_f16(const AnyV2VAttnDesc* d, int32_t head_dim, const float* bias, void* stream);

int anyv2v_silu_f16(const void* X, void* Y, int64_t n, void* stream);
int anyv2v_add_f16(const void* A, const void* B, void* Y, int64_t n, void* stream);
int anyv2v_timestep_embedding_f16(const float* t, void* out, int32_t B, int32_t dim, void* stream);
int anyv2v_ncfhw_to_tokens_f16(const void* X, void* Y, int32_t B, int32_t C, int32_t F, int32_t HW, int32_t ldy,
                               int32_t col0, void* stream);
int anyv2v_tokens_to_ncfhw_f16(const void* X, void* Y, int32_t B, int32_t C, int32_t F, int32_t HW, int32_t ldx,
                               int32_t col0, void* stream);
int anyv2v_adaptive_avgpool_f16(const void* X, void* Y, int32_t N, int32_t Hi, int32_t Wi, int32_t Ho, int32_t Wo,
                                int32_t C, void* stream);
int anyv2v_gather_rows_f16(const void* X, int32_t ldx, int32_t xcol0, const int32_t* idx, void* Y, int32_t ldy, int32_t ycol0,
                           int64_t M, int32_t C, void* stream);
int anyv2v_rotary_f16(void* X, int32_t ld, int64_t rows, int32_t col0, int32_t rot_dim, int32_t n_windows, int32_t window_stride,
                      int32_t rows_per_pos, int32_t n_pos, float theta, void* stream);
int anyv2v_copy_cols_f16(const void* X, int32_t ldx, int32_t xcol0, void* Y, int32_t ldy, int32_t ycol0, int64_t M,
                         int32_t C, void* stream);

int anyv2v_freeu_f16(const void* hidden, int32_t ld_hidden, void* hidden_out, int32_t ld_hidden_out, int32_t C_hidden, float b,
                     const void* skip, int32_t ld_skip, void* skip_out, int32_t ld_skip_out, int32_t C_skip, float s,
                     int32_t n_img, int32_t H, int32_t W, void* stream);

int anyv2v_softmax_rows_f32_f16(const float* S, int32_t lds, void* P, int32_t ldp, int32_t rows, int32_t cols, float scale,
                                void* stream);

int anyv2v_cfg_ddim_step_f16(const void* Vtok, int32_t ldv, int32_t b_unc, int32_t b_cond, float guidance,
                             const float* coef, const void* lat, void* out, int32_t C, int32_t F, int32_t HW,
                             void* stream);

int anyv2v_ddim_step_f16(const void* V, const void* X, void* Y, float sa_t, float sb_t, float sa_p, float sb_p,
                         int64_t n, void* stream);

int anyv2v_guided_step_f16(const void* E, int64_t n, int32_t b_unc, int32_t b_img, int32_t b_txt, float g_img, float g_txt,
                           int32_t prediction, float sa_t, float sb_t, float sa_p, float sb_p, const void* X, void* Y, void* stream);

int anyv2v_guided_step_noise_f16(const void* E, int64_t n, int32_t b_unc, int32_t b_img, int32_t b_txt, float g_img, float g_txt,
                                 int32_t prediction, float sa_t, float sb_t, float c_x0, float c_eps, const void* X, void* Y,
                                 const void* noise, float sigma, void* stream);

int anyv2v_set_batch_hint(int32_t num, int32_t den);
const char* anyv2v_last_error(void);
#define ANYV2V_ABI_VERSION 105
int anyv2v_version(void);
int anyv2v_selftest(void* scratch, int64_t scratch_bytes, void* stream);

#ifdef __cplusplus
}
#endif
#endif
```

Before: 3.034 frames/s.

## Emit LayerNorm row statistics from producer GEMMs and fold them into consumer GEMMs

Producer linear GEMMs (proj_in, attention out-projections) now write per-row partial sums and sums of squares from their epilogue. The next transformer-block GEMM with folded LayerNorm weights applies mean/rstd from those records inside its own epilogue. This removes the separate LayerNorm statistics pass over activations. In exchange it adds epilogue work, LDS parking space, extra kernel template variants, and bookkeeping to drop records wherever rows get gathered or sharded.

```diff
diff --git a/anyv2v_amd/_lib.py b/anyv2v_amd/_lib.py
--- a/anyv2v_amd/_lib.py
+++ b/anyv2v_amd/_lib.py
@@ -30,6 +30,13 @@
         ("ln_c1", C.c_void_p), ("ln_eps", C.c_float), ("reserved0", C.c_int32),
         ("gn_stats", C.c_void_p), ("gn_stats_floats", C.c_int64), ("gn_rows_per_group", C.c_int32), ("gn_groups", C.c_int32),
     ]
+
+class GemmLn(C.Structure):
+    _fields_ = [
+        ("rowstats", C.c_void_p), ("rowstats_floats", C.c_int64), ("ln_rowstats", C.c_void_p), ("ln_parts", C.c_int32),
+        ("reserved0", C.c_int32),
+    ]
+
 
 ANYV2V_GEMM_NAIVE = 1 << 0
 ANYV2V_GEMM_LDS_DMA = 1 << 1
@@ -82,6 +89,9 @@
     "anyv2v_gemm_f16": (C.c_int, [C.POINTER(GemmDesc), _VP]),
     "anyv2v_gemm_gn_stats_floats": (C.c_int64, [C.POINTER(GemmDesc)]),
     "anyv2v_gemm_gn_launches": (C.c_int64, [_I32]),
+    "anyv2v_gemm_ln_f16": (C.c_int, [C.POINTER(GemmDesc), C.POINTER(GemmLn), _VP]),
+    "anyv2v_gemm_rowstats_floats": (C.c_int64, [C.POINTER(GemmDesc)]),
+    "anyv2v_gemm_ln_launches": (None, [C.POINTER(C.c_int64), _I32]),
     "anyv2v_ff_geglu_f16": (C.c_int, [C.POINTER(FFDesc), _VP]),
     "anyv2v_groupnorm_f16": (C.c_int, [_VP, _VP, _I32, _I32, _VP, _VP, _VP, _VP, _I32, _I32, _I32, _F32, _I32, _VP]),
     "anyv2v_groupnorm_scratch_floats": (C.c_int64, [_I32, _I32, _I32]),
diff --git a/anyv2v_amd/csrc/gemm.hip b/anyv2v_amd/csrc/gemm.hip
--- a/anyv2v_amd/csrc/gemm.hip
+++ b/anyv2v_amd/csrc/gemm.hip
@@ -13,13 +13,20 @@
     return z;
 }
 
+static int64_t g_ln_launches[4] = {0, 0, 0, 0};
 static int64_t g_gn_launches = 0;
 
-extern "C" int anyv2v_gemm_f16(const AnyV2VGemmDesc* d, void* stream) {
+extern "C" int anyv2v_gemm_f16(const AnyV2VGemmDesc* d, void* stream) { return anyv2v_gemm_ln_f16(d, nullptr, stream); }
+
+extern "C" int anyv2v_gemm_ln_f16(const AnyV2VGemmDesc* d, const AnyV2VGemmLn* ln, void* stream) {
     AV_CHECK(d != nullptr, "gemm: null descriptor");
     AV_CHECK(d->A0 && d->W && d->C, "gemm: null A0/W/C");
     const int hinted = av_hint_rows(d->M);
-    const GemmPlan plan = av_gemm_plan(*d, hinted);
+    const GemmPlan plan = av_gemm_plan(*d, hinted, ln);
+    AV_CHECK(ln == nullptr || ln->rowstats == nullptr || plan.rows_decline == nullptr,
+             "gemm: rowstats set, but this launch is %s, which writes no LayerNorm row statistics (ask anyv2v_gemm_rowstats_floats first)",
+             plan.rows_decline);
+    AV_CHECK(ln == nullptr || ln->ln_rowstats == nullptr || d->ln_c1 != nullptr, "gemm: ln_rowstats needs ln_c1");
     AV_CHECK(d->gn_stats == nullptr || plan.gn_decline == nullptr,
              "gemm: gn_stats set, but this launch runs on %s, which writes no GroupNorm statistics (ask anyv2v_gemm_gn_stats_floats first)",
              plan.gn_decline);
@@ -44,6 +51,17 @@
     k.tilesN = plan.tilesN; k.vec_epi = plan.vec_epi; k.splits = plan.splits;
     if (plan.splits > 1 || plan.family == GEMM_SW_STREAMK) k.partial = (float*)d->workspace;
     if (plan.family == GEMM_WS_LN) k.ln_c1 = d->ln_c1, k.ln_eps = d->ln_eps;
+    if (plan.ln_epi == GEMM_EPI_LN_TILE) {
+        k.ln_c1 = d->ln_c1, k.ln_eps = d->ln_eps;
+        k.ln_rowstats = ln->ln_rowstats;
+        k.ln_parts = ln->ln_parts;
+    }
+    if (plan.ln_epi == GEMM_EPI_ROWSTATS) {
+        const long long need = (long long)2 * d->M * (d->N / 160);
+        AV_CHECK(ln->rowstats_floats >= need, "gemm: rowstats holds %lld floats, the launch writes %lld", (long long)ln->rowstats_floats, need);
+        AV_CHECK((((uintptr_t)ln->rowstats) & 7) == 0, "gemm: rowstats must be 8-byte aligned");
+        k.rowstats = ln->rowstats;
+    }
     k.rast_gm = plan.rast_gm; k.rast_gn = plan.rast_gn; k.rast_sm = plan.rast_sm; k.rast_sn = plan.rast_sn; k.rast_nfast = plan.rast_nfast;
     if (d->gn_stats != nullptr) {
         AV_CHECK(d->gn_stats_floats >= (int64_t)3 * (d->M / 16) * d->gn_groups, "gemm: gn_stats holds %lld floats, the launch writes %lld",
@@ -54,6 +72,7 @@
         k.gn_cg = d->N / d->gn_groups;
         ++g_gn_launches;
     }
+    if (plan.ln_epi != GEMM_EPI_PLAIN) ++g_ln_launches[(plan.ln_epi == GEMM_EPI_LN_TILE ? 2 : 0) + (plan.family == GEMM_BIG ? 1 : 0)];
     static const bool log_on = getenv("ANYV2V_GEMM_LOG") != nullptr;
     if (log_on)
         fprintf(stderr, "gemm-plan mode %d M %d (hinted %d) N %d K %d act %d res %d big %d splits %d kernel %s nf %d grid %d\n", d->mode, d->M,
@@ -79,6 +98,19 @@
     return plan.status == ANYV2V_OK && plan.gn_records ? (int64_t)3 * (d->M / 16) * d->gn_groups : 0;
 }
 
+extern "C" int64_t anyv2v_gemm_rowstats_floats(const AnyV2VGemmDesc* d) {
+    if (d == nullptr) return 0;
+    const GemmPlan plan = av_gemm_plan(*d, av_hint_rows(d->M));
+    return plan.status == ANYV2V_OK && plan.rows_records ? (int64_t)2 * d->M * (d->N / 160) : 0;
+}
+
+extern "C" void anyv2v_gemm_ln_launches(int64_t counts[4], int32_t reset) {
+    for (int i = 0; i < 4; ++i) {
+        counts[i] = g_ln_launches[i];
+        if (reset) g_ln_launches[i] = 0;
+    }
+}
+
 extern "C" int64_t anyv2v_gemm_gn_launches(int32_t reset) {
     const int64_t n = g_gn_launches;
     if (reset) g_gn_launches = 0;
diff --git a/anyv2v_amd/csrc/gemm_big.hip b/anyv2v_amd/csrc/gemm_big.hip
--- a/anyv2v_amd/csrc/gemm_big.hip
+++ b/anyv2v_amd/csrc/gemm_big.hip
@@ -52,15 +52,19 @@
 #undef AV_RB
 }
 
-template <int MF, bool GEGLU, int MODE, bool TRACE = false, bool SPLIT = false, bool RES = false, bool GN = false>
+template <int MF, bool GEGLU, int MODE, bool TRACE = false, bool SPLIT = false, bool RES = false, bool GN = false, bool ROWS = false,
+          bool LNT = false>
 __global__ __launch_bounds__(512) void gemm_big_kernel(const GemmK p) {
     static_assert(!(RES && (GEGLU || SPLIT)), "no residual on GEGLU / split-K launches");
     static_assert(!(GN && (GEGLU || SPLIT)), "no GroupNorm records on GEGLU / split-K launches");
+    static_assert(!(ROWS && (GEGLU || SPLIT || GN || LNT)), "row statistics: plain linear launches only");
+    static_assert(!(LNT && (SPLIT || RES || GN)), "the LayerNorm fold takes no residual and is never split");
     constexpr int BM = 64 * MF, BN = 320;
     constexpr int A_BYTES = BM * 128, B_BYTES = BN * 128, STAGE_BYTES = A_BYTES + B_BYTES;
     constexpr int SLAB_LD = (GEGLU ? 80 : 160) + 8;
     constexpr int SLAB_BYTES = 16 * SLAB_LD * 2;
-    static_assert(8 * SLAB_BYTES <= STAGE_BYTES, "epilogue slabs must fit in one pipeline stage");
+    constexpr int PARK_BYTES = ROWS ? 16 * ROWSTATS_PARK_LD * 4 : 0;
+    static_assert(8 * (SLAB_BYTES + PARK_BYTES) <= STAGE_BYTES, "epilogue slabs (and chunk sums) must fit in one pipeline stage");
     __shared__ __attribute__((aligned(16))) char smem[2 * STAGE_BYTES];
 
     const int tid = threadIdx.x, lane = tid & 63, w = tid >> 6, wr = w >> 1, wc = w & 1;
@@ -198,6 +202,28 @@
                     rr[mf][it] = *(const h8*)(p.R + (size_t)m * p.ldr + n_out_wave + cc * 8);
                 }
         }
+        if constexpr (LNT) {
+            int lane_l = lane;
+            asm volatile("" : "+v"(lane_l));
+            const float inv_k = 1.0f / (float)p.C0;
+            float ln_mean[MF], ln_rstd[MF];
+#pragma unroll
+            for (int mf = 0; mf < MF; ++mf) {
+                int m = m_wave + mf * 16 + (lane_l & 15);
+                m = m < p.M ? m : p.M - 1;
+                ln_row_moments(p.ln_rowstats + (size_t)m * p.ln_parts * 2, p.ln_parts, inv_k, p.ln_eps, ln_mean[mf], ln_rstd[mf]);
+            }
+#pragma unroll
+            for (int nf = 0; nf < 10; ++nf) {
+                const int n = n_wave + nf * 16 + 4 * (lane_l >> 4);
+                const f4 c1 = *(const f4*)(p.ln_c1 + n);
+                const h4 b = *(const h4*)(p.bias != nullptr ? p.bias + n : p.zeros);
+#pragma unroll
+                for (int mf = 0; mf < MF; ++mf)
+#pragma unroll
+                    for (int r = 0; r < 4; ++r) acc[mf][nf][r] = fmaf(fmaf(-ln_mean[mf], c1[r], acc[mf][nf][r]), ln_rstd[mf], (float)b[r]);
+            }
+        }
         asm volatile("s_waitcnt vmcnt(0)" ::: "memory");
         if constexpr (TRACE) if (tid == 0 && tile == b0 + AV_TRACE_TILE * G) p.trace[(size_t)blockIdx.x * 32 + 30] = (long long)__builtin_amdgcn_s_memtime();
         __builtin_amdgcn_s_barrier();
@@ -223,10 +249,11 @@
         }
         if constexpr (SPLIT) __builtin_unreachable();
         half_t* const slab = (half_t*)(smem + (stage ^ 1) * STAGE_BYTES + w * SLAB_BYTES);
+        float* const park = (float*)(smem + (stage ^ 1) * STAGE_BYTES + 8 * SLAB_BYTES + w * PARK_BYTES);
         h4 bvec[10];
 #pragma unroll
         for (int nf = 0; nf < 10; ++nf)
-            bvec[nf] = *(const h4*)(p.bias != nullptr ? p.bias + n_wave + nf * 16 + 4 * lq : p.zeros);
+            bvec[nf] = LNT ? (h4){0, 0, 0, 0} : *(const h4*)(p.bias != nullptr ? p.bias + n_wave + nf * 16 + 4 * lq : p.zeros);
         if constexpr (RES) {
 #pragma unroll
             for (int mf = 0; mf < MF; ++mf)
@@ -241,14 +268,14 @@
                     h4 o;
 #pragma unroll
                     for (int r = 0; r < 4; ++r) {
-                        const float hv = acc[mf][2 * np][r] + (float)bvec[2 * np][r];
-                        const float gv = acc[mf][2 * np + 1][r] + (float)bvec[2 * np + 1][r];
+                        const float hv = acc[mf][2 * np][r] + (LNT ? 0.f : (float)bvec[2 * np][r]);
+                        const float gv = acc[mf][2 * np + 1][r] + (LNT ? 0.f : (float)bvec[2 * np + 1][r]);
                         o[r] = (half_t)(hv * av_gelu(gv));
                     }
                     *(h4*)(slab + l15 * SLAB_LD + np * 16 + 4 * lq) = o;
                 }
             } else {
-                const bool has_rv = p.rowvec != nullptr;
+                const bool has_rv = !LNT && p.rowvec != nullptr;
                 const int mrow = m_wave + mf * 16 + l15;
                 const half_t* rv = has_rv ? p.rowvec + (size_t)((mrow < p.M ? mrow : 0) / p.rowvec_div) * p.ldrv + n_wave + 4 * lq
                                           : p.zeros;
@@ -258,7 +285,7 @@
                     if (has_rv) tv = *(const h4*)(rv + nf * 16);
                     h4 o;
 #pragma unroll
-                    for (int r = 0; r < 4; ++r) o[r] = (half_t)(acc[mf][nf][r] + (float)bvec[nf][r] + (float)tv[r]);
+                    for (int r = 0; r < 4; ++r) o[r] = (half_t)(acc[mf][nf][r] + (LNT ? 0.f : (float)bvec[nf][r]) + (float)tv[r]);
                     *(h4*)(slab + l15 * SLAB_LD + nf * 16 + 4 * lq) = o;
                 }
             }
@@ -273,6 +300,12 @@
                     if (ok) *(h8*)(slab + row * SLAB_LD + cc * 8) = v;
                 }
                 if (ok) *(h8*)(p.C + (size_t)(m_wave + mf * 16 + row) * p.ldc + n_out_wave + cc * 8) = v;
+                if constexpr (ROWS) rowstats_park_chunk(v, park + row * ROWSTATS_PARK_LD, cc);
+            }
+            if constexpr (ROWS) {
+                const int m = m_wave + mf * 16 + lane_e;
+                if (lane_e < 16 && m < p.M)
+                    rowstats_store_row(park + lane_e * ROWSTATS_PARK_LD, p.rowstats + ((size_t)m * (p.N / 160) + n_wave / 160) * 2);
             }
             if constexpr (GN) {
                 const int m0 = m_wave + mf * 16;
@@ -305,6 +338,18 @@
 #ifdef ANYV2V_EXPERIMENTS
 #include "../../tools/experiments/gemm_dispatch_big_probe.inc"
 #endif
+    if constexpr (MODE == MODE_LINEAR) {
+        if (k.rowstats != nullptr) {
+            if (res) AV_GO((gemm_big_kernel<3, false, MODE_LINEAR, false, false, true, false, true>), 512);
+            else AV_GO((gemm_big_kernel<3, false, MODE_LINEAR, false, false, false, false, true>), 512);
+            return av_launch_status("gemm_big<rowstats>");
+        }
+        if (k.ln_rowstats != nullptr) {
+            if (geglu) AV_GO((gemm_big_kernel<3, true, MODE_LINEAR, false, false, false, false, false, true>), 512);
+            else AV_GO((gemm_big_kernel<3, false, MODE_LINEAR, false, false, false, false, false, true>), 512);
+            return av_launch_status("gemm_big<ln>");
+        }
+    }
     if (gn) {
         if (res) AV_GO((gemm_big_kernel<3, false, MODE, false, false, true, true>), 512);
         else AV_GO((gemm_big_kernel<3, false, MODE, false, false, false, true>), 512);
diff --git a/anyv2v_amd/csrc/gemm_common.h b/anyv2v_amd/csrc/gemm_common.h
--- a/anyv2v_amd/csrc/gemm_common.h
+++ b/anyv2v_amd/csrc/gemm_common.h
@@ -24,6 +24,9 @@
     int rast_gm, rast_gn, rast_sm, rast_sn, rast_nfast;
     float* gn_stats;
     int gn_groups, gn_cg;
+    float* rowstats;
+    const float* ln_rowstats;
+    int ln_parts;
 };
 
 struct RowInfo {
@@ -202,6 +205,43 @@
     }
 }
 
+typedef float f2 __attribute__((ext_vector_type(2)));
+constexpr int ROWSTATS_PARK_LD = 42;
+__device__ __forceinline__ void rowstats_park_chunk(const h8& v, float* park_row, int chunk) {
+    float s = 0.f, q = 0.f;
+#pragma unroll
+    for (int e = 0; e < 8; ++e) {
+        const float f = (float)v[e];
+        s += f;
+        q = fmaf(f, f, q);
+    }
+    *(f2*)(park_row + 2 * chunk) = (f2){s, q};
+}
+__device__ __forceinline__ void rowstats_store_row(const float* park_row, float* dst) {
+    float s = 0.f, q = 0.f;
+#pragma unroll
+    for (int c = 0; c < 20; ++c) {
+        const f2 t = *(const f2*)(park_row + 2 * c);
+        s += t[0];
+        q += t[1];
+    }
+    *(f2*)dst = (f2){s, q};
+}
+__device__ __forceinline__ void ln_row_moments(const float* rec, int parts, float inv_k, float eps, float& mean, float& rstd) {
+    float s = 0.f, q = 0.f;
+    for (int i = 0; i < parts / 2; ++i) {
+        const f4 t = *(const f4*)(rec + 4 * i);
+        s += t[0];
+        q += t[1];
+        s += t[2];
+        q += t[3];
+    }
+    mean = s * inv_k;
+    const float m2 = mean * mean;
+    const float var = fmaxf(fmaf(q, inv_k, -m2), 0.0f);
+    rstd = __builtin_amdgcn_rsqf(var + eps);
+}
+
 int av_gemm_mfma_launch(const GemmK& k, const AnyV2VGemmDesc* d, const GemmPlan& plan, hipStream_t s);
 int av_gemm_big_launch(const GemmK& k, const AnyV2VGemmDesc* d, const GemmPlan& plan, hipStream_t s);
 int av_gemm_pp_launch(const GemmK& k, const AnyV2VGemmDesc* d, const GemmPlan& plan, hipStream_t s);
diff --git a/anyv2v_amd/csrc/gemm_mfma.hip b/anyv2v_amd/csrc/gemm_mfma.hip
--- a/anyv2v_amd/csrc/gemm_mfma.hip
+++ b/anyv2v_amd/csrc/gemm_mfma.hip
@@ -2,7 +2,7 @@
 
 #include "gemm_common.h"
 
-template <int NF, bool GEGLU, int BM, int NTHREADS, bool GN = false>
+template <int NF, bool GEGLU, int BM, int NTHREADS, bool GN = false, bool ROWS = false, bool LNT = false>
 __device__ __forceinline__ void epilogue(const GemmK& p, f4 (&acc)[4][NF], char* smem, int m_blk, int n_blk, int wr,
                                          int wc, int lane, int tid, int split = 0, long long* tr = nullptr) {
     constexpr int BN = NF * 32;
@@ -50,14 +50,15 @@
     constexpr int NIT = BM * CPR / NTHREADS;
     static_assert(BM * CPR % NTHREADS == 0, "store phase assumes an exact chunk split");
     const bool full_chunks = (Nout & 7) == 0;
-    h8 rr[NIT];
-    if (p.R != nullptr && full_chunks) {
+    const bool has_res = !LNT && p.R != nullptr;
+    h8 rr[LNT ? 1 : NIT];
+    if (has_res && full_chunks) {
 #pragma unroll
         for (int it = 0; it < NIT; ++it) {
             const int id = tid + it * NTHREADS;
             const int r = id / CPR, cc = id - r * CPR;
             const int m = m_blk + r, n0 = n_out_blk + cc * 8;
-            rr[it] = *(const h8*)((m < p.M && n0 < Nout) ? p.R + (size_t)m * p.ldr + n0 : p.zeros);
+            rr[LNT ? 0 : it] = *(const h8*)((m < p.M && n0 < Nout) ? p.R + (size_t)m * p.ldr + n0 : p.zeros);
         }
     }
     h4 bvec[NF];
@@ -67,9 +68,27 @@
         const half_t* src = (p.bias != nullptr && n + 4 <= p.N) ? p.bias + n : p.zeros;
         bvec[nf] = *(const h4*)src;
     }
-    h4 tvec[GEGLU ? 1 : 4][GEGLU ? 1 : NF];
-    const bool has_rowvec = !GEGLU && p.rowvec != nullptr;
-    if constexpr (!GEGLU) {
+    if constexpr (LNT) {
+        const float inv_k = 1.0f / (float)p.C0;
+#pragma unroll
+        for (int mf = 0; mf < 4; ++mf) {
+            const int m = m_blk + wr * 64 + mf * 16 + l15;
+            float mean, rstd;
+            ln_row_moments(p.ln_rowstats + (size_t)(m < p.M ? m : p.M - 1) * p.ln_parts * 2, p.ln_parts, inv_k, p.ln_eps, mean, rstd);
+#pragma unroll
+            for (int nf = 0; nf < NF; ++nf) {
+                const int n = n_blk + wc * NF * 16 + nf * 16 + 4 * lq;
+                const f4 c1 = *(const f4*)(n + 4 <= p.N ? (const void*)(p.ln_c1 + n) : (const void*)p.zeros);
+#pragma unroll
+                for (int r = 0; r < 4; ++r) acc[mf][nf][r] = fmaf(fmaf(-mean, c1[r], acc[mf][nf][r]), rstd, (float)bvec[nf][r]);
+            }
+        }
+#pragma unroll
+        for (int nf = 0; nf < NF; ++nf) bvec[nf] = (h4){0, 0, 0, 0};
+    }
+    h4 tvec[GEGLU || LNT ? 1 : 4][GEGLU || LNT ? 1 : NF];
+    const bool has_rowvec = !GEGLU && !LNT && p.rowvec != nullptr;
+    if constexpr (!GEGLU && !LNT) {
         if (has_rowvec) {
 #pragma unroll
             for (int mf = 0; mf < 4; ++mf) {
@@ -113,7 +132,9 @@
 #pragma unroll
                     for (int r = 0; r < 4; ++r) {
                         float v = acc[mf][nf][r] + (float)bvec[nf][r];
-                        if (has_rowvec) v += (float)tvec[mf][nf][r];
+                        if constexpr (!LNT) {
+                            if (has_rowvec) v += (float)tvec[mf][nf][r];
+                        }
                         if constexpr (ACT == ACT_SILU) v = av_silu(v);
                         if constexpr (ACT == ACT_GELU) v = av_gelu(v);
                         o[r] = (half_t)v;
@@ -139,10 +160,11 @@
             const int r = id / CPR, cc = id - r * CPR;
             const int m = m_blk + r, n0 = n_out_blk + cc * 8;
             h8 v = *(const h8*)(Cs + r * CS_LD + cc * 8);
-            if (p.R != nullptr) {
-                v = v + rr[it];
+            if (has_res) {
+                v = v + rr[LNT ? 0 : it];
                 if constexpr (GN) *(h8*)(Cs + r * CS_LD + cc * 8) = v;
             }
+            if constexpr (ROWS) rowstats_park_chunk(v, (float*)(Cs + BM * CS_LD) + r * ROWSTATS_PARK_LD, cc);
             if (m < p.M && n0 < Nout) *(h8*)(p.C + (size_t)m * p.ldc + n0) = v;
         }
         if constexpr (GN) {
@@ -155,6 +177,14 @@
                     gn_slab_records(Cs + f * 16 * CS_LD, CS_LD, p.gn_cg, lane,
                                     p.gn_stats + ((size_t)(m0 >> 4) * p.gn_groups + n_blk / p.gn_cg) * 3);
             }
+        }
+        if constexpr (ROWS) {
+            static_assert(!GEGLU && !GN && BN == 160 && BM <= NTHREADS, "row statistics: 160-column tiles, one lane per row");
+            __syncthreads();
+            const int m = m_blk + tid;
+            if (tid < BM && m < p.M)
+                rowstats_store_row((const float*)(Cs + BM * CS_LD) + tid * ROWSTATS_PARK_LD,
+                                   p.rowstats + ((size_t)m * (p.N / 160) + n_blk / 160) * 2);
         }
         return;
     }
@@ -275,9 +305,10 @@
     __builtin_amdgcn_sched_barrier(0);
 }
 
-template <int NF, bool GLDS, bool GEGLU, int MODE, bool TRACE = false, int KO = 0, bool GN = false>
+template <int NF, bool GLDS, bool GEGLU, int MODE, bool TRACE = false, int KO = 0, bool GN = false, bool ROWS = false, bool LNT = false>
 __global__ __launch_bounds__(256, 2) void gemm_mfma_kernel(const GemmK p) {
     constexpr int BM = 128, BN = NF * 32;
+    static_assert(!ROWS || BM * (BN + 8) * 2 + BM * ROWSTATS_PARK_LD * 4 <= 2 * (BM + BN) * 128, "row-statistics park area exceeds LDS");
     constexpr int A_BYTES = BM * 64 * 2;
     constexpr int B_BYTES = BN * 64 * 2;
     constexpr int NB = BN / 32;
@@ -383,7 +414,7 @@
         if constexpr (TRACE) if (tid == 0 && kt < 8) tr[12 + kt] = (long long)__builtin_amdgcn_s_memtime();
     }
     if constexpr (TRACE) if (tid == 0) tr[20] = (long long)__builtin_amdgcn_s_memtime();
-    epilogue<NF, GEGLU, BM, 256, GN>(p, acc, smem, m_blk, n_blk, wr, wc, lane, tid, split, tr);
+    epilogue<NF, GEGLU, BM, 256, GN, ROWS, LNT>(p, acc, smem, m_blk, n_blk, wr, wc, lane, tid, split, tr);
     if constexpr (TRACE) {
         if (tid == 0) tr[26] = (long long)__builtin_amdgcn_s_memtime();
         asm volatile("s_waitcnt vmcnt(0)" ::: "memory");
@@ -404,6 +435,18 @@
 #ifdef ANYV2V_EXPERIMENTS
 #include "../../tools/experiments/gemm_dispatch_mfma_probe.inc"
 #endif
+    if constexpr (MODE == MODE_LINEAR) {
+        if (k.rowstats != nullptr) {
+            AV_GO((gemm_mfma_kernel<5, true, false, MODE_LINEAR, false, 0, false, true>), 256);
+            return av_launch_status("gemm_mfma<rowstats>");
+        }
+        if (k.ln_rowstats != nullptr) {
+            if (geglu) AV_GO((gemm_mfma_kernel<4, true, true, MODE_LINEAR, false, 0, false, false, true>), 256);
+            else if (plan.nf == 5) AV_GO((gemm_mfma_kernel<5, true, false, MODE_LINEAR, false, 0, false, false, true>), 256);
+            else AV_GO((gemm_mfma_kernel<4, true, false, MODE_LINEAR, false, 0, false, false, true>), 256);
+            return av_launch_status("gemm_mfma<ln>");
+        }
+    }
     if (gn) AV_GO((gemm_mfma_kernel<5, true, false, MODE, false, 0, true>), 256);
     else if (geglu && glds) AV_GO((gemm_mfma_kernel<4, true, true, MODE>), 256);
     else if (geglu) AV_GO((gemm_mfma_kernel<4, false, true, MODE>), 256);
diff --git a/anyv2v_amd/csrc/gemm_plan.cpp b/anyv2v_amd/csrc/gemm_plan.cpp
--- a/anyv2v_amd/csrc/gemm_plan.cpp
+++ b/anyv2v_amd/csrc/gemm_plan.cpp
@@ -74,13 +74,12 @@
     }
 }
 
-}
-
-GemmPlan av_gemm_plan(const AnyV2VGemmDesc& d, int hinted_rows) {
+GemmPlan plan_families(const AnyV2VGemmDesc& d, int hinted_rows, const AnyV2VGemmLn* ln) {
     GemmPlan p = {};
     p.nf = 4;
     p.splits = p.tilesN = 1;
-    auto take = [&p](GemmFamily family, const char* what) { p.family = family; p.gn_decline = what; return p; };
+    auto take = [&p](GemmFamily family, const char* what) { p.family = family; p.gn_decline = p.rows_decline = what; return p; };
+    const bool ln_tile = d.ln_c1 != nullptr && ln != nullptr && ln->ln_rowstats != nullptr;
     PLAN_CHECK(d.A0 && d.W, "gemm: null A0/W/C");
     PLAN_CHECK(d.M > 0 && d.N > 0 && d.C0 > 0 && d.C1 >= 0, "gemm: bad M/N/C0/C1 (%d %d %d %d)", d.M, d.N, d.C0, d.C1);
     PLAN_CHECK(d.mode >= 0 && d.mode <= 2, "gemm: bad mode %d", d.mode);
@@ -113,7 +112,7 @@
 
     const bool ws_ok = fast && glds && ws_eligible(d);
     const bool ws_take = ws_ok && !(flags & (ANYV2V_GEMM_NO_WS | ANYV2V_GEMM_NO_BIG)) && (hinted_rows >= 32768 || (flags & ANYV2V_GEMM_FORCE_WS));
-    if (d.ln_c1 != nullptr || ws_take) {
+    if ((d.ln_c1 != nullptr && !ln_tile) || ws_take) {
         p.grid = 256;
         if (ws_ok) p.tilesN = d.N / ws_slab_cols(d);
         if (d.ln_c1 == nullptr) return take(GEMM_WS, "the weight-stationary kernel");
@@ -210,6 +209,17 @@
                        "N / gn_groups dividing 40, M and gn_rows_per_group multiples of 16)";
     else
         p.gn_records = true;
+    if (use.splits > 1)
+        p.rows_decline = "a split-K plan";
+    else if (d.mode != MODE_LINEAR || d.act != ACT_NONE || d.rowvec != nullptr || d.N % 160 != 0 || !glds || d.ln_c1 != nullptr ||
+             d.gn_stats != nullptr)
+        p.rows_decline = "a launch other than mode 0, act none, no rowvec, N % 160 = 0 with LDS-DMA staging, or one that also folds "
+                         "LayerNorm in or writes GroupNorm records";
+    else
+        p.rows_records = true;
+    const bool rows_on = ln != nullptr && ln->rowstats != nullptr && p.rows_records;
+    if (rows_on) p.ln_epi = GEMM_EPI_ROWSTATS;
+    if (ln_tile) p.ln_epi = GEMM_EPI_LN_TILE;
     if (use.big) {
         p.family = GEMM_BIG;
         persistent_grid(p, d);
@@ -220,9 +230,25 @@
         return p;
     }
     p.family = GEMM_MFMA128;
-    p.nf = d.gn_stats != nullptr && p.gn_records ? 5 : choose_nf(d.M);
+    p.nf = (d.gn_stats != nullptr && p.gn_records) || rows_on ? 5 : choose_nf(d.M);
     p.tilesN = ceil_div(d.N, p.nf * 32);
     p.tiles = ((d.M + 127) / 128) * p.tilesN;
     p.grid = p.tiles * p.splits;
     return p;
 }
+}
+
+GemmPlan av_gemm_plan(const AnyV2VGemmDesc& d, int hinted_rows, const AnyV2VGemmLn* ln) {
+    GemmPlan p = plan_families(d, hinted_rows, ln);
+    if (p.status != ANYV2V_OK || !(d.ln_c1 != nullptr && ln != nullptr && ln->ln_rowstats != nullptr)) return p;
+    const bool shape_ok = d.mode == MODE_LINEAR && d.C1 == 0 && d.R == nullptr && d.rowvec == nullptr && d.gn_stats == nullptr &&
+                          (d.act == ACT_NONE || d.act == ACT_GEGLU) && (ln->ln_parts == 4 || ln->ln_parts == 8) &&
+                          d.C0 == 160 * ln->ln_parts && ln->rowstats == nullptr && aligned16(d.ln_c1) && aligned16(ln->ln_rowstats);
+    const bool family_ok = (p.family == GEMM_MFMA128 || p.family == GEMM_BIG) && (d.flags & ANYV2V_GEMM_LDS_DMA) && p.splits == 1;
+    if (!(shape_ok && family_ok))
+        PLAN_FAIL(ANYV2V_EUNSUPPORTED, "gemm: ln_rowstats (LayerNorm fold on the tile kernels) needs mode 0, C0 = 160 x ln_parts (4 | 8), act none / "
+                  "GEGLU, no rowvec / R / C1 / gn_stats / rowstats, 16-byte aligned operands and an unsplit 128-row or persistent plan with "
+                  "LDS-DMA staging -- got C0 %d N %d act %d parts %d on %s (splits %d)", d.C0, d.N, d.act, ln->ln_parts,
+                  av_gemm_family_name(p.family), p.splits);
+    return p;
+}
diff --git a/anyv2v_amd/csrc/gemm_plan.h b/anyv2v_amd/csrc/gemm_plan.h
--- a/anyv2v_amd/csrc/gemm_plan.h
+++ b/anyv2v_amd/csrc/gemm_plan.h
@@ -8,6 +8,7 @@
 
 enum GemmFamily { GEMM_NAIVE, GEMM_WS, GEMM_WS_LN, GEMM_MFMA128, GEMM_BIG, GEMM_PP, GEMM_SW, GEMM_SW_STREAMK, GEMM_SWH, GEMM_FAMILY_COUNT };
 const char* av_gemm_family_name(GemmFamily f);
+enum GemmLnEpilogue { GEMM_EPI_PLAIN, GEMM_EPI_ROWSTATS, GEMM_EPI_LN_TILE };
 void anyv2v_set_error(const char* fmt, ...);
 
 constexpr int AV_GEMM_BM = 192, AV_GEMM_BN = 320;
@@ -25,6 +26,9 @@
     int sk_blocks;
     bool gn_records;
     const char* gn_decline;
+    GemmLnEpilogue ln_epi;
+    bool rows_records;
+    const char* rows_decline;
 };
 
-GemmPlan av_gemm_plan(const AnyV2VGemmDesc& d, int hinted_rows);
+GemmPlan av_gemm_plan(const AnyV2VGemmDesc& d, int hinted_rows, const AnyV2VGemmLn* ln = nullptr);
diff --git a/anyv2v_amd/ops.py b/anyv2v_amd/ops.py
--- a/anyv2v_amd/ops.py
+++ b/anyv2v_amd/ops.py
@@ -69,7 +69,7 @@
 def gemm(a0: torch.Tensor, w: torch.Tensor, *, a1: Optional[torch.Tensor] = None, bias=None, rowvec=None,
          rowvec_div: int = 0, residual=None, act: int = ACT_NONE, out: Optional[torch.Tensor] = None,
          mode: int = MODE_LINEAR, conv=None, temporal=None, M: Optional[int] = None, naive: bool = False, ln=None, gn=None,
-         _query: bool = False):
+         rowstats_out: Optional[torch.Tensor] = None, ln_rowstats: Optional[torch.Tensor] = None, _query=False):
     lib = _lib.load()
     _rowmajor(a0, "A0")
     _rowmajor(w, "W")
@@ -129,9 +129,31 @@
             assert stats.dtype == torch.float32 and stats.is_cuda and stats.is_contiguous()
             d.gn_stats, d.gn_stats_floats = stats.data_ptr(), stats.numel()
     if _query:
-        return int(lib.anyv2v_gemm_gn_stats_floats(C.byref(d)))
-    _lib.check(lib.anyv2v_gemm_f16(C.byref(d), _stream()), "anyv2v_gemm_f16")
-    return out
+        return int((lib.anyv2v_gemm_rowstats_floats if _query == "rowstats" else lib.anyv2v_gemm_gn_stats_floats)(C.byref(d)))
+    if rowstats_out is None and ln_rowstats is None:
+        _lib.check(lib.anyv2v_gemm_f16(C.byref(d), _stream()), "anyv2v_gemm_f16")
+        return out
+    e = _lib.GemmLn()
+    for t in (rowstats_out, ln_rowstats):
+        assert t is None or (t.dtype == torch.float32 and t.is_cuda and t.is_contiguous())
+    if rowstats_out is not None:
+        e.rowstats, e.rowstats_floats = rowstats_out.data_ptr(), rowstats_out.numel()
+    if ln_rowstats is not None:
+        assert ln is not None, "ln_rowstats goes with ln=(c1, eps)"
+        assert C0 % 160 == 0 and ln_rowstats.numel() >= 2 * M * (C0 // 160), "ln_rowstats: [M, K / 160, 2] records of a0's rows"
+        e.ln_rowstats, e.ln_parts = ln_rowstats.data_ptr(), C0 // 160
+    _lib.check(lib.anyv2v_gemm_ln_f16(C.byref(d), C.byref(e), _stream()), "anyv2v_gemm_ln_f16")
+    return out
+
+
+def ln_launches(reset: bool = True) -> dict:
+    c = (C.c_int64 * 4)()
+    _lib.load().anyv2v_gemm_ln_launches(c, int(reset))
+    return {"rows_mfma128": c[0], "rows_big": c[1], "ln_mfma128": c[2], "ln_big": c[3]}
+
+
+def gemm_rowstats_floats(a0: torch.Tensor, w: torch.Tensor, **kw) -> int:
+    return gemm(a0, w, _query="rowstats", **kw)
 
 
 def gemm_gn_stats_floats(a0: torch.Tensor, w: torch.Tensor, *, rows_per_group: int, groups: int = 32, **kw) -> int:
@@ -198,7 +220,15 @@
     return out
 
 
-def ln_gemm_supported(M: int, K: int, N: int, act: int = ACT_NONE, hinted: bool = True) -> bool:
+LN_ROWSTATS = _parse_switch(os.environ.get("ANYV2V_LN_ROWSTATS"))
+
+
+def ln_gemm_supported(M: int, K: int, N: int, act: int = ACT_NONE, hinted: bool = True, rowstats: bool = False) -> bool:
+    if rowstats and K in (640, 1280):
+        other = (_lib.ANYV2V_GEMM_PP | _lib.ANYV2V_GEMM_SW | _lib.ANYV2V_GEMM_STREAMK | _lib.ANYV2V_GEMM_FORCE_STREAMK
+                 | _lib.ANYV2V_GEMM_SWH | _lib.ANYV2V_GEMM_NAIVE)
+        return (not FORCE_NAIVE and USE_GLDS and not (GEMM_FLAGS & other) and act in (ACT_NONE, ACT_GEGLU)
+                and N % (128 if act == ACT_GEGLU else 8) == 0)
     if FORCE_NAIVE or not USE_GLDS or (GEMM_FLAGS & (_lib.ANYV2V_GEMM_NO_WS | _lib.ANYV2V_GEMM_NO_BIG)) or (M * _HINT[0] // _HINT[1] if hinted else M) < 32768:
         return False
     if K == 320:
diff --git a/anyv2v_amd/unet.py b/anyv2v_amd/unet.py
--- a/anyv2v_amd/unet.py
+++ b/anyv2v_amd/unet.py
@@ -206,6 +206,17 @@
     return out
 
 
+LN_ROWSTATS_TALLY = {}
+
+
+def _gemm_rows(a, w, *, bias, residual=None, rows=None):
+    if rows is not None and ops.gemm_rowstats_floats(a, w, bias=bias, residual=residual) > 0:
+        rec = torch.empty((a.shape[0], w.shape[0] // 160, 2), dtype=torch.float32, device=a.device)
+        rows.append(rec)
+        return ops.gemm(a, w, bias=bias, residual=residual, rowstats_out=rec)
+    return ops.gemm(a, w, bias=bias, residual=residual)
+
+
 class Geom:
 
     def __init__(self, kind: str, B: int, F: int, HW: int):
@@ -225,16 +236,18 @@
         self.t = None
         self.src_io = None
 
-    def run(self, attn: "Attention", ctx, h, geom: Geom, residual, kv=None, ln_in=None):
+    def run(self, attn: "Attention", ctx, h, geom: Geom, residual, kv=None, ln_in=None, rows=None):
         Cq = attn.inner_dim
         if ln_in is not None:
-            h, (w_in, b_in, c1_in), ln_eps = ln_in
-
-            def proj(rows, lo=0, out=None):
-                return ops.gemm(rows, w_in[lo:], bias=b_in[lo:], ln=(c1_in[lo:], ln_eps), out=out)
-        else:
-            def proj(rows, lo=0, out=None):
-                return ops.gemm(rows, (attn._w_qkv if kv is None else attn.to_q.weight)[lo:], out=out)
+            h, (w_in, b_in, c1_in), ln_eps = ln_in[:3]
+            rec_in = ln_in[3] if len(ln_in) > 3 else None
+
+            def proj(rows_, lo=0, out=None, r0=0):
+                return ops.gemm(rows_, w_in[lo:], bias=b_in[lo:], ln=(c1_in[lo:], ln_eps), out=out,
+                                ln_rowstats=None if rec_in is None else rec_in[r0:r0 + rows_.shape[0]])
+        else:
+            def proj(rows_, lo=0, out=None, r0=0):
+                return ops.gemm(rows_, (attn._w_qkv if kv is None else attn.to_q.weight)[lo:], out=out)
         T = h.shape[0]
         o = torch.empty((T, Cq), dtype=torch.float16, device=h.device)
         if kv is None:
@@ -248,12 +261,12 @@
                 ops.attention(src_qk[:, :Cq], src_qk[:, Cq:], qkv[:, 2 * Cq:], o, batch=geom.batch, heads=attn.heads, Sq=geom.S,
                               Sk=geom.S, inner=geom.inner, q_strides=geom.strides, kv_strides=geom.strides,
                               qk_mod=geom.batch // 2, scale=attn.scale)
-                return ops.gemm(o, attn.to_out[0].weight, bias=attn.to_out[0].bias, residual=residual)
+                return _gemm_rows(o, attn.to_out[0].weight, bias=attn.to_out[0].bias, residual=residual, rows=rows)
             if inject and T % 3 == 0 and _V_ONLY:
                 Ts = T // 3
                 qkv = torch.empty((T, 3 * Cq), dtype=torch.float16, device=h.device)
                 proj(h[:Ts], 0, qkv[:Ts])
-                proj(h[Ts:], 2 * Cq, qkv[Ts:, 2 * Cq:])
+                proj(h[Ts:], 2 * Cq, qkv[Ts:, 2 * Cq:], r0=Ts)
             else:
                 qkv = proj(h)
             if io is not None and io[0] == "record":
@@ -267,7 +280,7 @@
             k_, v_, Sk = kv
             ops.attention(q, k_, v_, o, batch=geom.batch, heads=attn.heads, Sq=geom.S, Sk=Sk, inner=1,
                           q_strides=geom.strides, kv_strides=(Sk, 0, 1), kv_div=geom.F, scale=attn.scale)
-        return ops.gemm(o, attn.to_out[0].weight, bias=attn.to_out[0].bias, residual=residual)
+        return _gemm_rows(o, attn.to_out[0].weight, bias=attn.to_out[0].bias, residual=residual, rows=rows)
 
 
 class Attention(nn.Module):
@@ -300,10 +313,10 @@
     def prepare_attention_mask(self, attention_mask, target_length, batch_size, out_dim=3):
         return attention_mask
 
-    def run(self, ctx, h, geom: Geom, residual, kv=None, ln_in=None):
+    def run(self, ctx, h, geom: Geom, residual, kv=None, ln_in=None, rows=None):
         proc = self.processor
         if isinstance(proc, HipAttnProcessor):
-            return proc.run(self, ctx, h, geom, residual, kv, ln_in)
+            return proc.run(self, ctx, h, geom, residual, kv, ln_in, rows)
         assert ln_in is None, "a foreign processor takes the normalised hidden states"
         return self._run_foreign(proc, ctx, h, geom, residual, kv)
 
@@ -363,8 +376,8 @@
         if ln_in is None and w2s is not None and ops.ff_fused_supported(h.shape[0], h.shape[1], w2s.shape[0] * 32):
             return ops.ff_geglu(h, self.net[0]._w, self.net[0]._b, w2s, self.net[2].bias, residual=residual)
         if ln_in is not None:
-            x, (w_in, b_in, c1_in), ln_eps = ln_in
-            g = ops.gemm(x, w_in, bias=b_in, act=ACT_GEGLU, ln=(c1_in, ln_eps))
+            x, (w_in, b_in, c1_in), ln_eps = ln_in[:3]
+            g = ops.gemm(x, w_in, bias=b_in, act=ACT_GEGLU, ln=(c1_in, ln_eps), ln_rowstats=ln_in[3] if len(ln_in) > 3 else None)
         elif self.geglu:
             g = ops.gemm(h, self.net[0]._w, bias=self.net[0]._b, act=ACT_GEGLU)
         else:
@@ -384,10 +397,21 @@
 
     def pack(self):
         self._ln = {}
+        self._lnr = {}
         dim = self.norm1.weight.shape[0]
+        cat = lambda a: torch.cat([a.to_q.weight.data, a.to_k.weight.data, a.to_v.weight.data], 0)
+        il = lambda t, n: torch.stack([t[:n].reshape(n // 16, 16, *t.shape[1:]), t[n:].reshape(n // 16, 16, *t.shape[1:])], 1) \
+            .reshape(2 * n, *t.shape[1:]).contiguous()
+        if dim in (640, 1280) and ops.LN_ROWSTATS and not _NO_LN_FOLD:
+            self._lnr["attn1"] = ops.ln_fold(cat(self.attn1), None, self.norm1.weight.data, self.norm1.bias.data)
+            w2 = self.attn2.to_q.weight.data if self.attn2.is_cross else cat(self.attn2)
+            self._lnr["attn2"] = ops.ln_fold(w2, None, self.norm2.weight.data, self.norm2.bias.data)
+            if self.ff.geglu:
+                g = self.ff.net[0]
+                w, b, c1 = ops.ln_fold(g.proj.weight.data, g.proj.bias.data, self.norm3.weight.data, self.norm3.bias.data)
+                self._lnr["ff"] = (il(w, g.dim_out), il(b, g.dim_out), il(c1, g.dim_out))
         if dim not in (320, 512) or _NO_LN_FOLD:
             return
-        cat = lambda a: torch.cat([a.to_q.weight.data, a.to_k.weight.data, a.to_v.weight.data], 0)
         if dim == 320:
             self._ln["attn1"] = ops.ln_fold(cat(self.attn1), None, self.norm1.weight.data, self.norm1.bias.data)
             w2 = self.attn2.to_q.weight.data if self.attn2.is_cross else cat(self.attn2)
@@ -395,42 +419,70 @@
         if self.ff.geglu and _LN_FOLD_FF:
             g = self.ff.net[0]
             w, b, c1 = ops.ln_fold(g.proj.weight.data, g.proj.bias.data, self.norm3.weight.data, self.norm3.bias.data)
-            n = g.dim_out
-            il = lambda t: torch.stack([t[:n].reshape(n // 16, 16, *t.shape[1:]), t[n:].reshape(n // 16, 16, *t.shape[1:])], 1) \
-                .reshape(2 * n, *t.shape[1:]).contiguous()
-            self._ln["ff"] = (il(w), il(b), il(c1))
+            self._ln["ff"] = (il(w, g.dim_out), il(b, g.dim_out), il(c1, g.dim_out))
 
     def _fold(self, name, proc_ok, M, N, act=ACT_NONE, per_branch=False):
         f = getattr(self, "_ln", {}).get(name)
         return f if (f is not None and proc_ok and ops.ln_gemm_supported(M, self.norm1.weight.shape[0], N, act, hinted=not per_branch)) else None
 
-    def run(self, ctx, x, geom: Geom, expand=None, shrink=None):
+    def _fold_rows(self, name, rec, why_not, N, act=ACT_NONE):
+        f = getattr(self, "_lnr", {}).get(name)
+        if f is None:
+            return None
+        if why_not is None and rec is None:
+            why_not = "no records: split-K producer, or a caller that passes none (frame-parallel shards)"
+        if why_not is None and not ops.ln_gemm_supported(0, self.norm1.weight.shape[0], N, act, rowstats=True):
+            why_not = "flags select a kernel without the fold"
+        key = "folded" if why_not is None else why_not
+        LN_ROWSTATS_TALLY[key] = LN_ROWSTATS_TALLY.get(key, 0) + 1
+        return f if why_not is None else None
+
+    def run(self, ctx, x, geom: Geom, expand=None, shrink=None, rec=None):
         dim = x.shape[1]
         rows_b = lambda t, g: t.shape[0] // g.B
-        f = self._fold("attn1", isinstance(self.attn1.processor, HipAttnProcessor), rows_b(x, geom), 3 * dim, per_branch=True)
-        if f is not None:
+        hip1, hip2 = isinstance(self.attn1.processor, HipAttnProcessor), isinstance(self.attn2.processor, HipAttnProcessor)
+        foreign = "a foreign attention processor"
+        want = bool(getattr(self, "_lnr", None))
+        out_rec = [] if want and hip1 else None
+        fr = self._fold_rows("attn1", rec, None if hip1 else foreign, 3 * dim)
+        f = self._fold("attn1", hip1, rows_b(x, geom), 3 * dim, per_branch=True)
+        if fr is not None:
+            x = self.attn1.run(ctx, None, geom, residual=x, ln_in=(x, fr, self.norm1.eps, rec), rows=out_rec)
+        elif f is not None:
             x = self.attn1.run(ctx, None, geom, residual=x, ln_in=(x, f, self.norm1.eps))
         else:
             h = ops.layernorm(x, self.norm1.weight, self.norm1.bias, self.norm1.eps)
-            x = self.attn1.run(ctx, h, geom, residual=x)
+            x = self.attn1.run(ctx, h, geom, residual=x, rows=out_rec) if hip1 else self.attn1.run(ctx, h, geom, residual=x)
+        rec = out_rec[0] if out_rec else None
+        why_not = None if hip2 else foreign
         if expand is not None:
             after = getattr(ctx, "batch_hint_after", None)
             ctx, geom = expand
             x = expand_shared(x, ctx)
+            rec, why_not = None, "expand_shared gathers the rows"
             if after is not None:
                 ops.set_batch_hint(*after)
         if shrink is not None:
+            rec = None if rec is None else rec[x.shape[0] // 3:]
             x = x[x.shape[0] // 3:]
             geom = shrink
             ops.set_batch_hint(3, 2)
         kv = ctx.kv_for(self.attn2) if self.attn2.is_cross else None
-        f = self._fold("attn2", isinstance(self.attn2.processor, HipAttnProcessor), rows_b(x, geom), dim if self.attn2.is_cross else 3 * dim,
-                       per_branch=True)
-        if f is not None:
+        n2 = dim if self.attn2.is_cross else 3 * dim
+        out_rec = [] if want and hip2 else None
+        fr = self._fold_rows("attn2", rec, why_not, n2)
+        f = self._fold("attn2", hip2, rows_b(x, geom), n2, per_branch=True)
+        if fr is not None:
+            x = self.attn2.run(ctx, None, geom, residual=x, kv=kv, ln_in=(x, fr, self.norm2.eps, rec), rows=out_rec)
+        elif f is not None:
             x = self.attn2.run(ctx, None, geom, residual=x, kv=kv, ln_in=(x, f, self.norm2.eps))
         else:
             h = ops.layernorm(x, self.norm2.weight, self.norm2.bias, self.norm2.eps)
-            x = self.attn2.run(ctx, h, geom, residual=x, kv=kv)
+            x = self.attn2.run(ctx, h, geom, residual=x, kv=kv, rows=out_rec) if hip2 else self.attn2.run(ctx, h, geom, residual=x, kv=kv)
+        rec = out_rec[0] if out_rec else None
+        fr = self._fold_rows("ff", rec, None if hip2 else foreign, 8 * dim, ACT_GEGLU)
+        if fr is not None:
+            return self.ff.run(None, residual=x, ln_in=(x, fr, self.norm3.eps, rec))
         f = self._fold("ff", True, x.shape[0], 8 * dim, ACT_GEGLU)
         if f is not None:
             return self.ff.run(None, residual=x, ln_in=(x, f, self.norm3.eps))
@@ -451,15 +503,18 @@
         HW = H * W
         h = ops.groupnorm(x, self.norm.weight, self.norm.bias, ctx.stats, HW, groups=self.norm.num_groups,
                           eps=self.norm.eps)
-        h = ops.gemm(h, self.proj_in.weight, bias=self.proj_in.bias)
+        rows = [] if getattr(self.transformer_blocks[0], "_lnr", None) and getattr(ctx, "fp", None) is None else None
+        h = _gemm_rows(h, self.proj_in.weight, bias=self.proj_in.bias, rows=rows)
+        rec = rows[0] if rows else None
         geom = Geom("spatial", ctx.B, ctx.F, HW)
         for i, blk in enumerate(self.transformer_blocks):
+            rec_i, rec = rec, None
             if full_ctx is not None and i == 0:
-                h = blk.run(ctx, h, geom, expand=(full_ctx, Geom("spatial", full_ctx.B, full_ctx.F, HW)))
+                h = blk.run(ctx, h, geom, expand=(full_ctx, Geom("spatial", full_ctx.B, full_ctx.F, HW)), rec=rec_i)
                 ctx, geom = full_ctx, Geom("spatial", full_ctx.B, full_ctx.F, HW)
                 x = expand_shared(x, full_ctx)
             else:
-                h = blk.run(ctx, h, geom)
+                h = blk.run(ctx, h, geom, rec=rec_i)
         return ops.gemm(h, self.proj_out.weight, bias=self.proj_out.bias, residual=x)
 
 
@@ -480,16 +535,19 @@
     def _run(self, ctx, x, HW, shard):
         h = ops.groupnorm(x, self.norm.weight, self.norm.bias, ctx.stats, ctx.F * HW, groups=self.norm.num_groups,
                           eps=self.norm.eps, shard=shard)
-        h = ops.gemm(h, self.proj_in.weight, bias=self.proj_in.bias)
+        rows = [] if getattr(self.transformer_blocks[0], "_lnr", None) and shard is None else None
+        h = _gemm_rows(h, self.proj_in.weight, bias=self.proj_in.bias, rows=rows)
+        rec = rows[0] if rows else None
         geom = Geom("temporal", ctx.B, ctx.F, HW)
         drop = shard is None and getattr(ctx, "drop_tail_at", None) is self and not self.transformer_blocks[0].attn2.is_cross
         for i, blk in enumerate(self.transformer_blocks):
+            rec_i, rec = rec, None
             if drop and i == 0:
-                h = blk.run(ctx, h, geom, shrink=Geom("temporal", ctx.B - 1, ctx.F, HW))
+                h = blk.run(ctx, h, geom, shrink=Geom("temporal", ctx.B - 1, ctx.F, HW), rec=rec_i)
                 geom = Geom("temporal", ctx.B - 1, ctx.F, HW)
                 x = x[x.shape[0] // 3:]
             else:
-                h = blk.run(ctx, h, geom)
+                h = blk.run(ctx, h, geom, rec=rec_i)
         return ops.gemm(h, self.proj_out.weight, bias=self.proj_out.bias, residual=x)
 
 
diff --git a/include/anyv2v_hip.h b/include/anyv2v_hip.h
--- a/include/anyv2v_hip.h
+++ b/include/anyv2v_hip.h
@@ -66,6 +66,17 @@
 int anyv2v_gemm_f16(const AnyV2VGemmDesc* d, void* stream);
 int64_t anyv2v_gemm_gn_stats_floats(const AnyV2VGemmDesc* d);
 int64_t anyv2v_gemm_gn_launches(int32_t reset);
+
+typedef struct AnyV2VGemmLn {
+    float* rowstats;
+    int64_t rowstats_floats;
+    const float* ln_rowstats;
+    int32_t ln_parts;
+    int32_t reserved0;
+} AnyV2VGemmLn;
+int anyv2v_gemm_ln_f16(const AnyV2VGemmDesc* d, const AnyV2VGemmLn* ln, void* stream);
+int64_t anyv2v_gemm_rowstats_floats(const AnyV2VGemmDesc* d);
+void anyv2v_gemm_ln_launches(int64_t counts[4], int32_t reset);
 
 typedef struct AnyV2VFFDesc {
     const void* X;
```

Result: no change. 3.032 frames/s (-0.1%).
